# vice87/gam-ngs

Measured on AMD Instinct MI355X. Metric: GCUPS, higher is better.
Workload: dtype int32 (fast blocks: exact packed-f16 offsets from per-lane int32 bases, two tasks per register; results bit-identical to the reference's int64 DP)

## Files before the change

gam_ngs_amd/api.py:

```python
import ctypes as C
from dataclasses import dataclass, field
from typing import List, Optional, Sequence

from . import lib as L

GAP_A, GAP_B, MATCH, MISMATCH = 0, 1, 2, 3
OPS_CHARS = "ABMX"
DEFAULT_BAND_SIZE = 150


def _check(ctx, rc, what):
    if rc != 0:
        msg = L.load_library().gamdp_last_error(ctx.handle) if ctx is not None and ctx.handle else b""
        raise L.GamdpError("%s failed with code %d: %s" % (what, rc, (msg or b"").decode()))


class Context:

    def __init__(self, device: int = 0):
        self.lib = L.load_library()
        h = C.c_void_p()
        rc = self.lib.gamdp_ctx_create(device, C.byref(h))
        if rc != 0:
            raise L.GamdpError("gamdp_ctx_create(device=%d) failed with code %d (no gfx950 GPU?); "
                               "libgamdp has no CPU fallback" % (device, rc))
        self.handle = h
        self.device = device

    def set_arena_bytes(self, nbytes: int):
        _check(self, self.lib.gamdp_ctx_set_arena_bytes(self.handle, nbytes), "gamdp_ctx_set_arena_bytes")

    def last_error(self):
        return (self.lib.gamdp_last_error(self.handle) or b"").decode()

    def set_l1_hits(self, mode: int):
        _check(self, self.lib.gamdp_ctx_set_l1_hits(self.handle, mode), "gamdp_ctx_set_l1_hits")

    def l1_hits_stats(self):
        st = L.L1HitsStats()
        _check(self, self.lib.gamdp_ctx_l1_hits_stats(self.handle, C.byref(st)), "gamdp_ctx_l1_hits_stats")
        return st.as_dict()

    def set_l1_chain(self, mode: int):
        _check(self, self.lib.gamdp_ctx_set_l1_chain(self.handle, mode), "gamdp_ctx_set_l1_chain")

    def set_l1_walk_bands(self, which: int):
        _check(self, self.lib.gamdp_ctx_set_l1_walk_bands(self.handle, which), "gamdp_ctx_set_l1_walk_bands")

    def l1_chain_stats(self):
        st = L.L1ChainStats()
        _check(self, self.lib.gamdp_ctx_l1_chain_stats(self.handle, C.byref(st)), "gamdp_ctx_l1_chain_stats")
        return st.as_dict()

    def set_walk_skip(self, mode: int):
        _check(self, self.lib.gamdp_ctx_set_walk_skip(self.handle, mode), "gamdp_ctx_set_walk_skip")

    def walk_skip_stats(self):
        st = L.WalkSkipStats()
        _check(self, self.lib.gamdp_ctx_walk_skip_stats(self.handle, C.byref(st)), "gamdp_ctx_walk_skip_stats")
        return st.as_dict()

    def l1_tail_calls(self):
        n = C.c_size_t()
        _check(self, self.lib.gamdp_ctx_l1_tail_calls(self.handle, None, 0, C.byref(n)), "gamdp_ctx_l1_tail_calls")
        arr = (L.L1TailCall * max(1, n.value))()
        _check(self, self.lib.gamdp_ctx_l1_tail_calls(self.handle, arr, n.value, C.byref(n)), "gamdp_ctx_l1_tail_calls")
        return [(arr[i].merge_block, bool(arr[i].right), arr[i].begin_a, arr[i].source) for i in range(n.value)]

    def kernel_time(self, reset=False):
        ms, n = C.c_double(), C.c_uint64()
        self.lib.gamdp_ctx_kernel_time(self.handle, C.byref(ms), C.byref(n), int(reset))
        return ms.value, n.value

    def launch_info(self):
        n = C.c_size_t()
        self.lib.gamdp_ctx_launch_info(self.handle, None, 0, C.byref(n))
        arr = (L.LaunchInfo * max(1, n.value))()
        self.lib.gamdp_ctx_launch_info(self.handle, arr, n.value, C.byref(n))
        return [arr[i].as_dict() for i in range(n.value)]

    def score_info(self):
        n = C.c_size_t()
        self.lib.gamdp_ctx_score_info(self.handle, None, 0, C.byref(n))
        arr = (L.ScoreLaunchInfo * max(1, n.value))()
        self.lib.gamdp_ctx_score_info(self.handle, arr, n.value, C.byref(n))
        return [arr[i].as_dict() for i in range(n.value)]

    def carry_info(self):
        n = C.c_size_t()
        self.lib.gamdp_ctx_carry_info(self.handle, None, 0, C.byref(n))
        arr = (L.ScoreLaunchInfo * max(1, n.value))()
        self.lib.gamdp_ctx_carry_info(self.handle, arr, n.value, C.byref(n))
        return [arr[i].as_dict() for i in range(n.value)]

    def close(self):
        if getattr(self, "handle", None):
            self.lib.gamdp_ctx_destroy(self.handle)
            self.handle = None

    def __del__(self):
        try:
            self.close()
        except Exception:
            pass


class SequenceSet:

    def __init__(self, ctx: Context, seqs: Sequence[bytes], ascii: bool = True):
        self.ctx = ctx
        n = len(seqs)
        self._keep = [bytes(s) for s in seqs]
        arr = (C.c_char_p * max(1, n))(*self._keep)
        lens = (C.c_uint64 * max(1, n))(*[len(s) for s in self._keep])
        h = C.c_void_p()
        rc = ctx.lib.gamdp_seqset_create(ctx.handle, arr, lens, n, int(ascii), C.byref(h))
        _check(ctx, rc, "gamdp_seqset_create")
        self.handle = h
        self.lengths = [len(s) for s in self._keep]

    @classmethod
    def from_fasta(cls, ctx: "Context", path: str):
        names, codes = load_fasta(path)
        self = cls(ctx, codes, ascii=False)
        self.names = names
        return self

    @classmethod
    def synthetic(cls, ctx: "Context", first_pair: int, n_pairs: int, length: int, stride: int = 1):
        self = cls.__new__(cls)
        self.ctx = ctx
        self._keep = []
        h = C.c_void_p()
        _check(ctx, ctx.lib.gamdp_seqset_create_synth_strided(ctx.handle, first_pair, stride, n_pairs, length, C.byref(h)),
               "gamdp_seqset_create_synth_strided")
        self.handle = h
        self.lengths = [ctx.lib.gamdp_seqset_length(h, i) for i in range(2 * n_pairs)]
        return self

    def __len__(self):
        return len(self.lengths)

    def contig(self, idx, rc=False, off=0):
        return Contig(self, idx, rc, off)

    def close(self):
        if getattr(self, "handle", None) and self.ctx.handle:
            self.ctx.lib.gamdp_seqset_destroy(self.handle)
        self.handle = None

    def __del__(self):
        try:
            self.close()
        except Exception:
            pass


class MultiContext:

    def __init__(self, devices: Sequence[int]):
        self.lib = L.load_library()
        arr = (C.c_int * len(devices))(*devices)
        h = C.c_void_p()
        rc = self.lib.gamdp_multi_create(arr, len(devices), C.byref(h))
        if rc != 0:
            raise L.GamdpError("gamdp_multi_create(%r) failed with code %d; libgamdp has no CPU fallback" % (list(devices), rc))
        self.handle = h
        self.devices = list(devices)

    def last_error(self):
        return (self.lib.gamdp_multi_last_error(self.handle) or b"").decode()

    def set_l1_hits(self, mode: int):
        for i in range(len(self.devices)):
            if self.lib.gamdp_ctx_set_l1_hits(self.lib.gamdp_multi_ctx(self.handle, i), mode) != 0:
                raise L.GamdpError("gamdp_ctx_set_l1_hits(%r) failed on context %d" % (mode, i))

    def set_l1_chain(self, mode: int):
        for i in range(len(self.devices)):
            if self.lib.gamdp_ctx_set_l1_chain(self.lib.gamdp_multi_ctx(self.handle, i), mode) != 0:
                raise L.GamdpError("gamdp_ctx_set_l1_chain(%r) failed on context %d" % (mode, i))

    def set_l1_walk_bands(self, which: int):
        for i in range(len(self.devices)):
            if self.lib.gamdp_ctx_set_l1_walk_bands(self.lib.gamdp_multi_ctx(self.handle, i), which) != 0:
                raise L.GamdpError("gamdp_ctx_set_l1_walk_bands(%r) failed on context %d" % (which, i))

    def set_walk_skip(self, mode: int, which=None):
        for i in (range(len(self.devices)) if which is None else (which,)):
            if self.lib.gamdp_ctx_set_walk_skip(self.lib.gamdp_multi_ctx(self.handle, i), mode) != 0:
                raise L.GamdpError("gamdp_ctx_set_walk_skip(%r) failed on context %d" % (mode, i))

    def walk_skip_stats(self):
        out = []
        for i in range(len(self.devices)):
            st = L.WalkSkipStats()
            if self.lib.gamdp_ctx_walk_skip_stats(self.lib.gamdp_multi_ctx(self.handle, i), C.byref(st)) != 0:
                raise L.GamdpError("gamdp_ctx_walk_skip_stats failed on context %d" % i)
            out.append(st.as_dict())
        return out

    def l1_chain_stats(self):
        out = []
        for i in range(len(self.devices)):
            st = L.L1ChainStats()
            if self.lib.gamdp_ctx_l1_chain_stats(self.lib.gamdp_multi_ctx(self.handle, i), C.byref(st)) != 0:
                raise L.GamdpError("gamdp_ctx_l1_chain_stats failed on context %d" % i)
            out.append(st.as_dict())
        return out

    def l1_hits_stats(self):
        out = []
# ... 471 lines not shown
```

gam_ngs_amd/csrc/gamdp_dev.h:

```cpp
#pragma once
#include <stdint.h>

namespace gamdp {

typedef uint32_t u32;
typedef uint64_t u64;

constexpr int SEQ_PAD_BASES = 4096;

#ifndef GAMDP_WAVES_PER_SIMD
#define GAMDP_WAVES_PER_SIMD 5
#endif

struct DevTask {
    const u32* a2;
    const u32* an;
    const u32* b2;
    const u32* bn;
    int64_t a_base;
    int64_t b_base;
    int64_t end_a;
    int32_t alen, blen;
    int32_t begin_a, begin_b;
    int32_t X;
    int32_t band;
    u32 flags;
    u32 res_idx;
    u64 ops_off;
    u64 ops_cap;
};

enum : u32 { TF_FORCE_START = 1, TF_FORCE_END = 2, TF_WANT_OPS = 4,
             TF_DIAG_SKIP_TRACEBACK = 8 ,
             TF_NO_DIRFREE = 16 ,
             TF_DIAG_COUNT_MAT = 32 ,
             TF_PADDING = 64 ,
             TF_CALL_N = 128  };

#ifdef GAMDP_DIAG
constexpr u32 TF_LIVE_MASK = ~0u;
#else
constexpr u32 TF_LIVE_MASK = ~(u32)(TF_DIAG_SKIP_TRACEBACK | TF_NO_DIRFREE | TF_DIAG_COUNT_MAT);
#endif

struct DevResult {
    int32_t begin_a, begin_b;
    int32_t score;
    u32 n_match, length;
    int32_t first_a, first_b, last_a, last_b;
    u32 flags;
};

struct LaunchParams {
    const DevTask* tasks;
    u32 n_tasks;
    u32* cursor;
    DevResult* results;
    uint8_t* ops_buf;
    u32* scratch;
    u64 slot_words;
    u64 dir_words;
    u32 ypad;
    u64 ckpt_off;
    u64 bnd_off;
    u32 flags;
    u32 prio_R, prio_from;
    u32* stats;
};
enum : int { LS_UNITS = 0, LS_DIRFREE, LS_PACKED_TOP, LS_PACKED_TOP_MIXED, LS_STRIPS, LS_TOP_WANTED, LS_SKIP_TESTS, LS_SKIP_TESTED, LS_SKIP_GROUPS, LS_SKIP_SHORT, LS_COUNT = 12 };
constexpr u32 LP_WALK_SKIP_DIAG = 32;
constexpr u32 LP_WALK_SIDE_BY_SIDE = 1;
constexpr u32 LP_NO_PACKED_TOP = 2;
constexpr u32 LP_NO_PACKED_TOP_MIXED = 16;
constexpr u32 LP_WALK_PRIO_SHIFT = 8;

enum KernelId : int {
    K_C17_CE4 = 0,
    K_C17_CE4_N,
    K_C5_CE0,
    K_C5_CE0_N,
    K_P17_CE4,
    K_O19_CE15,
    K_Q19_CE15,
    K_Q19_CE15_N,
    K_GEN_C2, K_GEN_C3, K_GEN_C5, K_GEN_C9, K_GEN_C17,
    K_WIDE,
    K_COUNT
};

constexpr int FAMILY_COLS[5] = {2, 3, 5, 9, 17};
constexpr int band_cols(const u32 band)
{
    for (int k = 0; k < 4; k++) if (2 * (u64)band + 1 <= 64u * (u64)FAMILY_COLS[k]) return FAMILY_COLS[k];
    return 17;
}
constexpr int cols_index(const int cols)
{
    for (int k = 0; k < 4; k++) if (FAMILY_COLS[k] == cols) return k;
    return 4;
}
static_assert(K_GEN_C3 == K_GEN_C2 + 1 && K_GEN_C5 == K_GEN_C2 + 2 && K_GEN_C9 == K_GEN_C2 + 3 && K_GEN_C17 == K_GEN_C2 + 4,
              "K_GEN_C2 .. K_GEN_C17: contiguous, in the order of FAMILY_COLS");
constexpr int gen_kernel_id(const int cols) { return (int)K_GEN_C2 + cols_index(cols); }

#if defined(__HIPCC__)
#define GAMDP_HD __host__ __device__
#else
#define GAMDP_HD
#endif

constexpr u32 PAT_OFF = 0x2000u, PAT_MIN = 0x0400u, PAT_MAX = 0x7BFFu - 21u;
GAMDP_HD inline u32 pat_encode(int rel) { return (PAT_OFF + (u32)rel) & 0xFFFFu; }
GAMDP_HD inline int pat_decode(u32 p16) { return (int)(int16_t)(uint16_t)p16 - (int)PAT_OFF; }

GAMDP_HD inline int preflight_hd(u64 alen, u64 blen, u64 band, u64 begin_a, u64 end_a, u64 begin_b, u64 end_b, bool fs, bool fe,
                                 u64* X_out, u64* cells_out)
{
    constexpr int64_t MAXGAP = 10;
    enum { S_OK = 0, S_EMPTY = 1, S_OOR = 2, S_INVALID = 3 };
    auto mn = [](int64_t x, int64_t y) { return x < y ? x : y; };
    *X_out = 0;
    *cells_out = 0;
    if (end_b < begin_b) return S_EMPTY;
    if (begin_a >= (1ull << 31) - 65536) return S_INVALID;
    const int64_t lo = ((int64_t)begin_a - (int64_t)band) > 0 ? ((int64_t)begin_a - (int64_t)band) : 0, hi = (int64_t)begin_a + (int64_t)band;
    if (begin_b >= blen) {
        bool any;
        if (!fs) any = lo < (int64_t)alen;
        else any = (lo <= mn(hi, MAXGAP)) || lo < (int64_t)alen;
        return any ? S_OOR : S_INVALID;
    }
    if (end_b >= blen) end_b = blen - 1;
    u64 X = end_b - begin_b + 1;
    const u64 lim = alen + band - begin_a;
    if (lim < X) X = lim;
    if (X > 500000) X = 500000;
    if (X == 0) return S_INVALID;
    const u64 Y = 2 * band + 1;
    *X_out = X;
    *cells_out = X * Y;
    if (fs) {
        const int64_t up = mn(hi, MAXGAP);
        if (lo <= up && up >= (int64_t)alen) return S_OOR;
    }
    if (begin_a > alen + band) {
        bool found = false;
        if (!fe) found = begin_a + (X - 1) - band <= end_a;
        {
            const bool ge = end_a >= begin_a + band;
            const int64_t i0 = ge ? (int64_t)(end_a - (begin_a + band)) : 0;
            const int64_t j0 = ge ? (int64_t)(2 * band) : (int64_t)(2 * band) - (int64_t)(begin_a + band - end_a);
            if (j0 >= 0 && (u64)i0 < X) {
                const int64_t kmax = mn((int64_t)X - 1 - i0, j0);
                if (!fe) found = true;
                else if (X >= (u64)MAXGAP + 1 && (u64)(i0 + kmax) >= X - 1 - (u64)MAXGAP) found = true;
            }
        }
        return found ? S_OOR : S_EMPTY;
    }
    return S_OK;
}

GAMDP_HD inline bool npre_window_has_n(const u32* pre, int64_t len, bool rc, u64 off, int64_t lo, int64_t hi)
{
    if (pre == nullptr) return false;
    const int64_t o_lo = (int64_t)off + (lo > 0 ? lo : 0), o_hi = ((int64_t)off + hi < len - 1) ? (int64_t)off + hi : len - 1;
    if (o_lo > o_hi) return false;
    const int64_t f_lo = rc ? len - 1 - o_hi : o_lo, f_hi = rc ? len - 1 - o_lo : o_hi;
    return pre[(f_hi / 256) + 1] != pre[f_lo / 256];
}
GAMDP_HD inline bool call_touches_n(const u32* pre_a, int64_t alen, bool a_rc, u64 a_off, const u32* pre_b, int64_t blen, bool b_rc, u64 b_off,
                                    int64_t band, int64_t begin_a, int64_t begin_b, int64_t X, int64_t margin)
{
    return npre_window_has_n(pre_a, alen, a_rc, a_off, begin_a - band - margin, begin_a + X - 1 + band + margin) ||
           npre_window_has_n(pre_b, blen, b_rc, b_off, begin_b - margin, begin_b + X - 1 + margin);
}

struct DevBlk { int32_t m_begin, m_end, s_begin, s_end; };
struct DevMB {
    const u32 *a2, *an;
    const u32 *b2, *bn;
    const u32 *b2rc, *bnrc;
    u64 mlen, slen;
    u64 m_start, s_start, s_end;
    u64 align_thr;
    u32 first_blk, n_blocks;
    u32 audit_first;
    u32 rows;
    u32 try_rev;
    u32 has_n;
    const u32 *npre_a, *npre_b;
    u32 max_x;
    u64 slot_off[2];
    u64 slot_words, dir_words;
    u64 ckpt_off, bnd_off;
};
struct ChainOut { u32 n_dp; u32 state; u32 t_begin, t_end; u32 hw, hw_twin; u32 t_end_att[2]; u32 t_begin2; u32 pad; };
struct ChainWin { u64 begin_a, end_a, begin_b, end_b; u32 X; u32 info; };
struct ChainSync { u32 verdict[2]; u32 n[2]; u32 fin; u32 cancel; u32 t_begin; u32 hw[2]; u32 t_end[2]; u32 t_begin2; };
struct ChainParams {
    const DevMB* mbs; const DevBlk* blks; u32 n_mbs;
    u32 n_twins;
    ChainSync* sync;
    u32 first_mb;
    u32* cursor;
    DevResult* audit; ChainOut* out;
    ChainWin* win;
    u32* scratch; u32 ypad; u32 band;
    u32 max_rows;
    DevResult* host_audit; ChainOut* host_out; u32* host_done; u32 epoch;
    ChainWin* host_win;
    u32 skew_call;
    int32_t n_margin;
    u32 n_by_contig;
};
int chain_slots_per_workgroup();

struct KernelInfo {
    KernelId id;
    const char* name;
    int cols;
    u32 band;
    int tasks_per_wave;
    int waves_per_cu;
    bool n_aware;
    bool dirfree;
    bool two_dir_images;
    int dir_block_words;
    int ckpt_words;
    int bnd_words;
    void (*kernel)(LaunchParams);
};
extern const KernelInfo kernel_info[K_COUNT];

inline u64 dir_words_for(const KernelInfo& ki, const u64 X, const u64 band)
{
    const u64 Y = 2 * band + 1;
    if (ki.id == K_WIDE) return X * Y;
    const u64 C = (u64)ki.cols, LE = (Y - 1) / C;
    const u64 extra = ki.tasks_per_wave > 1 ? 3 : 0;
    return ((X - 1 + LE) / 16 + 1 + extra) * (u64)ki.dir_block_words;
}
struct SlotGeom { u64 dir_words; u32 ypad; u64 slot_words, ckpt_off, bnd_off; };
inline SlotGeom slot_geom(const KernelInfo& ki, const u64 max_dir_words, const u32 max_band)
{
    SlotGeom g;
    g.ypad = ((2 * max_band + 2 + 63) / 64) * 64;
    g.dir_words = ((max_dir_words + 63) / 64) * 64;
    const u64 tpw = (u64)ki.tasks_per_wave;
    u64 ckpt_words = 0, bnd_words = 0;
    if (tpw > 1 || ki.dirfree) {
        const u64 nblk = g.dir_words / (u64)ki.dir_block_words + 1;
        ckpt_words = (nblk / 4 + 2) * (u64)ki.ckpt_words;
        bnd_words = (nblk + 4) * (u64)ki.bnd_words;
    }
    const u64 sides_end = (ki.two_dir_images ? 2 * g.dir_words : g.dir_words) + 4ull * g.ypad * tpw;
    g.slot_words = sides_end + ckpt_words + bnd_words;
    g.ckpt_off = ckpt_words ? sides_end : 0;
    g.bnd_off = g.ckpt_off + ckpt_words;
    return g;
}

struct KernelFamily {
    const void* kernel[5];
    const char* name[5];
    unsigned threads;
};
const KernelFamily& score_family();
const KernelFamily& carry_family();
const KernelFamily& chain_carry_family();
const KernelFamily& chain_gen_family();

enum ChainNBit : int {
    CHAIN_N_UNREPORTED,
    CHAIN_N_BY_WINDOW,
    CHAIN_N_EVERY_DP
};
struct ChainKernel {
    const char* name;
    const void* kernel;
    int cols;
    unsigned threads;
    const KernelInfo* slots;
    bool twins;
    ChainNBit n_bit;
};
const ChainKernel& chain2_kernel(bool has_n);
inline ChainKernel family_chain_kernel(const KernelFamily& f, const int cols, const KernelInfo* slots, const bool twins, const ChainNBit n_bit)
{
    return ChainKernel{f.name[cols_index(cols)], f.kernel[cols_index(cols)], cols, f.threads, slots, twins, n_bit};
}

int launch_align(int kid, const LaunchParams& p, unsigned n_slots, unsigned dyn_lds, void* stream);
int launch_wide(const LaunchParams& p, unsigned n_slots, void* stream);
constexpr int WIDE_WORKGROUPS_PER_CU = 8;

struct alignas(16) ScoreRec {
    int32_t score, end_a, end_b;
    u32 info;
};
struct ScoreParams {
    const DevTask* tasks;
    u32 n_tasks;
    u32* cursor;
    ScoreRec* results;
};

struct CarryParams {
    const DevTask* tasks;
    u32 n_tasks;
    u32* cursor;
    DevResult* results;
};
constexpr u32 CARRY_COLS_SHIFT = 16;


}
```

gam_ngs_amd/csrc/gamdp_host.cpp:

```cpp
#include <hip/hip_runtime.h>

#include <algorithm>
#include <atomic>
#include <thread>
#include <cstdio>
#include <cstdlib>
#include <chrono>
#include <cstring>
#include <memory>
#include <mutex>
#include <string>
#include <vector>

#include "gamdp.h"
#include "gamdp_dev.h"
#include "gamdp_internal.h"
#include "gamdp_hostpool.h"
#include "gamdp_hostsort.h"

namespace gamdp {

#define HIPCHK(ctx, expr)                                                                         \
    do {                                                                                          \
        hipError_t e_ = (expr);                                                                   \
        if (e_ != hipSuccess) {                                                                   \
            (ctx)->set_error(std::string(#expr) + ": " + hipGetErrorString(e_));                  \
            return GAMDP_EHIP;                                                                    \
        }                                                                                         \
    } while (0)

const Diag& diag()
{
    static const Diag d = [] {
        Diag x;
        x.timing = std::getenv("GAMDP_DIAG_TIMING") != nullptr;
#ifdef GAMDP_DIAG
        x.build = true;
        x.skip_traceback = std::getenv("GAMDP_DIAG_SKIP_TRACEBACK") != nullptr;
        x.no_dirfree = std::getenv("GAMDP_DIAG_NO_DIRFREE") != nullptr;
        x.count_mat = std::getenv("GAMDP_DIAG_COUNT_MAT") != nullptr;
        x.force_n = std::getenv("GAMDP_DIAG_FORCE_N") != nullptr;
        if (const char* e = std::getenv("GAMDP_DIAG_N_WINDOW_SHRINK")) x.n_window_shrink = (int64_t)std::atol(e);
        if (const char* e = std::getenv("GAMDP_DIAG_CHAIN_SKEW")) x.chain_skew = (u32)std::atoi(e);
        x.hits_drop = std::getenv("GAMDP_DIAG_HITS_DROP") != nullptr;
#endif
        return x;
    }();
    return d;
}

const Tuning& tuning()
{
    static const Tuning t = [] {
        Tuning x;
        auto set = [](const char* name) { return std::getenv(name) != nullptr; };
        const char* e;
        x.no_merge_n = set("GAMDP_NO_MERGE_N") || set("GAMDP_QUAD_MIN");
        if ((e = std::getenv("GAMDP_QUAD_MIN"))) x.quad_min = std::atol(e);
        if ((e = std::getenv("GAMDP_OCTO_MIN_ROWS"))) x.octo_min_rows = (size_t)std::min(std::max(std::atol(e), 0L), 500000L);
        x.no_pair = set("GAMDP_NO_PAIR");
        x.no_aux_launch = set("GAMDP_NO_AUX_LAUNCH");
        if ((e = std::getenv("GAMDP_SIDE_WALK_ROUNDS"))) x.side_walk_rounds = (u64)std::min(std::max(std::atol(e), 0L), 1000000L);
        x.no_packed_top = set("GAMDP_NO_PACKED_TOP");
        x.no_packed_top_mixed = set("GAMDP_NO_PACKED_TOP_MIXED");
        if ((e = std::getenv("GAMDP_WALK_PRIO"))) x.walk_prio = std::atoi(e) & 3;
        x.no_prio = set("GAMDP_NO_PRIO");
        if ((e = std::getenv("GAMDP_CHUNK_MIN"))) x.chunk_min = (long)std::atoll(e);
        if ((e = std::getenv("GAMDP_CHUNK_MIN_ROUNDS"))) x.chunk_min_rounds = std::min(std::max(std::atof(e), 0.0), 1000.0);
        if ((e = std::getenv("GAMDP_CHUNK_FIRST_DIV"))) x.chunk_first_div = (size_t)std::min(std::max(4L, std::atol(e)), 1024L);
        x.l1_rounds = set("GAMDP_L1_ROUNDS");
        x.l1_no_twins = set("GAMDP_L1_NO_TWINS");
        if ((e = std::getenv("GAMDP_L1_COHORTS"))) x.l1_cohorts = std::min(16, std::max(1, std::atoi(e)));
        if ((e = std::getenv("GAMDP_L1_COHORT_MIN"))) x.l1_cohort_min = (size_t)std::max(1L, std::atol(e));
        if ((e = std::getenv("GAMDP_L1_DEVICE_HITS"))) x.l1_device_hits = std::atoi(e) == 1;
        if ((e = std::getenv("GAMDP_L1_CHAIN_CARRY"))) x.l1_chain_carry = std::atoi(e) == 1;
        if ((e = std::getenv("GAMDP_L1_WALK_ANY_BAND"))) x.l1_walk_any_band = std::atoi(e) == 1;
        if ((e = std::getenv("GAMDP_WALK_SKIP"))) x.walk_skip = std::atoi(e) == 1;
        return x;
    }();
    return t;
}


static inline uint8_t encode_char(char ch)
{
    switch (ch) {
    case 'A': case 'a': return 0;
    case 'T': case 't': return 1;
    case 'C': case 'c': return 2;
    case 'G': case 'g': return 3;
    default: return 4;
    }
}

static inline u64 padded_bases(u64 len) { return ((len + 2 * (u64)SEQ_PAD_BASES + 63) / 64) * 64 + 64; }

static void pack_into(const uint8_t* codes, u64 len, bool rc, u32* plane2, u32* planeN, u64 at)
{
    static const uint8_t comp[5] = {1, 0, 3, 2, 4};
    for (u64 i = 0; i < len; i++) {
        uint8_t c = rc ? comp[codes[len - 1 - i] > 4 ? 4 : codes[len - 1 - i]] : codes[i];
        if (c > 4) c = 4;
        const u64 k = at + i;
        if (c == 4) planeN[k >> 5] |= 1u << (k & 31);
        else plane2[k >> 4] |= (u32)c << ((k & 15) * 2);
    }
}

int SeqSet::upload(Ctx* ctx_, const uint8_t* const* seqs, const uint64_t* lens, uint32_t n, bool ascii)
{
    ctx = ctx_;
    codes.resize(n);
    this->lens.assign(lens, lens + n);
    fwd.resize(n);
    rc.assign(n, DevSeq{nullptr, nullptr});
    has_n.assign(n, 0);
    npre.assign(n, std::vector<u32>());
    u64 total = 0;
    std::vector<u64> at(n);
    for (u32 i = 0; i < n; i++) {
        if (lens[i] >= (1ull << 31) - (1ull << 20)) return GAMDP_EINVAL;
        at[i] = total + SEQ_PAD_BASES;
        total += padded_bases(lens[i]);
    }
    std::vector<u32> h2(total / 16 + 4, 0), hn(total / 32 + 4, 0);
    for (u32 i = 0; i < n; i++) {
        codes[i].resize(lens[i]);
        bool anyn = false;
        for (u64 k = 0; k < lens[i]; k++) {
            uint8_t c = ascii ? encode_char((char)seqs[i][k]) : (seqs[i][k] > 4 ? (uint8_t)4 : seqs[i][k]);
            codes[i][k] = c;
            anyn |= (c == 4);
        }
        has_n[i] = anyn;
        if (anyn) {
            std::vector<u32>& pre = npre[i];
            pre.assign((size_t)(lens[i] + 255) / 256 + 1, 0);
            for (u64 k = 0; k < lens[i]; k++) pre[(size_t)(k / 256) + 1] += (codes[i][k] == 4);
            for (size_t k = 1; k < pre.size(); k++) pre[k] += pre[k - 1];
        }
        pack_into(codes[i].data(), lens[i], false, h2.data(), hn.data(), at[i]);
    }
    HIPCHK(ctx, hipMalloc(&d2, h2.size() * sizeof(u32)));
    HIPCHK(ctx, hipMalloc(&dn, hn.size() * sizeof(u32)));
    HIPCHK(ctx, hipMemcpyAsync(d2, h2.data(), h2.size() * sizeof(u32), hipMemcpyHostToDevice, ctx->stream));
    HIPCHK(ctx, hipMemcpyAsync(dn, hn.data(), hn.size() * sizeof(u32), hipMemcpyHostToDevice, ctx->stream));
    HIPCHK(ctx, hipStreamSynchronize(ctx->stream));
    for (u32 i = 0; i < n; i++) fwd[i] = DevSeq{d2 + at[i] / 16, dn + at[i] / 32};
    dev_npre.assign(n, nullptr);
    {
        std::vector<u32> all;
        std::vector<size_t> first(n, 0);
        for (u32 i = 0; i < n; i++) { first[i] = all.size(); all.insert(all.end(), npre[i].begin(), npre[i].end()); }
        if (!all.empty()) {
            HIPCHK(ctx, hipMalloc(&d_npre, all.size() * sizeof(u32)));
            HIPCHK(ctx, hipMemcpy(d_npre, all.data(), all.size() * sizeof(u32), hipMemcpyHostToDevice));
            for (u32 i = 0; i < n; i++) if (!npre[i].empty()) dev_npre[i] = d_npre + first[i];
        }
    }
    return 0;
}


namespace {
struct SynthGen {
    uint64_t s;
    explicit SynthGen(uint64_t k) : s(0x47414DULL + k * 0xD1B54A32D192ED03ULL) { (void)next(); }
    uint64_t next()
    {
        uint64_t z = (s += 0x9E3779B97F4A7C15ULL);
        z = (z ^ (z >> 30)) * 0xBF58476D1CE4E5B9ULL;
        z = (z ^ (z >> 27)) * 0x94D049BB133111EBULL;
        return z ^ (z >> 31);
    }
};
uint64_t synth_pair_codes(uint64_t k, uint64_t len, uint8_t* master, uint8_t* slave)
{
    SynthGen g(k);
    for (uint64_t i = 0; i < len; i++) master[i] = (uint8_t)(g.next() >> 62);
    uint64_t n = 0;
    for (uint64_t i = 0; i < len; i++) {
        const uint64_t r = g.next(), u = r >> 40;
        if (u >= 167772) {
            uint8_t base = master[i];
            if (u < 671088) base = (uint8_t)((base + 1 + (r & 0xFFFF) % 3) & 3);
            slave[n++] = base;
        }
        const uint64_t r2 = g.next();
        if ((r2 >> 40) < 167772) slave[n++] = (uint8_t)(r2 & 3);
    }
    return n;
}
}

int SeqSet::upload_synth(Ctx* ctx_, uint64_t first_pair, uint64_t stride_pairs, uint32_t n_pairs, uint64_t len)
{
    ctx = ctx_;
    const u32 n = 2 * n_pairs;
    lens.assign(n, 0);
    fwd.resize(n);
    rc.assign(n, DevSeq{nullptr, nullptr});
    has_n.assign(n, 0);
    dev_npre.assign(n, nullptr);
    const u64 stride = padded_bases(len + len / 8 + 64);
    const u64 total = stride * n;
    std::vector<u32> h2(total / 16 + 4, 0), hn(total / 32 + 4, 0);
    const unsigned nt = std::max(1u, std::min(32u, std::thread::hardware_concurrency()));
    Threads pool;
    std::atomic<u32> cursor(0);
    std::atomic<int> failed(0);
    for (unsigned t = 0; t < nt; t++) {
        pool.start([&]() {
            failed |= guarded_thread_body([&]() -> int {
            std::vector<uint8_t> m(len), s(len + len / 8 + 64);
            for (;;) {
                const u32 k = cursor.fetch_add(1);
                if (k >= n_pairs) break;
                const u64 sl = synth_pair_codes(first_pair + (u64)k * stride_pairs, len, m.data(), s.data());
                lens[2 * k] = len;
                lens[2 * k + 1] = sl;
                pack_into(m.data(), len, false, h2.data(), hn.data(), stride * (2 * k) + SEQ_PAD_BASES);
                pack_into(s.data(), sl, false, h2.data(), hn.data(), stride * (2 * k + 1) + SEQ_PAD_BASES);
            }
            return 0;
            });
        });
    }
    pool.join();
    if (failed) return GAMDP_ENOMEM;
    HIPCHK(ctx, hipMalloc(&d2, h2.size() * sizeof(u32)));
// ... 361 lines not shown

static void pair_aux_launch(std::vector<Launch>& launches, int n_cu, u64 arena_call)
{
    int small = -1, big = -1;
    for (size_t li = 0; li < launches.size(); li++) {
        const Launch& L = launches[li];
        const u64 tpw = (u64)kernel_info[L.kid].tasks_per_wave, units = L.count / tpw;
        if (tpw == 1 && L.kid != K_WIDE && units <= (u64)L.n_slots && units <= 4ull * (u64)n_cu) { if (small < 0) small = (int)li; }
        else if (tpw > 1 && units >= 2ull * L.n_slots) { if (big < 0) big = (int)li; }
    }
    if (small < 0 || big < 0 || launches.size() != 2) return;
    const u64 main_words = launches[big].slot_words * launches[big].n_slots, small_words = launches[small].slot_words * launches[small].n_slots;
    if ((main_words + small_words) * sizeof(u32) <= arena_call) {
        launches[small].aux = true;
        launches[small].scratch_off = main_words;
    }
}

int Ctx::align_plan(u64 arena_call)
{
    Plan& plan = w_plan;
    plan.launches.clear(); plan.items.clear(); plan.n_host_tasks = 0;
    const std::vector<u32>& rowsv = w_rows;
    for (int kid = 0; kid < K_COUNT; kid++) {
        auto& g = w_groups[kid];
        if (g.empty()) continue;
        const KernelInfo& ki = kernel_info[kid];
        const u32 max_resident = (u32)n_cu * (u32)ki.waves_per_cu;
        if (ki.band != 0) sort_by_key_desc(g, rowsv, &w_sort_tmp, &w_sort_count);
        else sort_by_key_desc(g, w_key, &w_sort_tmp, &w_sort_count);
        std::vector<std::vector<u32>> work;
        work.push_back(g);
        while (!work.empty()) {
            std::vector<u32> cur = std::move(work.back());
            work.pop_back();
            u32 maxband = ki.band;
            u64 maxdir = 0;
            if (ki.band != 0) maxdir = dir_words_for(ki, rowsv[cur[0]], ki.band);
            else {
                std::mutex red;
                parallel_for(cur.size(), [&](size_t lo, size_t hi) {
                    u32 mb = 0; u64 md = 0;
                    for (size_t k = lo; k < hi; k++) { const u32 i = cur[k]; mb = std::max<u32>(mb, (u32)w_prep[i].dt.band); md = std::max(md, w_prep[i].dir_words); }
                    std::lock_guard<std::mutex> gd(red);
                    maxband = std::max(maxband, mb); maxdir = std::max(maxdir, md);
                });
            }
            const SlotGeom geom = slot_geom(ki, maxdir, maxband);
            const u32 tpw = (u32)ki.tasks_per_wave;
            const u64 fit = arena_call / (geom.slot_words * sizeof(u32));
            if (fit == 0) { set_error("scratch arena too small for one task"); return GAMDP_ENOMEM; }
            const u64 want = std::min<u64>((cur.size() + tpw - 1) / tpw, max_resident);
            if (fit < want && cur.size() > 1) {
                std::vector<u32> big, small;
                for (u32 i : cur) ((ki.band ? dir_words_for(ki, rowsv[i], ki.band) : w_prep[i].dir_words) * 2 >= maxdir ? big : small).push_back(i);
                if (!small.empty()) {
                    work.push_back(std::move(small));
                    work.push_back(std::move(big));
                    continue;
                }
            }
            Launch L;
            const size_t padded = (cur.size() + tpw - 1) / tpw * tpw;
            L.kid = kid; L.first = (u32)plan.n_host_tasks; L.count = (u32)padded;
            L.slot_words = geom.slot_words; L.dir_words = geom.dir_words; L.ypad = geom.ypad; L.band_max = maxband;
            L.ckpt_off = geom.ckpt_off; L.bnd_off = geom.bnd_off;
            L.n_slots = (u32)std::min<u64>(want, fit);
            L.dyn_lds = 0;
            plan.n_host_tasks += padded;
            plan.items.push_back(std::move(cur));
            plan.launches.push_back(L);
        }
    }
    if (!tuning().no_aux_launch && !interval_sink && !defer_frees) pair_aux_launch(plan.launches, n_cu, arena_call);
    return 0;
}


int Ctx::grow_staging(u64 base)
{
    if (base + 1 <= cap_pinned) return 0;
    free_host(h_tasks);
    free_host(h_results);
    h_tasks = nullptr; h_results = nullptr; cap_pinned = 0;
    const u64 want = base + base / 4 + 256;
    if (hipHostMalloc(&h_tasks, want * sizeof(DevTask)) != hipSuccess ||
        hipHostMalloc(&h_results, want * sizeof(DevResult)) != hipSuccess) {
        set_error("hipHostMalloc of staging buffers failed");
        return GAMDP_ENOMEM;
    }
    cap_pinned = want;
    return 0;
}

int Ctx::align_stage(const AlignCall& a)
{
    const Plan& plan = w_plan;
    int rc_ = grow(this, d_tasks, cap_tasks, plan.n_host_tasks + 1);
    if (rc_) return rc_;
    if ((rc_ = grow_staging(std::max<u64>(plan.n_host_tasks, a.n)))) return rc_;
    for (size_t li = 0; li < plan.launches.size(); li++) {
        const std::vector<u32>& cur = plan.items[li];
        const Launch& L = plan.launches[li];
        DevTask* dst = h_tasks + L.first;
        parallel_for(cur.size(), [&](size_t lo, size_t hi) { for (size_t k = lo; k < hi; k++) dst[k] = w_prep[cur[k]].dt; });
        auto pad = [&](size_t k, const DevTask& of) { dst[k] = of; dst[k].res_idx = (u32)a.n; dst[k].flags = (dst[k].flags & ~(u32)TF_WANT_OPS) | TF_PADDING; };
        size_t k = cur.size();
        for (; k < L.count; k++) pad(k, dst[cur.size() - 1]);
    }
    return 0;
}

int Ctx::align_scratch(u64 arena_call)
{
    const std::vector<Launch>& launches = w_plan.launches;
    u64 need_scratch = 0;
    for (auto& L : launches) need_scratch = std::max(need_scratch, L.scratch_off + L.slot_words * L.n_slots);
    if (need_scratch > cap_scratch) {
        if (d_scratch) { free_dev(d_scratch); d_scratch = nullptr; cap_scratch = 0; }
        if (defer_frees) need_scratch = std::max(need_scratch, std::min<u64>(2 * need_scratch, arena_call / sizeof(u32)));
        if (hipMalloc(&d_scratch, need_scratch * sizeof(u32)) != hipSuccess) {
            d_scratch = nullptr;
            (void)hipGetLastError();
            flush_frees();
            if (arena_div == 1) {
                for (Ctx* h : helpers)
                    if (h->d_scratch) { (void)hipFree(h->d_scratch); h->d_scratch = nullptr; h->cap_scratch = 0; }
                if (d_chain_scratch) { (void)hipFree(d_chain_scratch); d_chain_scratch = nullptr; cap_chain_scratch = 0; }
            }
            if (hipMalloc(&d_scratch, need_scratch * sizeof(u32)) != hipSuccess) {
                d_scratch = nullptr;
                set_error("hipMalloc of scratch arena (" + std::to_string(need_scratch * sizeof(u32)) + " bytes) failed");
                return GAMDP_ENOMEM;
            }
        }
        cap_scratch = need_scratch;
    }
    if (launches.size() > cap_cursor) {
        free_dev(d_cursor);
        d_cursor = nullptr; cap_cursor = 0;
        HIPCHK(this, hipMalloc(&d_cursor, launches.size() * (1 + LS_COUNT) * sizeof(u32)));
        cap_cursor = (u32)launches.size();
    }
    return 0;
}

static void launch_policy(const Launch& L, LaunchParams& p, const int walk_skip)
{
    const Tuning& tu = tuning();
    const u64 tpw = (u64)kernel_info[L.kid].tasks_per_wave, units = L.count / tpw;
    p.flags = (L.kid == K_P17_CE4 && (u64)L.count / 2 <= tu.side_walk_rounds * L.n_slots) ? LP_WALK_SIDE_BY_SIDE : 0u;
    if (tu.no_packed_top) p.flags |= LP_NO_PACKED_TOP;
    if (tu.no_packed_top_mixed) p.flags |= LP_NO_PACKED_TOP_MIXED;
    if (L.kid == K_O19_CE15 && walk_skip == GAMDP_WALK_SKIP_DIAG) p.flags |= LP_WALK_SKIP_DIAG;
    p.flags |= (tu.walk_prio >= 0 ? (u32)tu.walk_prio : (units > 2ull * L.n_slots ? 1u : 0u)) << LP_WALK_PRIO_SHIFT;
    p.prio_R = tu.no_prio ? 0u : (u32)std::max<u64>(1, L.dir_words / (u64)kernel_info[L.kid].dir_block_words);
    const u64 shaped = (L.kid == K_P17_CE4 ? 2ull : 1ull) * L.n_slots;
    p.prio_from = units <= 2ull * L.n_slots ? 0u : (u32)(units - std::min<u64>(units, shaped));
}

int Ctx::align_run(AlignCall& a)
{
    const std::vector<Launch>& launches = w_plan.launches;
    u32* const d_stats = d_cursor + cap_cursor;
    a.t_gpu = std::chrono::steady_clock::now();
    bool any_aux = false;
    for (auto& L : launches) any_aux |= L.aux;
    struct AuxJoin {
        Ctx* c = nullptr;
        ~AuxJoin() { if (c) { (void)hipEventRecord(c->aux_done, c->aux_stream); (void)hipStreamWaitEvent(c->stream, c->aux_done, 0); } }
    } aux_join;
    HIPCHK(this, hipMemsetAsync(d_cursor, 0, (size_t)cap_cursor * (1 + LS_COUNT) * sizeof(u32), stream));
    if (any_aux) {
        if (!aux_stream) {
            HIPCHK(this, hipStreamCreateWithFlags(&aux_stream, hipStreamNonBlocking));
            HIPCHK(this, hipEventCreateWithFlags(&aux_done, hipEventDisableTiming));
            HIPCHK(this, hipEventCreateWithFlags(&aux_go, hipEventDisableTiming));
        }
        HIPCHK(this, hipEventRecord(aux_go, stream));
        HIPCHK(this, hipStreamWaitEvent(aux_stream, aux_go, 0));
        aux_join.c = this;
        for (auto& L : launches)
            if (L.aux) HIPCHK(this, hipMemcpyAsync(d_tasks + L.first, h_tasks + L.first, (size_t)L.count * sizeof(DevTask), hipMemcpyHostToDevice, aux_stream));
        for (auto& L : launches)
            if (!L.aux) HIPCHK(this, hipMemcpyAsync(d_tasks + L.first, h_tasks + L.first, (size_t)L.count * sizeof(DevTask), hipMemcpyHostToDevice, stream));
    } else {
        HIPCHK(this, hipMemcpyAsync(d_tasks, h_tasks, w_plan.n_host_tasks * sizeof(DevTask), hipMemcpyHostToDevice, stream));
    }
    while (events.size() < launches.size()) {
        hipEvent_t e0, e1;
        HIPCHK(this, hipEventCreate(&e0));
        HIPCHK(this, hipEventCreate(&e1));
        events.push_back({e0, e1});
    }
    for (size_t li = 0; li < launches.size(); li++) {
        const Launch& L = launches[li];
        LaunchParams p;
        p.tasks = d_tasks + L.first; p.n_tasks = L.count; p.cursor = d_cursor + li;
        p.results = d_results; p.ops_buf = d_ops;
        p.scratch = d_scratch + L.scratch_off; p.slot_words = L.slot_words; p.dir_words = L.dir_words; p.ypad = L.ypad;
        p.ckpt_off = L.ckpt_off; p.bnd_off = L.bnd_off;
        p.stats = d_stats + li * LS_COUNT;
        launch_policy(L, p, walk_skip);
        hipStream_t const on = L.aux ? aux_stream : stream;
        HIPCHK(this, hipEventRecord(events[li].first, on));
        const int e = launch_align(L.kid, p, L.n_slots, L.dyn_lds, on);
        if (e != 0) { set_error(std::string("kernel launch failed: ") + hipGetErrorString((hipError_t)e)); return GAMDP_EHIP; }
        HIPCHK(this, hipEventRecord(events[li].second, on));
    }
    if (any_aux) {
        aux_join.c = nullptr;
        HIPCHK(this, hipEventRecord(aux_done, aux_stream));
        HIPCHK(this, hipStreamWaitEvent(stream, aux_done, 0));
    }
    HIPCHK(this, hipMemcpyAsync(h_results, d_results, a.n * sizeof(DevResult), hipMemcpyDeviceToHost, stream));
    a.hops.resize(a.ops_total);
    if (a.ops_total) HIPCHK(this, hipMemcpyAsync(a.hops.data(), d_ops, a.ops_total, hipMemcpyDeviceToHost, stream));
    a.hstats.resize(log_launches ? launches.size() * LS_COUNT : 0);
    if (!a.hstats.empty()) HIPCHK(this, hipMemcpyAsync(a.hstats.data(), d_stats, a.hstats.size() * sizeof(u32), hipMemcpyDeviceToHost, stream));
    a.mark("enqueued");
    HIPCHK(this, hipStreamSynchronize(stream));
    a.mark("gpu done");
    a.ms_gpu = a.since(a.t_gpu);
    return 0;
}

void Ctx::align_collect(AlignCall& a)
{
    const std::vector<Launch>& launches = w_plan.launches;
    const size_t n = a.n;
    bool any_aux = false;
    for (auto& L : launches) any_aux |= L.aux;
    float busy_hi = 0;
    for (size_t li = 0; li < launches.size(); li++) {
        const Launch& L = launches[li];
        const KernelInfo& ki = kernel_info[L.kid];
        float ms = 0;
        if (hipEventElapsedTime(&ms, events[li].first, events[li].second) == hipSuccess) {
            kernel_launches++;
            if (!any_aux) kernel_ms += ms;
            else {
                float off = 0;
                if (li > 0 && hipEventElapsedTime(&off, events[0].first, events[li].first) != hipSuccess) off = busy_hi;
                const float lo = std::max(off, busy_hi), hi = off + ms;
                if (hi > lo) kernel_ms += hi - lo;
                busy_hi = std::max(busy_hi, hi);
            }
        }
        if (log_launches) {
            gamdp_launch_info r;
            std::memset(&r, 0, sizeof(r));
            std::snprintf(r.kernel, sizeof(r.kernel), "%s", ki.name);
            r.n_aware = ki.n_aware ? 1u : 0u;
            r.tasks_per_wavefront = (u32)ki.tasks_per_wave;
            r.tasks = (u32)w_plan.items[li].size();
            r.units = L.count / r.tasks_per_wavefront;
            r.slots = L.n_slots;
            r.band_max = L.band_max;
            const u32* st = a.hstats.data() + li * LS_COUNT;
            r.units_dirfree = st[LS_DIRFREE]; r.units_packed_top = st[LS_PACKED_TOP]; r.units_packed_top_mixed = st[LS_PACKED_TOP_MIXED];
            r.strips = st[LS_STRIPS]; r.units_top_wanted = st[LS_TOP_WANTED];
            if (L.kid == K_O19_CE15) {
                gamdp_walk_skip_stats& W = last_walk_skip;
                W.tests += st[LS_SKIP_TESTS]; W.groups_tested += st[LS_SKIP_TESTED]; W.groups_skipped += st[LS_SKIP_GROUPS];
                W.rows_skipped += 64ull * st[LS_SKIP_GROUPS] - st[LS_SKIP_SHORT];
                W.strips += st[LS_STRIPS];
            }
            r.piece = log_piece;
            r.rounds = L.n_slots ? (double)r.units / (double)L.n_slots : 0.0;
            r.kernel_ms = (double)ms;
            launch_log.push_back(r);
        }
        if (interval_sink && ref_event) {
            float t0 = 0;
            if (hipEventElapsedTime(&t0, ref_event, events[li].first) == hipSuccess) interval_sink->push_back({t0, t0 + ms});
        }
    }
    a.t_fill = std::chrono::steady_clock::now();
    a.mark("events");
    const DevResult* hres = h_results;
    gamdp_result* out = a.out;
    parallel_for(n, [&](size_t lo, size_t hi) {
        for (size_t i = lo; i < hi; i++) {
            if (w_kid[i] < 0) continue;
            fill_result(hres[i], w_key[i], out[i]);
        }
    });
    if (a.ops_total) {
        parallel_for(w_plan.n_host_tasks, [&](size_t lo, size_t hi) {
            for (size_t q = lo; q < hi; q++) {
                const DevTask& d = h_tasks[q];
                const u32 i = d.res_idx;
                if (i >= n) continue;
                if ((d.flags & TF_WANT_OPS) && out[i].status == GAMDP_ST_OK) {
                    const u64 len = std::min<u64>(out[i].length, d.ops_cap);
                    uint8_t* dst = a.ops->ops_buf + a.ops->ops_off[i];
                    const uint8_t* src = a.hops.data() + d.ops_off;
                    if (out[i].length <= d.ops_cap) for (u64 k = 0; k < len; k++) dst[k] = src[len - 1 - k];
                    else for (u64 k = 0; k < len; k++) dst[k] = 0xFF;
                }
            }
        });
    }
    if (diag().timing) {
        a.mark("results");
        std::fprintf(stderr, "libgamdp align: %zu tasks, %zu launches: prepare %.2f ms, plan+stage %.2f ms, upload+kernels+download %.2f ms [ctx %p began %.3f]\n",
                     n, launches.size(), a.ms_prep, a.ms_plan, a.ms_gpu, (void*)this,
                     std::chrono::duration<double, std::milli>(a.t_begin.time_since_epoch()).count());
        std::fprintf(stderr, "libgamdp align: results %.2f ms [ctx %p began %.3f]\n", a.marks.back().second - std::chrono::duration<double, std::milli>(a.t_fill - a.t_begin).count(), (void*)this,
                     std::chrono::duration<double, std::milli>(a.t_fill.time_since_epoch()).count());
        std::string line = "libgamdp align: phases (ms since the call began):";
        for (auto& m : a.marks) { char b[64]; std::snprintf(b, sizeof b, " %s %.2f", m.first, m.second); line += b; }
        std::fprintf(stderr, "%s; kernels %.2f ms\n", line.c_str(), [&] { double k = 0; for (auto& r : launch_log) k += r.kernel_ms; return k; }());
    }
}

int Ctx::align(const TaskSrc& tasks, size_t n, gamdp_result* out, const gamdp_ops* ops)
{
    if (hipSetDevice(device) != hipSuccess) { set_error("hipSetDevice failed"); return GAMDP_EHIP; }
    if (n == 0) return 0;
    int rc_ = align_check(tasks, n);
    if (rc_) return rc_;
    AlignCall a{tasks, n, out, ops};
    align_prepare(a);
    align_group(a);
    route_merge_n(w_groups, a.rows_of, w_prep, w_kid, n_cu);
    route_band150(w_groups, a.rows_of, n_cu);
    route_band512(w_groups);
    a.ms_prep = a.since(a.t_begin);
    a.mark("groups");
    rc_ = grow(this, d_results, cap_results, n + 1);
    if (rc_) return rc_;
    if (a.ops_total) { rc_ = grow(this, d_ops, cap_ops, a.ops_total); if (rc_) return rc_; }
    if (arena_budget() == 0) { set_error("hipMemGetInfo failed"); return GAMDP_EHIP; }
    const u64 arena_call = this->arena_call();
    if ((rc_ = align_plan(arena_call))) return rc_;
    a.mark("sort+plan");
    if ((rc_ = align_stage(a))) return rc_;
    a.mark("staging");
    if (w_plan.launches.empty()) return 0;
    if ((rc_ = align_scratch(arena_call))) return rc_;
    a.ms_plan = a.since(a.t_begin) - a.ms_prep;
    a.mark("buffers");
    if ((rc_ = align_run(a))) return rc_;
    align_collect(a);
    w_plan.items.clear();
    return 0;
}


struct ScoreCall {
    typedef ScoreRec Rec;
    typedef gamdp_score_result Out;
    typedef ScoreParams Params;
    static constexpr const char* api = "gamdp_score_batch";
    static const KernelFamily& family() { return score_family(); }
    static u32 cols_of(const Rec& r) { return r.info >> 8; }
    static void collect(const Rec& r, u64 cells, Out& o)
    {
        (void)cells;
        o.status = (uint8_t)(r.info & 0xFFu);
        if (o.status != GAMDP_ST_OK) return;
        o.score = r.score;
        o.end_a = (u64)(int64_t)r.end_a; o.end_b = (u64)(int64_t)r.end_b;
    }
};
struct CarryCall {
    typedef DevResult Rec;
    typedef gamdp_result Out;
    typedef CarryParams Params;
    static constexpr const char* api = "gamdp_carry_batch";
    static const KernelFamily& family() { return carry_family(); }
    static u32 cols_of(const Rec& r) { return r.flags >> CARRY_COLS_SHIFT; }
    static void collect(const Rec& r, u64 cells, Out& o) { fill_result(r, cells, o); }
};

template <class K>
int Ctx::fill_only(const TaskSrc& tasks, size_t n, typename K::Out* out, std::vector<gamdp_score_launch_info>& log)
{
    typedef typename K::Rec Rec;
    if (hipSetDevice(device) != hipSuccess) { set_error("hipSetDevice failed"); return GAMDP_EHIP; }
    log.clear();
    if (n == 0) return 0;
    int rc_ = align_check(tasks, n);
    if (rc_) return rc_;
    for (size_t i = 0; i < n; i++) {
        const u32 band = tasks[i].band;
        if (band > GAMDP_MAX_TUNED_BAND) {
            set_error(std::string(K::api) + ": task " + std::to_string(i) + " has band " + std::to_string(band) + ", above GAMDP_MAX_TUNED_BAND");
            return GAMDP_ENOTSUP;
        }
    }
    if (w_prep.size() < n) { w_prep.resize(n); w_status.resize(n); w_key.resize(n); w_kid.resize(n); w_rows.resize(n); }
    std::vector<int8_t> colsv(n);
    parallel_for(n, [&](size_t lo, size_t hi) {
        for (size_t i = lo; i < hi; i++) {
            const int st = w_status[i] = prepare_task(tasks[i], w_prep[i]);
            w_key[i] = w_prep[i].cells;
            std::memset(&out[i], 0, sizeof(out[i]));
            out[i].status = (uint8_t)st;
            out[i].cells = w_prep[i].cells;
            w_prep[i].dt.res_idx = (u32)i;
            colsv[i] = st != GAMDP_ST_OK ? (int8_t)-1 : (int8_t)band_cols((u32)w_prep[i].dt.band);
            w_rows[i] = st != GAMDP_ST_OK ? 0u : (u32)w_prep[i].dt.X;
        }
    });
    struct SLaunch { int cols; u32 first, count, band_max; };
    std::vector<SLaunch> launches;
    std::vector<u32> order, g;
    for (const int cols : FAMILY_COLS) {
        g.clear();
        u32 band_max = 0;
        for (size_t i = 0; i < n; i++) if (colsv[i] == cols) { g.push_back((u32)i); band_max = std::max(band_max, (u32)w_prep[i].dt.band); }
        if (g.empty()) continue;
        sort_by_key_desc(g, w_rows, &w_sort_tmp, &w_sort_count);
        launches.push_back({cols, (u32)order.size(), (u32)g.size(), band_max});
        order.insert(order.end(), g.begin(), g.end());
    }
    if (launches.empty()) return 0;
    static_assert(sizeof(Rec) <= sizeof(DevResult), "the records are staged in the result buffers of align()");
// ... 19 lines not shown
        typename K::Params p;
        p.tasks = d_tasks + L.first; p.n_tasks = L.count; p.cursor = d_cursor + li; p.results = d_rec;
        const int e = launch_kernel(K::family().kernel[cols_index(L.cols)], K::family().threads, p, slots[li], stream);
        if (e != 0) { set_error(std::string("kernel launch failed: ") + hipGetErrorString((hipError_t)e)); return GAMDP_EHIP; }
        HIPCHK(this, hipEventRecord(events[li].second, stream));
    }
    HIPCHK(this, hipMemcpyAsync(h_rec, d_rec, n * sizeof(Rec), hipMemcpyDeviceToHost, stream));
    HIPCHK(this, hipStreamSynchronize(stream));
    parallel_for(n, [&](size_t lo, size_t hi) {
        for (size_t i = lo; i < hi; i++) {
            if (colsv[i] < 0) continue;
            K::collect(h_rec[i], w_key[i], out[i]);
        }
    });
    for (size_t li = 0; li < launches.size(); li++) {
        const SLaunch& L = launches[li];
        float ms = 0;
        if (hipEventElapsedTime(&ms, events[li].first, events[li].second) == hipSuccess) { kernel_launches++; kernel_ms += ms; }
        gamdp_score_launch_info r;
        std::memset(&r, 0, sizeof(r));
        std::snprintf(r.kernel, sizeof(r.kernel), "%s", K::family().name[cols_index(L.cols)]);
        r.cols = K::cols_of(h_rec[order[L.first]]);
        for (u32 k = 0; k < L.count; k++) if (K::cols_of(h_rec[order[L.first + k]]) != r.cols) r.cols = 0;
        r.tasks = L.count; r.slots = slots[li]; r.band_max = L.band_max;
        r.kernel_ms = (double)ms;
        log.push_back(r);
    }
    return 0;
}

int Ctx::score(const TaskSrc& tasks, size_t n, gamdp_score_result* out) { return fill_only<ScoreCall>(tasks, n, out, score_log); }
int Ctx::carry(const TaskSrc& tasks, size_t n, gamdp_result* out) { return fill_only<CarryCall>(tasks, n, out, carry_log); }


static bool batch_pieces(const gamdp_task* tasks, size_t n, const SeqSet* sb, int n_cu, size_t bound[5])
{
    const long chunk_env = tuning().chunk_min;
    bool chunked = chunk_env >= 0 && n >= (size_t)chunk_env;
    bool b150 = false;
    if (chunked) { size_t n150 = 0, cnt = 0; for (size_t i = 0; i < n; i += 64, cnt++) n150 += tasks[i].band == 150; b150 = 2 * n150 >= cnt; }
    if (chunk_env < 0 && n >= 65536) {
        double est = 0;
        size_t cnt = 0;
        size_t n150 = 0;
        u64 rows_max = 0, rows_sum = 0;
        for (size_t i = 0; i < n; i += 64, cnt++) {
            const gamdp_task& t = tasks[i];
            const u64 blen = t.b_id < sb->lens.size() ? sb->lens[t.b_id] - std::min<u64>(t.b_off, sb->lens[t.b_id]) : 0;
            const u64 eb = blen ? std::min<u64>(t.end_b, blen - 1) : 0;
            const u64 rows = (blen && eb >= t.begin_b) ? std::min<u64>(eb - t.begin_b + 1, 500000) : 0;
            est += (double)rows * (2.0 * t.band + 1.0);
            rows_max = std::max(rows_max, rows); rows_sum += rows;
            n150 += t.band == 150;
        }
        b150 = 2 * n150 >= cnt;
        chunked = est / (double)std::max<size_t>(1, cnt) < (b150 ? 4.5e6 : 8e6);
        const double units_per_piece = (double)n * (7.0 / 24.0) / (b150 ? 8.0 : 2.0);
        const bool one_length = (double)rows_max * (double)std::max<size_t>(1, cnt) <= 1.25 * (double)rows_sum;
        const double min_rounds_env = tuning().chunk_min_rounds;
        const double min_rounds = min_rounds_env >= 0 ? min_rounds_env : (one_length ? 3.0 : 2.5);
        if (units_per_piece < min_rounds * 16.0 * (double)n_cu) chunked = false;
        {
            const double cells_total = est / (double)std::max<size_t>(1, cnt) * (double)n;
            const double kernel_ms = cells_total / (b150 ? 7.0e9 : 12.0e9), host_ms = (double)n * 1.5e-5;
            if (min_rounds_env < 0 && host_ms < 0.05 * kernel_ms) chunked = false;
        }
    }
    if (!chunked) return false;
    const size_t first_div = tuning().chunk_first_div;
    const size_t round = (size_t)n_cu * 16 * (b150 ? 8 : 2);
    auto whole = [&](size_t v, bool up) { const size_t r = up ? (v + round - 1) / round : v / round; return std::max<size_t>(1, r) * round; };
    const bool by_rounds = chunk_env < 0;
    const size_t n0 = by_rounds ? std::min(n, whole(n / first_div, false)) : n / first_div;
    const size_t per = by_rounds ? whole((n - n0 + 2) / 3, true) : (n - n0 + 2) / 3;
    const size_t b[5] = {0, n0, std::min(n, n0 + per), std::min(n, n0 + 2 * per), n};
    std::copy(b, b + 5, bound);
    return true;
}

}

using namespace gamdp;

extern "C" {

int gamdp_ctx_create(int device, gamdp_ctx** out)
{
    if (!out) return GAMDP_EINVAL;
    *out = nullptr;
    Ctx* c = new (std::nothrow) Ctx();
    if (!c) return GAMDP_ENOMEM;
    const int rc_ = c->init(device);
    if (rc_) {
        std::fprintf(stderr, "libgamdp: %s\n", c->err.c_str());
        delete c;
        return rc_;
    }
    *out = reinterpret_cast<gamdp_ctx*>(c);
    return 0;
}

void gamdp_ctx_destroy(gamdp_ctx* ctx) { delete reinterpret_cast<Ctx*>(ctx); }

int gamdp_ctx_set_arena_bytes(gamdp_ctx* ctx, uint64_t bytes)
{
    if (!ctx) return GAMDP_EINVAL;
    Ctx* c = reinterpret_cast<Ctx*>(ctx);
    c->arena_limit = bytes;
    c->arena_auto = bytes == 0;
    for (Ctx* h : c->helpers) h->arena_limit = bytes;
    return 0;
}

const char* gamdp_last_error(const gamdp_ctx* ctx) { return ctx ? reinterpret_cast<const Ctx*>(ctx)->err.c_str() : "null ctx"; }

void* gamdp_ctx_stream(gamdp_ctx* ctx) { return ctx ? (void*)reinterpret_cast<Ctx*>(ctx)->stream : nullptr; }

int gamdp_ctx_kernel_time(gamdp_ctx* ctx, double* total_ms, uint64_t* launches, int reset)
{
    if (!ctx) return GAMDP_EINVAL;
    Ctx* c = reinterpret_cast<Ctx*>(ctx);
    if (total_ms) *total_ms = c->kernel_ms;
    if (launches) *launches = c->kernel_launches;
    if (reset) { c->kernel_ms = 0; c->kernel_launches = 0; }
    return 0;
}

int gamdp_ctx_launch_info(const gamdp_ctx* ctx, gamdp_launch_info* out, size_t cap, size_t* n)
{
    if (!ctx || (cap && !out)) return GAMDP_EINVAL;
    const Ctx* c = reinterpret_cast<const Ctx*>(ctx);
    if (n) *n = c->launch_log.size();
    for (size_t i = 0; i < c->launch_log.size() && i < cap; i++) out[i] = c->launch_log[i];
    return 0;
}

static_assert(sizeof(gamdp_walk_skip_stats) == 48 && offsetof(gamdp_walk_skip_stats, strips) == 32 && offsetof(gamdp_walk_skip_stats, mode) == 40,
              "gamdp_walk_skip_stats: the layout include/gamdp.h documents (gam_ngs_amd/lib.py WalkSkipStats mirrors it)");

int gamdp_ctx_set_walk_skip(gamdp_ctx* ctx, int mode)
{
    if ((mode != GAMDP_WALK_STRIPS && mode != GAMDP_WALK_SKIP_DIAG) || !ctx) return GAMDP_EINVAL;
    reinterpret_cast<Ctx*>(ctx)->walk_skip = mode;
    return 0;
}

int gamdp_ctx_walk_skip_stats(const gamdp_ctx* ctx, gamdp_walk_skip_stats* out)
{
    if (!ctx || !out) return GAMDP_EINVAL;
    *out = reinterpret_cast<const Ctx*>(ctx)->last_walk_skip;
    return 0;
}

int gamdp_seqset_create(gamdp_ctx* ctx, const uint8_t* const* seqs, const uint64_t* lens, uint32_t n, int is_ascii,
                        gamdp_seqset** out)
{
    if (!ctx || !out || (n && (!seqs || !lens))) return GAMDP_EINVAL;
    *out = nullptr;
    Ctx* c = reinterpret_cast<Ctx*>(ctx);
    if (hipSetDevice(c->device) != hipSuccess) return GAMDP_EHIP;
    SeqSet* s = new (std::nothrow) SeqSet();
    if (!s) return GAMDP_ENOMEM;
    const int rc_ = guarded(c, [&] { return s->upload(c, seqs, lens, n, is_ascii != 0); });
    if (rc_) { delete s; return rc_; }
    *out = reinterpret_cast<gamdp_seqset*>(s);
    return 0;
}

void gamdp_seqset_destroy(gamdp_seqset* set)
{
    SeqSet* s = reinterpret_cast<SeqSet*>(set);
    if (s && s->ctx) (void)hipSetDevice(s->ctx->device);
    delete s;
}

uint32_t gamdp_seqset_size(const gamdp_seqset* set) { return set ? (uint32_t)reinterpret_cast<const SeqSet*>(set)->lens.size() : 0; }

uint64_t gamdp_seqset_length(const gamdp_seqset* set, uint32_t id)
{
    const SeqSet* s = reinterpret_cast<const SeqSet*>(set);
    return (s && id < s->lens.size()) ? s->lens[id] : 0;
}

int gamdp_align_batch(gamdp_ctx* ctx, const gamdp_seqset* set_a, const gamdp_seqset* set_b, const gamdp_task* tasks,
                      size_t n, gamdp_result* out, const gamdp_ops* ops)
{
    if (!ctx || !set_a || !set_b || (n && (!tasks || !out))) return GAMDP_EINVAL;
    Ctx* c = reinterpret_cast<Ctx*>(ctx);
    const SeqSet* sa = reinterpret_cast<const SeqSet*>(set_a);
    const SeqSet* sb = reinterpret_cast<const SeqSet*>(set_b);
    c->launch_log.clear();
    c->last_walk_skip = gamdp_walk_skip_stats{};
    c->last_walk_skip.mode = (uint32_t)c->walk_skip;
    struct LogGuard { Ctx* c; ~LogGuard() { c->log_launches = false; for (Ctx* h : c->helpers) h->log_launches = false; } } log_guard{c};
    c->log_launches = true; c->log_piece = 0;
    return guarded(c, [&]() -> int {
    const auto t_call = std::chrono::steady_clock::now();
    if (c->arena_budget(true) == 0) { c->set_error("hipMemGetInfo failed"); return GAMDP_EHIP; }
    const double ms_arena = std::chrono::duration<double, std::milli>(std::chrono::steady_clock::now() - t_call).count();
    struct CallTimer { std::chrono::steady_clock::time_point t0; size_t n; const double* arena; ~CallTimer() { if (diag().timing) std::fprintf(stderr, "libgamdp align_batch: %zu calls, %.2f ms in all (arena budget %.2f ms)\n", n, std::chrono::duration<double, std::milli>(std::chrono::steady_clock::now() - t0).count(), *arena); } } call_timer{t_call, n, &ms_arena};
    auto run = [&](Ctx* cc, size_t first, size_t cnt) -> int {
        TaskSrc src;
        src.gt = tasks + first; src.sa = sa; src.sb = sb;
        return cc->align(src, cnt, out + first, nullptr);
    };
    if (ops && ops->ops_buf) {
        TaskSrc src;
        src.gt = tasks; src.sa = sa; src.sb = sb;
        return c->align(src, n, out, ops);
    }
    size_t bound[5];
    if (n < 8 || !batch_pieces(tasks, n, sb, c->n_cu, bound)) return run(c, 0, n);
    if (hipSetDevice(c->device) != hipSuccess) { c->set_error("hipSetDevice failed"); return GAMDP_EHIP; }
    if (c->helpers.empty()) {
        Ctx* h = new (std::nothrow) Ctx();
        if (!h || h->init(c->device) != 0) { c->set_error("helper context: " + (h ? h->err : std::string("out of memory"))); delete h; return GAMDP_ENODEV; }
        c->helpers.push_back(h);
    }
    Ctx* cc[2] = {c, c->helpers[0]};
    if (c->arena_budget() == 0) { c->set_error("hipMemGetInfo failed"); return GAMDP_EHIP; }
    cc[1]->arena_limit = c->arena_limit; cc[1]->arena_share = c->arena_share;
    struct DivGuard { Ctx* a; Ctx* b; ~DivGuard() { a->arena_div = 1; b->arena_div = 1; } } div_guard{cc[0], cc[1]};
    cc[0]->arena_div = cc[1]->arena_div = 2;
    cc[0]->trim_scratch(); cc[1]->trim_scratch();
    cc[1]->kernel_ms = 0; cc[1]->kernel_launches = 0;
    cc[1]->launch_log.clear(); cc[1]->log_launches = true;
    cc[1]->walk_skip = c->walk_skip; cc[1]->last_walk_skip = gamdp_walk_skip_stats{};
    int rc[2] = {0, 0};
    auto worker = [&](int t) noexcept {
        for (size_t k = (size_t)t; k < 4 && rc[t] == 0; k += 2) {
            const size_t first = bound[k], cnt = bound[k + 1] - bound[k];
            cc[t]->log_piece = (u32)k;
            if (cnt) rc[t] = guarded(cc[t], [&] { return run(cc[t], first, cnt); });
        }
    };
    {
        Threads pool;
        pool.start(worker, 1);
        worker(0);
    }
    c->kernel_ms += cc[1]->kernel_ms; c->kernel_launches += cc[1]->kernel_launches;
    c->launch_log.insert(c->launch_log.end(), cc[1]->launch_log.begin(), cc[1]->launch_log.end());
    {
        gamdp_walk_skip_stats& W = c->last_walk_skip;
        const gamdp_walk_skip_stats& H = cc[1]->last_walk_skip;
        W.tests += H.tests; W.groups_tested += H.groups_tested; W.groups_skipped += H.groups_skipped; W.rows_skipped += H.rows_skipped; W.strips += H.strips;
    }
    std::stable_sort(c->launch_log.begin(), c->launch_log.end(), [](const gamdp_launch_info& x, const gamdp_launch_info& y) { return x.piece < y.piece; });
    if (rc[1]) c->set_error(cc[1]->err);
    return rc[0] ? rc[0] : rc[1];
    });
}

int gamdp_score_batch(gamdp_ctx* ctx, const gamdp_seqset* set_a, const gamdp_seqset* set_b, const gamdp_task* tasks, size_t n,
                      gamdp_score_result* out)
{
    if (!ctx || !set_a || !set_b || !out || (n && !tasks)) return GAMDP_EINVAL;
    Ctx* c = reinterpret_cast<Ctx*>(ctx);
    return guarded(c, [&]() -> int {
        TaskSrc src;
        src.gt = tasks; src.sa = reinterpret_cast<const SeqSet*>(set_a); src.sb = reinterpret_cast<const SeqSet*>(set_b);
        return c->score(src, n, out);
    });
}

int gamdp_ctx_score_info(const gamdp_ctx* ctx, gamdp_score_launch_info* out, size_t cap, size_t* n)
{
    if (!ctx || (cap && !out)) return GAMDP_EINVAL;
    const Ctx* c = reinterpret_cast<const Ctx*>(ctx);
    if (n) *n = c->score_log.size();
    for (size_t i = 0; i < c->score_log.size() && i < cap; i++) out[i] = c->score_log[i];
    return 0;
}

int gamdp_carry_batch(gamdp_ctx* ctx, const gamdp_seqset* set_a, const gamdp_seqset* set_b, const gamdp_task* tasks, size_t n,
                      gamdp_result* out)
{
    if (!ctx || !set_a || !set_b || !out || (n && !tasks)) return GAMDP_EINVAL;
    Ctx* c = reinterpret_cast<Ctx*>(ctx);
    return guarded(c, [&]() -> int {
        TaskSrc src;
        src.gt = tasks; src.sa = reinterpret_cast<const SeqSet*>(set_a); src.sb = reinterpret_cast<const SeqSet*>(set_b);
        return c->carry(src, n, out);
    });
}

int gamdp_ctx_carry_info(const gamdp_ctx* ctx, gamdp_score_launch_info* out, size_t cap, size_t* n)
{
    if (!ctx || (cap && !out)) return GAMDP_EINVAL;
    const Ctx* c = reinterpret_cast<const Ctx*>(ctx);
    if (n) *n = c->carry_log.size();
    for (size_t i = 0; i < c->carry_log.size() && i < cap; i++) out[i] = c->carry_log[i];
    return 0;
}

int gamdp_task_preflight(uint64_t alen, uint64_t blen, uint32_t band, uint64_t begin_a, uint64_t end_a, uint64_t begin_b,
                         uint64_t end_b, int force_start, int force_end, uint64_t* cells)
{
    u64 X = 0, c = 0;
    const int st = preflight(alen, blen, band, begin_a, end_a, begin_b, end_b, force_start != 0, force_end != 0, &X, &c);
    if (cells) *cells = c;
    return st;
}

unsigned gamdp_build_info(void) { return diag().build ? 1u : 0u; }

void gamdp_encode(const char* chars, uint64_t n, uint8_t* codes)
{
    for (uint64_t i = 0; i < n; i++) codes[i] = encode_char(chars[i]);
}

void gamdp_decode(const uint8_t* codes, uint64_t n, char* chars)
{
    static const char L[5] = {'A', 'T', 'C', 'G', 'N'};
    for (uint64_t i = 0; i < n; i++) chars[i] = L[codes[i] > 4 ? 4 : codes[i]];
}

void gamdp_revcomp(uint8_t* codes, uint64_t n)
{
    static const uint8_t comp[5] = {1, 0, 3, 2, 4};
    for (uint64_t i = 0; i < n / 2; i++) {
        const uint8_t x = comp[codes[i] > 4 ? 4 : codes[i]], y = comp[codes[n - 1 - i] > 4 ? 4 : codes[n - 1 - i]];
        codes[i] = y;
        codes[n - 1 - i] = x;
    }
    if (n & 1) codes[n / 2] = comp[codes[n / 2] > 4 ? 4 : codes[n / 2]];
}

int64_t gamdp_find_hits(const uint8_t* a, uint64_t alen, uint64_t a_start, uint64_t a_end, const uint8_t* b, uint64_t blen,
                        uint64_t b_start, uint64_t b_end, uint64_t word, uint32_t* hits, uint64_t cap)
{
    std::vector<uint32_t> h;
    find_hits(a, alen, a_start, a_end, b, blen, b_start, b_end, word, h);
    for (size_t i = 0; i < h.size() && i < cap && hits; i++) hits[i] = h[i];
    return (int64_t)h.size();
}

uint64_t gamdp_synth_pair(uint64_t k, uint64_t len, uint8_t* master, uint8_t* slave)
{
    return synth_pair_codes(k, len, master, slave);
}

int gamdp_seqset_create_synth(gamdp_ctx* ctx, uint64_t first_pair, uint32_t n_pairs, uint64_t len, gamdp_seqset** out)
{
    return gamdp_seqset_create_synth_strided(ctx, first_pair, 1, n_pairs, len, out);
}

int gamdp_seqset_create_synth_strided(gamdp_ctx* ctx, uint64_t first_pair, uint64_t stride_pairs, uint32_t n_pairs, uint64_t len,
                                      gamdp_seqset** out)
{
    if (!ctx || !out || len == 0 || len >= (1ull << 30) || n_pairs >= (1u << 30)) return GAMDP_EINVAL;
    *out = nullptr;
    Ctx* c = reinterpret_cast<Ctx*>(ctx);
    if (hipSetDevice(c->device) != hipSuccess) return GAMDP_EHIP;
    SeqSet* s = new (std::nothrow) SeqSet();
    if (!s) return GAMDP_ENOMEM;
    const int rc_ = guarded(c, [&] { return s->upload_synth(c, first_pair, stride_pairs, n_pairs, len); });
    if (rc_) { delete s; return rc_; }
    *out = reinterpret_cast<gamdp_seqset*>(s);
    return 0;
}

}
```

gam_ngs_amd/csrc/gamdp_internal.h:

```cpp
#pragma once
#include <hip/hip_runtime.h>

#include <algorithm>
#include <mutex>
#include <new>
#include <thread>
#include <string>
#include <utility>
#include <vector>

#include "gamdp.h"
#include "gamdp_dev.h"

namespace gamdp {

constexpr int64_t FORCE_MAXGAP_ = 10;

struct Ctx;

struct Diag {
    bool build = false;
    bool timing = false;
    bool skip_traceback = false;
    bool no_dirfree = false;
    bool count_mat = false;
    bool force_n = false;
    int64_t n_window_shrink = 0;
    u32 chain_skew = ~0u;
    bool hits_drop = false;
};
const Diag& diag();

struct Tuning {
    bool no_merge_n = false;
    long quad_min = -1;
    size_t octo_min_rows = 0;
    bool no_pair = false;
    bool no_aux_launch = false;
    u64 side_walk_rounds = 2;
    bool no_packed_top = false;
    bool no_packed_top_mixed = false;
    int walk_prio = -1;
    bool no_prio = false;
    long chunk_min = -1;
    double chunk_min_rounds = -1;
    size_t chunk_first_div = 8;
    bool l1_rounds = false;
    bool l1_no_twins = false;
    int l1_cohorts = 0;
    size_t l1_cohort_min = 48;
    bool l1_device_hits = false;
    bool l1_chain_carry = false;
    bool l1_walk_any_band = false;
    bool walk_skip = false;
};
const Tuning& tuning();

int preflight(u64 alen, u64 blen, u64 band, u64 begin_a, u64 end_a, u64 begin_b, u64 end_b, bool fs, bool fe,
              u64* X_out, u64* cells_out);

struct DevSeq {
    u32* p2;
    u32* pn;
};

struct SeqSet {
    Ctx* ctx = nullptr;
    std::vector<std::vector<uint8_t>> codes;
    std::vector<u64> lens;
    std::vector<uint8_t> has_n;
    std::vector<std::vector<u32>> npre;
    bool window_has_n(u32 id, bool rc, u64 off, int64_t lo, int64_t hi) const
    {
        if (!has_n[id]) return false;
        if (id >= npre.size() || npre[id].empty()) return true;
        return npre_window_has_n(npre[id].data(), (int64_t)lens[id], rc, off, lo, hi);
    }
    u32* d_npre = nullptr;
    std::vector<const u32*> dev_npre;
    std::vector<DevSeq> fwd;
    mutable std::vector<DevSeq> rc;
    mutable std::vector<u32*> rc_allocs;
    mutable std::mutex rc_mu;
    u32 *d2 = nullptr, *dn = nullptr;

    int upload(Ctx* ctx, const uint8_t* const* seqs, const uint64_t* lens, uint32_t n, bool ascii);
    int ensure_rc(const std::vector<u32>& ids, Ctx* use = nullptr) const;
    int upload_synth(Ctx* ctx, uint64_t first_pair, uint64_t stride_pairs, uint32_t n_pairs, uint64_t len);
    bool has_codes() const { return !codes.empty() || lens.empty(); }
    ~SeqSet();
};

struct ITask {
    const SeqSet* sa;
    const SeqSet* sb;
    u32 a_id, b_id;
    u64 a_off, b_off;
    bool a_rc, b_rc, force_start, force_end;
    u32 band;
    u64 begin_a, end_a, begin_b, end_b;
};

struct TaskSrc {
    const ITask* it = nullptr;
    const gamdp_task* gt = nullptr;
    const SeqSet* sa = nullptr;
    const SeqSet* sb = nullptr;
    ITask operator[](size_t i) const
    {
        if (it) return it[i];
        const gamdp_task& t = gt[i];
        return ITask{sa, sb, t.a_id, t.b_id, t.a_off, t.b_off, t.a_rc != 0, t.b_rc != 0, t.force_start != 0, t.force_end != 0, t.band, t.begin_a, t.end_a, t.begin_b, t.end_b};
    }
};

struct Prepared {
    DevTask dt;
    int kid;
    u64 cells;
    u64 dir_words;
};

struct Launch {
    int kid;
    u32 first, count;
    u64 slot_words, dir_words;
    u32 ypad, n_slots, dyn_lds;
    u64 ckpt_off, bnd_off;
    u32 band_max;
    u64 scratch_off = 0;
    bool aux = false;
};
struct Plan {
    std::vector<Launch> launches;
    std::vector<std::vector<u32>> items;
    u64 n_host_tasks = 0;
};
struct AlignCall;
struct HitsBuffers;
void hits_free(HitsBuffers* h);

struct Ctx {
    int device = -1;
    int n_cu = 0;
    u32 max_lds_per_wg = 65536;
    hipStream_t stream = nullptr;
    hipStream_t aux_stream = nullptr;
    hipEvent_t aux_done = nullptr, aux_go = nullptr;
    std::string err;
    u64 arena_limit = 0;
    bool arena_auto = true;
    u32 arena_share = 1, arena_div = 1;
    u64 arena_budget(bool refresh = false);
    u64 arena_call() const { return arena_limit / ((u64)(arena_share ? arena_share : 1) * (u64)(arena_div ? arena_div : 1)); }
    void trim_scratch();

    u32* d_scratch = nullptr; u64 cap_scratch = 0;
    DevTask* d_tasks = nullptr; u64 cap_tasks = 0;
    DevResult* d_results = nullptr; u64 cap_results = 0;
    uint8_t* d_ops = nullptr; u64 cap_ops = 0;
    u32* d_cursor = nullptr;
    u32 cap_cursor = 0;
    std::vector<gamdp_launch_info> launch_log;
    bool log_launches = false;
    u32 log_piece = 0;
    DevTask* h_tasks = nullptr;
    DevResult* h_results = nullptr;
    u64 cap_pinned = 0;
    std::vector<std::pair<hipEvent_t, hipEvent_t>> events;
    double kernel_ms = 0;
    u64 kernel_launches = 0;
    std::vector<Ctx*> helpers;
    hipEvent_t ref_event = nullptr;
    std::vector<std::pair<float, float>>* interval_sink = nullptr;
    gamdp_l1_stats last_l1{};
    int l1_hits_mode = GAMDP_L1_HITS_HOST;
    gamdp_l1_hits_stats last_l1_hits{};
    std::vector<gamdp_l1_tail_call> last_l1_tails;
    int l1_chain = GAMDP_L1_CHAIN_WALK;
    int walk_bands = GAMDP_L1_WALK_BAND_150;
    gamdp_l1_chain_stats last_l1_chain{};
    int walk_skip = GAMDP_WALK_STRIPS;
    gamdp_walk_skip_stats last_walk_skip{};
    HitsBuffers* hits = nullptr;

    void set_error(const std::string& s) { err = s; }
    int init(int dev);
    std::vector<Prepared> w_prep;
    std::vector<int> w_status;
    std::vector<u64> w_key;
    std::vector<int8_t> w_kid;
    std::vector<u32> w_rows;
    std::vector<std::vector<u32>> w_groups;
    std::vector<u32> w_sort_tmp; std::vector<size_t> w_sort_count;
    Plan w_plan;

    uint8_t* d_chain = nullptr; u64 cap_chain = 0;
    uint8_t* h_chain = nullptr; u64 cap_hchain = 0;
    hipStream_t chain_stream = nullptr;
    bool defer_frees = false;
    std::vector<void*> deferred_dev, deferred_host;
    void free_dev(void* p) { if (!p) return; if (defer_frees) deferred_dev.push_back(p); else (void)hipFree(p); }
    void free_host(void* p) { if (!p) return; if (defer_frees) deferred_host.push_back(p); else (void)hipHostFree(p); }
    void flush_frees()
    {
        for (void* p : deferred_dev) (void)hipFree(p);
        for (void* p : deferred_host) (void)hipHostFree(p);
        deferred_dev.clear(); deferred_host.clear();
    }
    u32* d_chain_scratch = nullptr; u64 cap_chain_scratch = 0;
    uint8_t* h_mirror = nullptr; u64 cap_mirror = 0;
    u32 chain_epoch = 0;

    int align(const TaskSrc& tasks, size_t n, gamdp_result* out, const gamdp_ops* ops);
    int align_check(const TaskSrc& tasks, size_t n);
    void align_prepare(AlignCall& a);
    void align_group(AlignCall& a);
    int align_plan(u64 arena_call);
    int align_stage(const AlignCall& a);
    int align_scratch(u64 arena_call);
    int align_run(AlignCall& a);
    void align_collect(AlignCall& a);
    int grow_staging(u64 base);
    int score(const TaskSrc& tasks, size_t n, gamdp_score_result* out);
    std::vector<gamdp_score_launch_info> score_log;
    int carry(const TaskSrc& tasks, size_t n, gamdp_result* out);
    std::vector<gamdp_score_launch_info> carry_log;
    template <class K> int fill_only(const TaskSrc& tasks, size_t n, typename K::Out* out, std::vector<gamdp_score_launch_info>& log);
    int align(const ITask* tasks, size_t n, gamdp_result* out, const gamdp_ops* ops) { TaskSrc s; s.it = tasks; return align(s, n, out, ops); }
    int align(const std::vector<ITask>& tasks, gamdp_result* out, const gamdp_ops* ops) { return align(tasks.data(), tasks.size(), out, ops); }
    ~Ctx();
};

struct Fasta {
    std::vector<std::string> names;
    std::vector<std::vector<uint8_t>> codes;
    std::string err;
};

template <class F>
int guarded(Ctx* c, F&& f) noexcept
{
    auto note = [&](const char* what) noexcept { try { if (c) c->set_error(what); } catch (...) {} };
    try { return f(); }
    catch (const std::bad_alloc&) { note("out of host memory"); return GAMDP_ENOMEM; }
    catch (const std::exception& e) { try { if (c) c->set_error(std::string("host exception: ") + e.what()); } catch (...) {} return GAMDP_EHIP; }
    catch (...) { note("unknown host exception"); return GAMDP_EHIP; }
}
template <class F>
int guarded_thread_body(F&& f) noexcept
{
    try { return f(); }
    catch (const std::bad_alloc&) { return GAMDP_ENOMEM; }
    catch (...) { return GAMDP_EHIP; }
}
struct Threads {
    std::vector<std::thread> th;
    template <class... A> void start(A&&... a) { th.emplace_back(std::forward<A>(a)...); }
    void join() { for (auto& t : th) if (t.joinable()) t.join(); }
    ~Threads() { join(); }
};

template <class T>
int grow(Ctx* ctx, T*& ptr, u64& cap, u64 need, bool exact = false)
{
    if (need <= cap) return 0;
    if (ptr) { ctx->free_dev(ptr); ptr = nullptr; cap = 0; }
    u64 want = exact ? need : need + (ctx->defer_frees ? need + 1024 : need / 4);
    if (hipMalloc(&ptr, want * sizeof(T)) != hipSuccess) {
        if (hipMalloc(&ptr, need * sizeof(T)) != hipSuccess) {
            ctx->set_error("hipMalloc of " + std::to_string(need * sizeof(T)) + " bytes failed");
            return GAMDP_ENOMEM;
        }
        want = need;
    }
    cap = want;
    return 0;
}

inline int grow_pinned(Ctx* ctx, uint8_t*& ptr, u64& cap, u64 need, unsigned flags)
{
    if (need <= cap) return 0;
    if (ptr) { ctx->free_host(ptr); ptr = nullptr; cap = 0; }
    const u64 want = need + need / 4;
    if (hipHostMalloc(&ptr, want, flags) != hipSuccess) {
        ptr = nullptr;
        ctx->set_error("hipHostMalloc of " + std::to_string(want) + " bytes failed");
        return GAMDP_ENOMEM;
    }
    cap = want;
    return 0;
}

template <class P>
int launch_kernel(const void* kernel, unsigned threads, const P& p, unsigned grid, void* stream)
{
    P copy = p;
    void* args[] = {&copy};
    return (int)hipLaunchKernel(kernel, dim3(grid), dim3(threads), args, 0, static_cast<hipStream_t>(stream));
}
inline int family_waves_per_cu(const KernelFamily& f, int cols)
{
    int n = 0;
    const hipError_t e = hipOccupancyMaxActiveBlocksPerMultiprocessor(&n, f.kernel[cols_index(cols)], (int)f.threads, 0);
    return (e == hipSuccess && n > 0) ? n : 4;
}

void fill_result(const DevResult& r, u64 cells, gamdp_result& o);

void partition_lpt(const u64* weights, size_t n, int parts, u32* part_of);

struct HitsReq {
    const SeqSet *sa, *sb;
    gamdp_hits_task t;
};
enum HitsHow : uint8_t { HITS_DEVICE = 0, HITS_TRIVIAL = 1, HITS_UNFIT = 2 };
int find_hits_queries(Ctx* c, const HitsReq* q, size_t n, gamdp_hits_result* out, uint32_t* hits_buf, const uint64_t* hits_off,
                      const uint64_t* hits_cap, uint8_t* how, double* kernel_ms = nullptr, u32* launches = nullptr);

void find_hits(const uint8_t* a, u64 alen, u64 a_start, u64 a_end, const uint8_t* b, u64 blen, u64 b_start, u64 b_end,
               u64 word, std::vector<uint32_t>& hits);

}
```

gam_ngs_amd/csrc/gamdp_kernel.hip:

```cpp
#include <hip/hip_runtime.h>

#include <type_traits>
#include <utility>

#include "gamdp_dev.h"

namespace gamdp {
namespace {

#include "kernel_common.inc"
#include "kernel_fill.inc"
#include "kernel_pair.inc"
#include "kernel_strip.inc"
#include "kernel_finish.inc"

#ifdef GAMDP_DIAG
__device__ __forceinline__ u32 diag_clock() { return (u32)wall_clock64(); }
__device__ __forceinline__ u32 diag_hw_id() { return ((u32)__builtin_amdgcn_s_getreg((3 << 11) | 20) << 16) | ((u32)__builtin_amdgcn_s_getreg((15 << 11) | 4) & 0xffffu); }
#else
__device__ __forceinline__ constexpr u32 diag_clock() { return 0u; }
__device__ __forceinline__ constexpr u32 diag_hw_id() { return 0u; }
#endif

__device__ __forceinline__ void count_unit(const LaunchParams& p, const int lane, const bool dirfree, const bool packed_top, const bool mixed_top, const bool top_wanted = false)
// ... 600 lines not shown
                const int32_t pm_b = uni(bk[-1].m_begin), pm_e = uni(bk[-1].m_end), ps_b = uni(bk[-1].s_begin), ps_e = uni(bk[-1].s_end);
                const int32_t mgap = pm_b <= cm_b ? (cm_b - pm_e - 1) : (pm_b - cm_e - 1);
                const int32_t sgap = ps_b <= cs_b ? (cs_b - ps_e - 1) : (ps_b - cs_e - 1);
                cur_ms = (int64_t)(last_a + (u64)(int64_t)mgap); if (cur_ms < 0) cur_ms = 0;
                cur_ss = (int64_t)(last_b + (u64)(int64_t)sgap); if (cur_ss < 0) cur_ss = 0;
            }
#ifdef GAMDP_DIAG
            if (attempt == 0 && k == cp.skew_call) ++cur_ss;
#endif
            const u64 begin_a = (u64)cur_ms, end_a = (u64)(cur_ms + ml - 1), begin_b = (u64)cur_ss, end_b = (u64)(cur_ss + sl - 1);
            set_prio_by_remaining(rows_left, (int)cp.max_rows);
            rows_left -= sl;
            u64 X = 0, cells = 0;
            const int st = preflight_hd(mlen, slen, band, begin_a, end_a, begin_b, end_b, false, false, &X, &cells);
            const u32 idx = audit_first + n_dp;
            if (st == 0 && X > (u64)max_x) { overflow = true; break; }
            bool call_n = false;
            if constexpr (CE < 0) call_n = st == 0;
            else if constexpr (HASN)
                call_n = st == 0 && (cp.n_by_contig != 0 || call_touches_n(unip(mb->npre_a), (int64_t)mlen, false, 0, unip(mb->npre_b), (int64_t)slen, try_rev, 0, (int64_t)band,
                                                                            (int64_t)begin_a, (int64_t)begin_b, (int64_t)X, (int64_t)cp.n_margin));
            if (lane == 0) { ChainWin w; w.begin_a = begin_a; w.end_a = end_a; w.begin_b = begin_b; w.end_b = end_b; w.X = (u32)X; w.info = (try_rev ? 1u : 0u) | (call_n ? 2u : 0u) | ((u32)st << 8); cp.win[idx] = w; }
            u32 status;
            if (st != 0) {
                DevResult r;
                r.begin_a = r.begin_b = r.score = 0; r.n_match = r.length = 0;
                r.first_a = r.first_b = r.last_a = r.last_b = 0;
                r.flags = (u32)st << 8;
                if (lane == 0) cp.audit[idx] = r;
                status = (u32)st;
                last_a = last_b = 0;
                settled_bad = true;
            } else {
                const int par = sent % CH_NS;
                mail_wait_ge(&s_mail.done_of[par], sent - CH_NS + 1);
                DevTask dt;
                dt.a2 = mb->a2; dt.an = mb->an;
                dt.b2 = try_rev ? mb->b2rc : mb->b2; dt.bn = try_rev ? mb->bnrc : mb->bn;
                dt.a_base = 0; dt.b_base = 0;
                dt.end_a = (int64_t)(end_a < (1ull << 40) ? end_a : (1ull << 40));
                dt.alen = (int32_t)mlen; dt.blen = (int32_t)slen;
                dt.begin_a = (int32_t)begin_a; dt.begin_b = (int32_t)begin_b;
                dt.X = (int32_t)X; dt.band = (int32_t)band;
                dt.flags = call_n ? TF_CALL_N : 0u; dt.res_idx = idx; dt.ops_off = 0; dt.ops_cap = 0;
                Tk t;
                t.cancel = role == 2 ? &sy->cancel : nullptr;
                if constexpr (CE < 0) fill_task<C, -1, true>(dt, p, slots + (u64)par * p.slot_words, lane, false, t);
                else if constexpr (HASN) {
                    if (call_n) fill_task<C, CE, true>(dt, p, slots + (u64)par * p.slot_words, lane, false, t);
                    else fill_task<C, CE, false>(dt, p, slots + (u64)par * p.slot_words, lane, false, t);
                } else fill_task<C, CE, false>(dt, p, slots + (u64)par * p.slot_words, lane, false, t);
                if (lane == 0) { s_mail.tk[par] = t; s_mail.dt[par] = dt; }
                ++sent;
                mail_post(&s_mail.filled, sent, lane);
                mail_wait_ge(&s_mail.early_of[par], sent);
                const u32 fl = (u32)uni(s_mail.e_flags[par]);
                status = fl >> 8;
                if (status == ST_OK) { last_a = (u64)(int64_t)uni(s_mail.e_last_a[par]); last_b = (u64)(int64_t)uni(s_mail.e_last_b[par]); }
                else last_a = last_b = 0;
            }
            ++n_dp;
            if (status == ST_OUT_OF_RANGE || status == 3u) { thrown = true; break; }
        }
        mail_wait_ge(&s_mail.n_done, sent);
        const bool all_good = !settled_bad && uni(s_mail.bad) == 0;
        const u64 sumlen = (u64)uni64((int64_t)s_mail.sum);
        if (cancelled) { state = 1; break; }
        if (overflow) { state = 3; break; }
        if (thrown) { state = 2; break; }
        if (all_good && sumlen >= align_thr) { state = try_rev ? 0x100u : 0u; break; }
        if (++attempt == 2 || role == 1) { state = 1; break; }
        try_rev = !try_rev;
    }
    if (lane == 0) { s_mail.total = sent; s_mail.quit = 1; }
    mail_post(&s_mail.filled, sent + CH_NW, lane);
    __builtin_amdgcn_s_waitcnt(0);
    if (role != 0) {
        const int me = role - 1;
        if (lane == 0) {
            sy->verdict[me] = state; sy->n[me] = n_dp;
            sy->hw[me] = hw_me; sy->t_end[me] = diag_clock(); if (role == 2) sy->t_begin2 = t_begin;
            if (role == 1 && state != 1u) __hip_atomic_store(&sy->cancel, 1u, __ATOMIC_RELAXED, __HIP_MEMORY_SCOPE_AGENT);
        }
        __builtin_amdgcn_s_waitcnt(0);
        u32 before = 0;
        if (lane == 0) before = __hip_atomic_fetch_add(&sy->fin, 1u, __ATOMIC_ACQ_REL, __HIP_MEMORY_SCOPE_AGENT);
        before = (u32)__builtin_amdgcn_readfirstlane((int)before);
        const bool mine = role == 1 ? (state != 1u || before != 0u) : (before != 0u && (u32)uni((int)__hip_atomic_load(&sy->verdict[0], __ATOMIC_RELAXED, __HIP_MEMORY_SCOPE_AGENT)) == 1u);
        if (!mine) {
            if (role == 2 && lane == 0) { cp.host_out[mi].t_begin2 = t_begin; cp.host_out[mi].t_end_att[1] = diag_clock(); }
            return;
        }
        __builtin_amdgcn_fence(__ATOMIC_ACQUIRE, "agent");
        const u32 v0 = (u32)uni((int)sy->verdict[0]), n0 = (u32)uni((int)sy->n[0]), v1 = (u32)uni((int)sy->verdict[1]), n1 = (u32)uni((int)sy->n[1]);
        if (v0 != 1u) { state = v0; n_dp = n0; }
        else { state = v1; n_dp = n1; }
        t_begin = (u32)uni((int)sy->t_begin);
        hw_me = (u32)uni((int)sy->hw[0]); hw_other = (u32)uni((int)sy->hw[1]);
        te0 = (u32)uni((int)sy->t_end[0]); te1 = (u32)uni((int)sy->t_end[1]); tb2 = (u32)uni((int)sy->t_begin2);
    }
    if (lane == 0) { ChainOut o; o.n_dp = n_dp; o.state = state; o.t_begin = t_begin; o.t_end = diag_clock(); o.hw = hw_me; o.hw_twin = hw_other; o.t_end_att[0] = te0; o.t_end_att[1] = te1; o.t_begin2 = tb2; o.pad = 0; cp.out[mi] = o; }
    __builtin_amdgcn_fence(__ATOMIC_ACQUIRE, "agent");
    {
        const u32* src = reinterpret_cast<const u32*>(cp.audit + audit_first);
        u32* dst = reinterpret_cast<u32*>(cp.host_audit + audit_first);
        const u32 nw = n_dp * (u32)(sizeof(DevResult) / sizeof(u32));
        for (u32 w = (u32)lane; w < nw; w += 64) dst[w] = src[w];
        const u32* wsrc = reinterpret_cast<const u32*>(cp.win + audit_first);
        u32* wdst = reinterpret_cast<u32*>(cp.host_win + audit_first);
        const u32 nww = n_dp * (u32)(sizeof(ChainWin) / sizeof(u32));
        for (u32 w = (u32)lane; w < nww; w += 64) wdst[w] = wsrc[w];
        if (lane == 0) { ChainOut o; o.n_dp = n_dp; o.state = state; o.t_begin = t_begin; o.t_end = diag_clock(); o.hw = hw_me; o.hw_twin = hw_other; o.t_end_att[0] = te0; o.t_end_att[1] = te1; o.t_begin2 = tb2; o.pad = 0; cp.host_out[mi] = o; }
    }
    __builtin_amdgcn_s_waitcnt(0);
    __builtin_amdgcn_fence(__ATOMIC_RELEASE, "");
    if (lane == 0) __hip_atomic_store(cp.host_done + mi, cp.epoch, __ATOMIC_RELEASE, __HIP_MEMORY_SCOPE_SYSTEM);
}

template <int C, int CE, bool HASN>
__device__ __forceinline__ void chain_walker(const LaunchParams& p, const int lane)
{
    __builtin_amdgcn_s_setprio(3);
    for (;;) {
        int w = 0;
        if (lane == 0) w = __hip_atomic_fetch_add(&s_mail.claim, 1, __ATOMIC_RELAXED, __HIP_MEMORY_SCOPE_WORKGROUP);
        w = __builtin_amdgcn_readfirstlane(w);
        mail_wait_ge(&s_mail.filled, w + 1);
        if (uni(s_mail.quit) != 0 && w >= uni(s_mail.total)) break;
        const int par = w % CH_NS;
        WalkCarry wc;
        end_cell<C, true>(&s_mail.tk[par], lane, &wc);
        wc.early_seq = w + 1;
        if constexpr (CE < 0) finish_walk<C, -1, true, 64, false, true>(&s_mail.tk[par], &s_mail.dt[par], &p, lane, 0, 0, &wc);
        else if constexpr (HASN) {
            if ((u32)uni((int)s_mail.dt[par].flags) & TF_CALL_N) finish_walk<C, CE, true, 64, false, true>(&s_mail.tk[par], &s_mail.dt[par], &p, lane, 0, 0, &wc);
            else finish_walk<C, CE, false, 64, false, true>(&s_mail.tk[par], &s_mail.dt[par], &p, lane, 0, 0, &wc);
        } else finish_walk<C, CE, false, 64, false, true>(&s_mail.tk[par], &s_mail.dt[par], &p, lane, 0, 0, &wc);
    }
}

template <int C, int CE, bool HASN>
__device__ __forceinline__ void chain_workgroup(const ChainParams& cp)
{
    const int lane = threadIdx.x & 63;
    const int wave = uni((int)(threadIdx.x >> 6));
    const bool twin = blockIdx.x < cp.n_twins;
    const u32 mi = twin ? blockIdx.x : cp.first_mb + blockIdx.x - cp.n_twins;
    const int role = twin ? 2 : (mi < cp.n_twins ? 1 : 0);
    const DevMB* const mbp = unip(cp.mbs + mi);
    u32* slots = cp.scratch + (u64)uni64((int64_t)mbp->slot_off[twin ? 1 : 0]);
    LaunchParams p;
    p.tasks = nullptr; p.n_tasks = 0; p.cursor = nullptr; p.results = cp.audit; p.ops_buf = nullptr;
    p.scratch = cp.scratch; p.slot_words = (u64)uni64((int64_t)mbp->slot_words); p.dir_words = (u64)uni64((int64_t)mbp->dir_words); p.ypad = cp.ypad;
    p.ckpt_off = (u64)uni64((int64_t)mbp->ckpt_off); p.bnd_off = (u64)uni64((int64_t)mbp->bnd_off); p.flags = 0; p.prio_R = 0; p.prio_from = 0; p.stats = nullptr;
    if (threadIdx.x == 0) {
        s_mail.filled = 0; s_mail.quit = 0; s_mail.total = 0; s_mail.claim = 0; s_mail.n_done = 0;
        for (int k = 0; k < CH_NS; ++k) { s_mail.early_of[k] = 0; s_mail.done_of[k] = 0; }
    }
    __syncthreads();
    if constexpr (CE < 0) {
        if (wave == 0) chain_filler<C, -1, true>(cp, p, mi, slots, lane, role);
        else chain_walker<C, -1, true>(p, lane);
    } else {
        const bool mb_n = HASN && uni((int)cp.mbs[mi].has_n) != 0;
        if (wave == 0) {
            if constexpr (HASN) {
                if (mb_n) chain_filler<C, CE, true>(cp, p, mi, slots, lane, role);
                else chain_filler<C, CE, false>(cp, p, mi, slots, lane, role);
            } else chain_filler<C, CE, false>(cp, p, mi, slots, lane, role);
        } else {
            if constexpr (HASN) {
                if (mb_n) chain_walker<C, CE, true>(p, lane);
                else chain_walker<C, CE, false>(p, lane);
            } else chain_walker<C, CE, false>(p, lane);
        }
    }
}

template <bool HASN>
__global__ __launch_bounds__(64 * (1 + CH_NW), GAMDP_WAVES_PER_SIMD) void k_chain2(const ChainParams cp)
{
    chain_workgroup<5, 0, HASN>(cp);
}

template <int C>
__global__ __launch_bounds__(64 * (1 + CH_NW), GAMDP_WAVES_PER_SIMD) void k_chain2g(const ChainParams cp)
{
    static_assert(C == 2 || C == 3 || C == 5 || C == 9 || C == 17, "the column counts of the generic kernels");
    chain_workgroup<C, -1, true>(cp);
}

}

int chain_slots_per_workgroup() { return CH_NS; }

const ChainKernel& chain2_kernel(const bool has_n)
{
    static const ChainKernel with_n = {"k_chain2<true>", (const void*)k_chain2<true>, 5, 64 * (1 + CH_NW), &kernel_info[K_C5_CE0_N], true, CHAIN_N_BY_WINDOW};
    static const ChainKernel without = {"k_chain2<false>", (const void*)k_chain2<false>, 5, 64 * (1 + CH_NW), &kernel_info[K_C5_CE0_N], true, CHAIN_N_BY_WINDOW};
    return has_n ? with_n : without;
}

const KernelFamily& chain_gen_family()
{
    static const KernelFamily f = {
        {(const void*)k_chain2g<2>, (const void*)k_chain2g<3>, (const void*)k_chain2g<5>, (const void*)k_chain2g<9>, (const void*)k_chain2g<17>},
        {"k_chain2g<2>", "k_chain2g<3>", "k_chain2g<5>", "k_chain2g<9>", "k_chain2g<17>"},
        64 * (1 + CH_NW)};
    return f;
}

namespace {
constexpr int W1 = 4 * GAMDP_WAVES_PER_SIMD, W2 = 4 * GAMDP_PAIR_WAVES_PER_SIMD;
constexpr int I17 = IMG_WORDS<17, true>, I19 = IMG_WORDS<19, true>, I9 = IMG_WORDS<9, true>;
constexpr int B1 = (int)Strip<64>::BND_WORDS, BQ = (int)Strip<QL>::BND_WORDS;
constexpr int P17_CK = (int)PairFmt<17, 64>::CK_WORDS, P17_BND = (int)PairFmt<17, 64>::BND_WORDS;
constexpr int O19_CK = (int)PairFmt<19, QL>::CK_WORDS, O19_BND = (int)PairFmt<19, QL>::BND_WORDS;
}
constexpr KernelInfo kernel_info[K_COUNT] = {
    {K_C17_CE4,    "k_align<17,4,false>",    17, 512, 1,      W1, false, true,  false, I17,    I17,    B1,      k_align<17, 4, false>},
    {K_C17_CE4_N,  "k_align<17,4,true>",     17, 512, 1,      W1, true,  true,  false, I17,    I17,    B1,      k_align<17, 4, true>},
    {K_C5_CE0,     "k_align<5,0,false>",      5, 150, 1,      W1, false, false, false, 5 * 64, 5 * 64, B1,      k_align<5, 0, false>},
    {K_C5_CE0_N,   "k_align<5,0,true>",       5, 150, 1,      W1, true,  false, false, 5 * 64, 5 * 64, B1,      k_align<5, 0, true>},
    {K_P17_CE4,    "k_align_p<17,4>",        17, 512, 2,      W2, false, true,  true,  I17,    P17_CK, P17_BND, k_align_p<17, 4>},
    {K_O19_CE15,   "k_align_o<19,15>",       19, 150, 2 * QT, W2, false, true,  true,  I19,    O19_CK, O19_BND, k_align_o<19, 15>},
    {K_Q19_CE15,   "k_align_q<19,15,false>", 19, 150, QT,     W1, false, true,  false, I19,    I19,    BQ,      k_align_q<19, 15, false>},
    {K_Q19_CE15_N, "k_align_q<19,15,true>",  19, 150, QT,     W1, true,  true,  false, I19,    I19,    BQ,      k_align_q<19, 15, true>},
    {K_GEN_C2,     "k_align<2,-1,true>",      2,   0, 1,      W1, true,  false, false, 2 * 64, 2 * 64, B1,      k_align<2, -1, true>},
    {K_GEN_C3,     "k_align<3,-1,true>",      3,   0, 1,      W1, true,  false, false, 3 * 64, 3 * 64, B1,      k_align<3, -1, true>},
    {K_GEN_C5,     "k_align<5,-1,true>",      5,   0, 1,      W1, true,  false, false, 5 * 64, 5 * 64, B1,      k_align<5, -1, true>},
    {K_GEN_C9,     "k_align<9,-1,true>",      9,   0, 1,      W1, true,  true,  false, I9,     I9,     B1,      k_align<9, -1, true>},
    {K_GEN_C17,    "k_align<17,-1,true>",    17,   0, 1,      W1, true,  true,  false, I17,    I17,    B1,      k_align<17, -1, true>},
    {K_WIDE,       "k_align_w",               0,   0, 1,      WIDE_WORKGROUPS_PER_CU, true, false, false, 1, 1, B1, nullptr},
};
static_assert([] { for (int k = 0; k < K_COUNT; k++) if (kernel_info[k].id != k) return false; return true; }(),
              "kernel_info: one row per KernelId, in KernelId order");
static_assert(kernel_info[K_C17_CE4].dirfree == DIRFREE_OK<4, 17, false> && kernel_info[K_C17_CE4_N].dirfree == DIRFREE_OK<4, 17, true> &&
                  kernel_info[K_C5_CE0].dirfree == DIRFREE_OK<0, 5, false> && kernel_info[K_C5_CE0_N].dirfree == DIRFREE_OK<0, 5, true> &&
                  kernel_info[K_P17_CE4].dirfree == DIRFREE_OK<4, 17, false> && kernel_info[K_O19_CE15].dirfree == DIRFREE_OK<15, 19, false> &&
                  kernel_info[K_Q19_CE15].dirfree == DIRFREE_OK<15, 19, false> && kernel_info[K_Q19_CE15_N].dirfree == DIRFREE_OK<15, 19, true> &&
                  kernel_info[K_GEN_C2].dirfree == DIRFREE_OK<-1, 2, true> && kernel_info[K_GEN_C3].dirfree == DIRFREE_OK<-1, 3, true> &&
                  kernel_info[K_GEN_C5].dirfree == DIRFREE_OK<-1, 5, true> && kernel_info[K_GEN_C9].dirfree == DIRFREE_OK<-1, 9, true> &&
                  kernel_info[K_GEN_C17].dirfree == DIRFREE_OK<-1, 17, true>,
              "kernel_info: the dirfree column must agree with DIRFREE_OK");

int launch_align(int kid, const LaunchParams& p, unsigned n_slots, unsigned dyn_lds, void* stream)
{
    if (kid == K_WIDE) return launch_wide(p, n_slots, stream);
    if (kid < 0 || kid >= K_COUNT) return (int)hipErrorInvalidValue;
    const void* f = (const void*)kernel_info[kid].kernel;
    LaunchParams lp = p;
    void* args[] = {&lp};
    return (int)hipLaunchKernel(f, dim3(n_slots), dim3(64), args, dyn_lds, static_cast<hipStream_t>(stream));
}

}
```

gam_ngs_amd/csrc/gamdp_l1.cpp:

```cpp
#include <algorithm>
#include <atomic>
#include <chrono>
#include <cstdio>
#include <cstdlib>
#include <cstring>
#include <mutex>
#include <thread>
#include <new>
#include <string>
#include <unordered_map>
#include <vector>

#include "gamdp.h"
#include "gamdp_internal.h"

namespace gamdp {

void find_hits(const uint8_t* a, u64 alen, u64 a_start, u64 a_end, const uint8_t* b, u64 blen, u64 b_start, u64 b_end,
               u64 word, std::vector<uint32_t>& hits)
{
    hits.clear();
    if (alen == 0 || blen == 0) return;
    if (a_end >= alen) a_end = alen - 1;
    if (b_end >= blen) b_end = blen - 1;
// ... 424 lines not shown
    for (u32 i = 0; i < (u32)M.size(); i++) {
        if (M[i].phase != Machine::MAIN) continue;
        const gamdp_mb_in& in = *M[i].in;
        ChainPick p{i, 0, 1};
        bool empty_frame = false;
        for (u32 k = 0; k < in.n_blocks; k++) {
            const int32_t sl = frame_len(in.blocks[k].s_begin, in.blocks[k].s_end);
            empty_frame = empty_frame || in.blocks[k].s_end < in.blocks[k].s_begin;
            p.rows += (u64)sl;
            p.longest = std::max<u32>(p.longest, (u32)sl);
        }
        if (empty_frame) continue;
        s.ch.push_back(p);
        s.n_blk += in.n_blocks;
        s.has_n = s.has_n || ms->has_n[in.m_id] || ss->has_n[in.s_id];
        s.need_rc.push_back((u32)in.s_id);
    }
    std::stable_sort(s.ch.begin(), s.ch.end(), [](const ChainPick& x, const ChainPick& y) { return x.rows > y.rows; });
    const u64 n_mb = s.ch.size();
    const u64 tw_cap = n_mb < 256 ? std::max<u64>(16, 256 - n_mb) : 256;
    if (!tuning().l1_no_twins)
        while (s.n_tw < n_mb && s.n_tw < tw_cap && s.ch[s.n_tw].rows * 8 >= s.ch[0].rows && s.ch[s.n_tw].rows >= 1024) s.n_tw++;
    return s;
}

struct ChainLayout {
    u64 n_mb, n_audit;
    u64 mb, blk, sync, out, aud, win, total;
    u64 m_out, m_done, m_aud, m_win, m_total;
    ChainLayout(const u64 n_mb_, const u64 n_blk, const u64 n_tw) : n_mb(n_mb_), n_audit(2 * n_blk)
    {
        auto up = [](u64 v) { return (v + 255) & ~255ull; };
        mb = 0; blk = up(mb + n_mb * sizeof(DevMB)); sync = up(blk + n_blk * sizeof(DevBlk)); out = up(sync + (n_tw + 1) * sizeof(ChainSync));
        aud = up(out + n_mb * sizeof(ChainOut)); win = up(aud + n_audit * sizeof(DevResult)); total = up(win + n_audit * sizeof(ChainWin));
        m_out = 0; m_done = up(m_out + n_mb * sizeof(ChainOut)); m_aud = up(m_done + n_mb * sizeof(u32));
        m_win = up(m_aud + n_audit * sizeof(DevResult)); m_total = up(m_win + n_audit * sizeof(ChainWin));
    }
};

int chain_buffers(Ctx* c, const ChainLayout& L, uint8_t*& d_mirror)
{
    int rc_ = grow(c, c->d_chain, c->cap_chain, L.total);
    if (!rc_) rc_ = grow_pinned(c, c->h_chain, c->cap_hchain, L.out, hipHostMallocDefault);
    if (!rc_) rc_ = grow_pinned(c, c->h_mirror, c->cap_mirror, L.m_total, hipHostMallocMapped | hipHostMallocCoherent);
    if (rc_) return rc_;
    if (hipHostGetDevicePointer((void**)&d_mirror, c->h_mirror, 0) != hipSuccess) { c->set_error("hipHostGetDevicePointer failed"); return GAMDP_EHIP; }
    if (!c->chain_stream) {
        int least = 0, greatest = 0;
        if (hipDeviceGetStreamPriorityRange(&least, &greatest) != hipSuccess) { least = 0; (void)hipGetLastError(); }
        if (hipStreamCreateWithPriority(&c->chain_stream, hipStreamNonBlocking, least) != hipSuccess) { c->set_error("hipStreamCreate failed"); return GAMDP_EHIP; }
    }
    std::memset(c->h_mirror + L.m_done, 0, L.n_mb * sizeof(u32));
    if (++c->chain_epoch == 0) c->chain_epoch = 1;
    return 0;
}

void describe_chains(const std::vector<Machine>& M, const ChainSel& sel, const SeqSet* ms, const SeqSet* ss, DevMB* hmb, DevBlk* hbk,
                     std::vector<u32>& q_of)
{
    q_of.assign(M.size(), ~0u);
    u32 blk_at = 0;
    for (size_t q = 0; q < sel.ch.size(); q++) {
        const Machine& m = M[sel.ch[q].mi];
        const gamdp_mb_in& in = *m.in;
        q_of[sel.ch[q].mi] = (u32)q;
        DevMB& x = hmb[q];
        x.a2 = ms->fwd[in.m_id].p2; x.an = ms->fwd[in.m_id].pn;
        x.b2 = ss->fwd[in.s_id].p2; x.bn = ss->fwd[in.s_id].pn;
        x.b2rc = ss->rc[in.s_id].p2; x.bnrc = ss->rc[in.s_id].pn;
        x.mlen = m.mlen; x.slen = m.slen;
        x.m_start = m.m_start; x.s_start = m.s_start; x.s_end = m.s_end;
        x.align_thr = m.align_thr;
        x.first_blk = blk_at; x.n_blocks = in.n_blocks; x.audit_first = 2 * blk_at;
        x.rows = (u32)std::min<u64>(sel.ch[q].rows, 0x7fffffffu);
        x.try_rev = m.try_rev ? 1u : 0u;
        x.has_n = (ms->has_n[in.m_id] || ss->has_n[in.s_id] || diag().force_n) ? 1u : 0u;
        x.npre_a = (size_t)in.m_id < ms->dev_npre.size() ? ms->dev_npre[in.m_id] : nullptr;
        x.npre_b = (size_t)in.s_id < ss->dev_npre.size() ? ss->dev_npre[in.s_id] : nullptr;
        for (u32 k = 0; k < in.n_blocks; k++) {
            const gamdp_block& b = m.blk(k);
            hbk[blk_at + k] = DevBlk{b.m_begin, b.m_end, b.s_begin, b.s_end};
        }
        blk_at += in.n_blocks;
    }
}

struct ChainSlots {
    std::vector<std::pair<u32, u32>> pieces;
    u64 need_scratch = 0, slotw_max = 0, n_tw = 0;
    u32 ypad = 0;
};
bool plan_slots(const ChainSel& sel, DevMB* hmb, const KernelInfo* ki, const u32 band, const u64 arena, ChainSlots& S)
{
    const u64 n_mb = sel.ch.size();
    if (ki == nullptr) {
        for (size_t q = 0; q < n_mb; q++) {
            DevMB& x = hmb[q];
            x.max_x = 0; x.slot_off[0] = x.slot_off[1] = 0; x.slot_words = x.dir_words = x.ckpt_off = x.bnd_off = 0;
        }
        S.pieces.emplace_back(0u, (u32)n_mb);
        return true;
    }
    const u64 per_wg = (u64)chain_slots_per_workgroup();
    const u64 arena_words = arena / sizeof(u32);
    S.n_tw = sel.n_tw;
    u64 words_all = 0, words_twins = 0;
    for (size_t q = 0; q < n_mb; q++) {
        DevMB& x = hmb[q];
        const SlotGeom g = slot_geom(*ki, dir_words_for(*ki, sel.ch[q].longest, band), band);
        S.ypad = g.ypad;
        x.max_x = sel.ch[q].longest;
        x.dir_words = g.dir_words; x.slot_words = g.slot_words;
        x.ckpt_off = g.ckpt_off; x.bnd_off = g.bnd_off;
        S.slotw_max = std::max(S.slotw_max, x.slot_words);
        words_all += per_wg * x.slot_words;
        if (q < S.n_tw) words_twins += per_wg * x.slot_words;
    }
    if (per_wg * S.slotw_max > arena_words) return false;
    if (words_all + words_twins > arena_words) S.n_tw = 0;
    u64 at = 0;
    for (size_t q = 0; q < S.n_tw; q++) { hmb[q].slot_off[1] = at; at += per_wg * hmb[q].slot_words; }
    u32 first = 0;
    for (size_t q = 0; q < n_mb; q++) {
        const u64 mine = per_wg * hmb[q].slot_words;
        if (at + mine > arena_words) {
            S.pieces.emplace_back(first, (u32)q - first);
            S.need_scratch = std::max(S.need_scratch, at);
            first = (u32)q; at = 0;
        }
        hmb[q].slot_off[0] = at;
        if (q >= S.n_tw) hmb[q].slot_off[1] = 0;
        at += mine;
    }
    S.pieces.emplace_back(first, (u32)n_mb - first);
    S.need_scratch = std::max(S.need_scratch, at);
    return true;
}

int enqueue_chains(Ctx* c, const ChainSel& sel, const ChainLayout& L, const ChainSlots& S, uint8_t* const dm, const u32 band,
                   const SeqSet* ms, const SeqSet* ss, const ChainKernel& ck, ChainRun& run)
{
    uint8_t *const h = c->h_chain, *const d = c->d_chain, *const hm = c->h_mirror;
    ChainParams cp;
    cp.mbs = (const DevMB*)(d + L.mb); cp.blks = (const DevBlk*)(d + L.blk); cp.n_mbs = (u32)L.n_mb;
    cp.n_twins = (u32)S.n_tw; cp.sync = (ChainSync*)(d + L.sync);
    std::memset(h + L.sync, 0, (S.n_tw + 1) * sizeof(ChainSync));
    cp.cursor = nullptr; cp.audit = (DevResult*)(d + L.aud); cp.out = (ChainOut*)(d + L.out); cp.win = (ChainWin*)(d + L.win);
    cp.scratch = c->d_chain_scratch; cp.ypad = S.ypad; cp.band = band;
    cp.max_rows = (u32)std::min<u64>(std::max<u64>(1, sel.ch[0].rows), 0x7fffffffu);
    cp.host_out = (ChainOut*)(dm + L.m_out); cp.host_done = (u32*)(dm + L.m_done); cp.host_audit = (DevResult*)(dm + L.m_aud); cp.host_win = (ChainWin*)(dm + L.m_win);
    cp.epoch = c->chain_epoch;
    cp.skew_call = diag().chain_skew;
    cp.n_margin = (int32_t)(64 - diag().n_window_shrink); cp.n_by_contig = diag().force_n ? 1u : 0u;
    run.n_by_contig = cp.n_by_contig != 0;
    run.kernel = ck;
    run.scratch_bytes = S.need_scratch * sizeof(u32); run.n_launches = (u32)S.pieces.size(); run.n_twins = (u32)S.n_tw;
    if (hipEventCreate(&run.e0) != hipSuccess || hipEventCreate(&run.e1) != hipSuccess) { c->set_error("hipEventCreate failed"); return GAMDP_EHIP; }
    if (diag().timing) std::fprintf(stderr, "gamdp chain: %zu merge blocks, %llu blocks, %zu piece(s), %.1f MB of scratch (slots of up to %llu words), %llu twins, has_n %d\n", (size_t)L.n_mb, (unsigned long long)sel.n_blk, S.pieces.size(), S.need_scratch * 4e-6, (unsigned long long)S.slotw_max, (unsigned long long)S.n_tw, (int)sel.has_n);
    run.n_mb = L.n_mb; run.band = band; run.hmb = (const DevMB*)(h + L.mb); run.ms = ms; run.ss = ss;
    run.hout = (const ChainOut*)(hm + L.m_out); run.done = (const volatile u32*)(hm + L.m_done); run.haud = (const DevResult*)(hm + L.m_aud); run.hwin = (const ChainWin*)(hm + L.m_win);
    run.epoch = cp.epoch; run.stream = c->chain_stream; run.dout = cp.out;
    run.t_launch = std::chrono::steady_clock::now();
    bool ok = hipMemcpyAsync(d, h, L.out, hipMemcpyHostToDevice, c->chain_stream) == hipSuccess;
    ok = ok && hipEventRecord(run.e0, c->chain_stream) == hipSuccess;
    for (size_t pc = 0; ok && pc < S.pieces.size(); pc++) {
        cp.first_mb = S.pieces[pc].first;
        ok = launch_kernel(ck.kernel, ck.threads, cp, (unsigned)(S.pieces[pc].second + S.n_tw), c->chain_stream) == 0;
    }
    ok = ok && hipEventRecord(run.e1, c->chain_stream) == hipSuccess;
    if (!ok) {
        (void)hipStreamSynchronize(c->chain_stream);
        c->set_error(std::string("chain launch: ") + hipGetErrorString(hipGetLastError()));
        return GAMDP_EHIP;
    }
    run.launched = true;
    return 0;
}

ChainKernel pick_chain_kernel(const int l1_chain, const int walk_bands, const u32 band, const bool has_n, const bool rounds)
{
    const bool carry = l1_chain == GAMDP_L1_CHAIN_CARRY;
    const bool generic = !carry && band != 150 && walk_bands == GAMDP_L1_WALK_ANY_BAND;
    if (rounds || ((carry || generic) ? band > GAMDP_MAX_TUNED_BAND : band != 150)) return ChainKernel{};
    const int cols = band_cols(band);
    if (carry) return family_chain_kernel(chain_carry_family(), cols, nullptr, false, CHAIN_N_UNREPORTED);
    if (generic) return family_chain_kernel(chain_gen_family(), cols, &kernel_info[gen_kernel_id(cols)], true, CHAIN_N_EVERY_DP);
    return chain2_kernel(has_n);
}

int launch_main_chains(Ctx* c, std::vector<Machine>& M, const SeqSet* ms, const SeqSet* ss, const u32 band, const u64 arena, ChainRun& run)
{
    run.launched = false;
    ChainSel sel = select_chains(M, ms, ss);
    const ChainKernel ck = pick_chain_kernel(c->l1_chain, c->walk_bands, band, sel.has_n || diag().force_n, tuning().l1_rounds);
    if (!ck.kernel || sel.ch.empty()) return 0;
    if (!ck.twins) sel.n_tw = 0;
    int rc_ = ss->ensure_rc(sel.need_rc, c);
    if (rc_) return rc_;
    const ChainLayout L(sel.ch.size(), sel.n_blk, sel.n_tw);
    uint8_t* d_mirror = nullptr;
    if ((rc_ = chain_buffers(c, L, d_mirror))) return rc_;
    DevMB* const hmb = (DevMB*)(c->h_chain + L.mb);
    describe_chains(M, sel, ms, ss, hmb, (DevBlk*)(c->h_chain + L.blk), run.q_of);
    ChainSlots slots;
    if (!plan_slots(sel, hmb, ck.slots, band, arena, slots)) return 0;
    if ((rc_ = grow(c, c->d_chain_scratch, c->cap_chain_scratch, slots.need_scratch, true))) return rc_;
    if ((rc_ = enqueue_chains(c, sel, L, slots, d_mirror, band, ms, ss, ck, run))) return rc_;
    for (const ChainPick& p : sel.ch) M[p.mi].on_device = true;
    return 0;
}

int replay_chain(Ctx* cc, const ChainRun& run, Machine& m, const u32 mi, u64* calls_used)
{
    const u32 q = run.q_of[mi];
    const DevMB& x = run.hmb[q];
    const u32 n_dp = run.hout[q].n_dp;
    *calls_used = 0;
    if ((run.hout[q].state & 0xffu) == 3u) {
        m.on_device = false;
        return 0;
    }
    u32 used = 0;
    auto differs = [&](const char* what, const u64 dev, const u64 host) {
        cc->set_error("internal: merge block " + std::to_string(mi) + ", call " + std::to_string(used) + " of its chain: the device's " + what + " is " +
                      std::to_string(dev) + ", the host's " + std::to_string(host));
        return GAMDP_EHIP;
    };
    while (m.phase == Machine::MAIN) {
        if (used >= n_dp) { cc->set_error("internal: the device's chain of merge block " + std::to_string(mi) + " is shorter than the host's"); return GAMDP_EHIP; }
        ITask t;
        m.pending(t);
        u64 X = 0, cells = 0;
        const int st = preflight(m.mlen, m.slen, run.band, t.begin_a, t.end_a, t.begin_b, t.end_b, false, false, &X, &cells);
        const ChainWin& w = run.hwin[x.audit_first + used];
        const DevResult& rec = run.haud[x.audit_first + used];
        if (w.begin_a != t.begin_a) return differs("begin_a", w.begin_a, t.begin_a);
        if (w.end_a != t.end_a) return differs("end_a", w.end_a, t.end_a);
        if (w.begin_b != t.begin_b) return differs("begin_b", w.begin_b, t.begin_b);
        if (w.end_b != t.end_b) return differs("end_b", w.end_b, t.end_b);
        if ((w.info & 1u) != (t.b_rc ? 1u : 0u)) return differs("orientation", w.info & 1u, t.b_rc ? 1u : 0u);
        if ((w.info >> 8) != (u32)st) return differs("pre-check status", w.info >> 8, (u64)st);
        if (w.X != (u32)X) return differs("row count", w.X, X);
        if (run.kernel.n_bit != CHAIN_N_UNREPORTED) {
            const bool want_n = run.kernel.n_bit == CHAIN_N_EVERY_DP ? st == GAMDP_ST_OK : st == GAMDP_ST_OK && x.has_n != 0 &&
                                (run.n_by_contig || run.ms->window_has_n(t.a_id, false, 0, (int64_t)t.begin_a - (int64_t)run.band - 64, (int64_t)t.begin_a + (int64_t)X - 1 + (int64_t)run.band + 64) ||
                                 run.ss->window_has_n(t.b_id, t.b_rc, 0, (int64_t)t.begin_b - 64, (int64_t)t.begin_b + (int64_t)X - 1 + 64));
            if (((w.info >> 1) & 1u) != (want_n ? 1u : 0u)) return differs("choice of the N-aware cell", (w.info >> 1) & 1u, want_n ? 1u : 0u);
        }
        if (st != GAMDP_ST_OK && (rec.flags >> 8) != (u32)st) return differs("record status", rec.flags >> 8, (u64)st);
        gamdp_result r;
        fill_result(rec, cells, r);
        m.feed(r);
        used++;
    }
    if (used != n_dp) { cc->set_error("internal: the device's chain of merge block " + std::to_string(mi) + " is longer than the host's"); return GAMDP_EHIP; }
    *calls_used = used;
    return 0;
}

struct CohortStats {
    int rounds = 0; double pending_ms = 0, align_ms = 0, feed_ms = 0; int rc = 0;
    gamdp_l1_hits_stats hits{};
    std::vector<gamdp_l1_tail_call> tails;
    u64 chains = 0, chain_calls = 0;
};

inline auto now() { return std::chrono::steady_clock::now(); }
template <class T> double msec(T a, T b) { return std::chrono::duration<double, std::milli>(b - a).count(); }

enum class Wait { NOTHING, AGAIN, FAILED };
Wait wait_for_chain(Ctx* c, const ChainRun& run, const std::vector<u32>& waiting, bool& drained)
{
    if (waiting.empty()) return Wait::NOTHING;
    if (drained) { c->set_error("internal: the chain launch ended without handing over merge block " + std::to_string(waiting[0])); return Wait::FAILED; }
    const hipError_t qs = hipStreamQuery(run.stream);
    if (qs == hipSuccess) { drained = true; return Wait::AGAIN; }
    if (qs != hipErrorNotReady) { c->set_error(std::string("chain kernel: ") + hipGetErrorString(qs)); return Wait::FAILED; }
    if (diag().timing && diag().build && std::chrono::duration<double>(now() - run.t_launch).count() > 5.0) {
        run.dump(stderr);
        std::_Exit(3);
    }
    for (int spin = 0; spin < 256; spin++) {
        bool any = false;
        for (u32 i : waiting) any = any || run.done[run.q_of[i]] == run.epoch;
        if (any) break;
        std::this_thread::yield();
    }
    return Wait::AGAIN;
}

struct TailQuery { u32 mi; Machine::Phase side; u32 task; HitsReq req; };
struct Seed { u64 n_hits; u32 first, last; int source; };
inline Seed seed_of(const std::vector<uint32_t>& hits, const int source)
{
    return Seed{hits.size(), hits.empty() ? 0 : hits.front(), hits.empty() ? 0 : hits.back(), source};
}

int answer_tails(Ctx* c, const std::vector<Machine>& M, const std::vector<TailQuery>& tq, const bool device_hits, RcCache& rc_cache,
                 gamdp_l1_hits_stats& hs, std::vector<Seed>& seeds)
{
    std::vector<uint32_t> hits;
    auto on_host = [&](const TailQuery& q, const int source) {
        const auto h0 = now();
        M[q.mi].host_tail_hits(q.side, q.req, rc_cache, hits);
        hs.host_hits_ms += msec(h0, now());
        return seed_of(hits, source);
// ... 368 lines not shown
```

gam_ngs_amd/csrc/kernel_finish.inc:

```

constexpr int CH_NW = 2, CH_NS = CH_NW + 1;
struct ChainMail {
    int filled, quit, total;
    int claim;
    int n_done;
    int early_of[CH_NS], done_of[CH_NS];
    int e_flags[CH_NS], e_last_a[CH_NS], e_last_b[CH_NS];
    int bad;
    unsigned long long sum;
    Tk tk[CH_NS];
    DevTask dt[CH_NS];
};
__shared__ ChainMail s_mail;
__device__ __forceinline__ int mail_load(int* p) { return __builtin_amdgcn_readfirstlane(__hip_atomic_load(p, __ATOMIC_ACQUIRE, __HIP_MEMORY_SCOPE_WORKGROUP)); }
__device__ __forceinline__ void mail_wait_ge(int* p, const int v) { while (mail_load(p) < v) __builtin_amdgcn_s_sleep(1); }
__device__ __forceinline__ void mail_post(int* p, const int v, const int lane)
{
    __builtin_amdgcn_s_waitcnt(0);
    if (lane == 0) __hip_atomic_store(p, v, __ATOMIC_RELEASE, __HIP_MEMORY_SCOPE_WORKGROUP);
}

struct WalkCarry {
    int early_seq;
    int status;
    int best;
    int x, y, pos, end_pos, end_x;
    u32 len, nm;
    int la, lb, fa, fb, have;
    int mat_q, mat_lo, mat_hi, old_q, old_lo, old_hi, mat_calls;
    int need_q, need_ghi;
    int mat_ticks;
};

template <int C, bool WG2 = false>
__device__ __noinline__ void end_cell(const Tk* tp, const int lane, WalkCarry* wc)
{
    const Tk t = load_uniform(tp);
    const int X = t.X, Y = t.Y, w = t.band;
    if constexpr (!WG2) __syncthreads();
    __builtin_amdgcn_fence(__ATOMIC_ACQUIRE, "agent");

    int best = NEG, bkey = 0x7fffffff;
    {
        const giptr lr = (X == 1) ? t.h0row : t.lastrow;
        if (!t.fe) {
            for (int j = lane; j < Y; j += 64) {
                const int64_t pos = (int64_t)t.begin_a + (X - 1) + j - w;
                if (pos >= 0 && pos <= t.end_a) {
                    const int v = (pos < t.alen) ? lr[j] : 0;
                    if (v > best || (v == best && j < bkey)) { best = v; bkey = j; }
                }
            }
        }
        const bool ge = t.end_a >= (int64_t)t.begin_a + w;
        const int64_t jA64 = ge ? (int64_t)2 * w : (int64_t)2 * w - ((int64_t)t.begin_a + w - t.end_a);
        if (jA64 >= 0 && t.iA < X) {
            const int jA = (int)jA64;
            const int cnt = min(X - t.iA, jA + 1);
            for (int k = lane; k < cnt; k += 64) {
                const int i = t.iA + k, j = jA - k;
                bool ok = true;
                if (t.fe) ok = (X >= FORCE_MAXGAP + 1) && (i >= X - 1 - FORCE_MAXGAP);
                if (ok) {
                    int v = 0;
                    if (t.end_a < t.alen) v = (i == 0) ? t.h0row[j] : ((i == X - 1) ? lr[j] : t.adh[k]);
                    const int key = Y + k;
                    if (v > best || (v == best && key < bkey)) { best = v; bkey = key; }
                }
            }
        }
#pragma unroll
        for (int o = 32; o >= 1; o >>= 1) {
            const int ov = __shfl_xor(best, o, 64), ok = __shfl_xor(bkey, o, 64);
            if (ov > best || (ov == best && ok < bkey)) { best = ov; bkey = ok; }
        }
    }
    best = __builtin_amdgcn_readfirstlane(best);
    bkey = __builtin_amdgcn_readfirstlane(bkey);
    WalkCarry r;
    r.early_seq = 0;
    r.status = 0; r.best = best;
    r.x = r.y = r.pos = r.end_pos = r.end_x = 0;
    r.len = r.nm = 0;
    r.la = r.lb = r.fa = r.fb = r.have = 0;
    r.mat_q = -1; r.mat_lo = 0; r.mat_hi = -1; r.old_q = -1; r.old_lo = 0; r.old_hi = -1; r.mat_calls = 0; r.mat_ticks = 0;
    r.need_q = 0; r.need_ghi = 0;
    if (bkey != 0x7fffffff) {
        int x, y;
        if (bkey < Y) { x = X - 1; y = bkey; }
        else {
            const bool ge = t.end_a >= (int64_t)t.begin_a + w;
            const int jA = ge ? 2 * w : (int)((int64_t)2 * w - ((int64_t)t.begin_a + w - t.end_a));
            x = t.iA + (bkey - Y);
            y = jA - (bkey - Y);
        }
        const int64_t pos64 = (int64_t)t.begin_a + x + y - w;
        if (pos64 >= t.alen) r.status = 1;
        else { r.status = 2; r.x = x; r.y = y; r.pos = (int)pos64; r.end_pos = (int)pos64; r.end_x = x; }
    }
    *wc = r;
}

template <int C, int CE, bool HASN, int LPT = 64, bool PK = false, bool EARLY = false>
__device__ __noinline__ void finish_walk(const Tk* tp, const DevTask* dtp_, const LaunchParams* pp, const int lane, const int lane_base_, const int pk_half_, WalkCarry* wcp)
{
    const int lane_base = (LPT == 64) ? 0 : uni(lane_base_);
    const int pk_half = PK ? uni(pk_half_) : 0;
    typedef Strip<LPT, PK> ST;
    const Tk t = load_uniform(tp);
    const DevTask* dtp = unip(dtp_);
    const u32 dt_flags = (u32)uni((int)dtp->flags) & TF_LIVE_MASK, dt_res_idx = (u32)uni((int)dtp->res_idx);
    const u64 dt_ops_off = (u64)uni64((int64_t)dtp->ops_off), dt_ops_cap = (u64)uni64((int64_t)dtp->ops_cap);
    uint8_t* const p_ops_buf = unip(pp->ops_buf);
    DevResult* const p_results = unip(pp->results);
    const int Y = t.Y;
    const int wc_status = uni(wcp->status), best = uni(wcp->best);

    DevResult res;
    res.begin_a = res.begin_b = res.score = 0;
    res.n_match = res.length = 0;
    res.first_a = res.first_b = res.last_a = res.last_b = 0;
    res.flags = ST_EMPTY << 8;
    bool posted = false;
    const int early_seq = EARLY ? uni(wcp->early_seq) : 0;
    auto post_early = [&](const u32 flags, const int a, const int b) {
        if constexpr (EARLY) {
            if (!posted) {
                posted = true;
                const int sl = (early_seq - 1) % CH_NS;
                if (lane == 0) { s_mail.e_flags[sl] = (int)flags; s_mail.e_last_a[sl] = a; s_mail.e_last_b[sl] = b; }
                mail_post(&s_mail.early_of[sl], early_seq, lane);
            }
        }
    };
    if (wc_status != 0) {
        if (wc_status == 1) {
            res.flags = ST_OUT_OF_RANGE << 8;
        } else {
            int x = uni(wcp->x), y = uni(wcp->y), pos = uni(wcp->pos);
            const int end_pos = uni(wcp->end_pos), end_x = uni(wcp->end_x);
            const bool want_ops = dt_flags & TF_WANT_OPS;
            uint8_t* ops = p_ops_buf + dt_ops_off;
            u32 len = (u32)uni((int)wcp->len), nm = (u32)uni((int)wcp->nm);
            const int have0 = uni(wcp->have);
            bool have_last = have0 & 2, have_first = have0 & 1;
            int la = uni(wcp->la), lb = uni(wcp->lb), fa = uni(wcp->fa), fb = uni(wcp->fb);
            int l = y / C, c = y - l * C;
            constexpr int TB_DEPTH = 16;
            int cblk0 = -1, cl = -1, cg = -1;
            u32 cw = 0;
            int64_t sa_w0 = INT64_MIN, sb_w0 = INT64_MIN, san_w0 = INT64_MIN, sbn_w0 = INT64_MIN;
            u32 sa_v = 0, sb_v = 0, san_v = 0, sbn_v = 0;
            int mat_q = uni(wcp->mat_q), mat_lo = uni(wcp->mat_lo), mat_hi = uni(wcp->mat_hi), mat_calls = uni(wcp->mat_calls);
            int old_q = uni(wcp->old_q), old_lo = uni(wcp->old_lo), old_hi = uni(wcp->old_hi);
            long long mat_ticks = 0;
            int dg_iters = 0, dg_refills = 0;
            const long long walk_t0 = (dt_flags & TF_DIAG_COUNT_MAT) ? wall_clock64() : 0;
            int cvalid_lo = 0;
            auto get_word = [&](const int blk, const int l_, const int c_) -> u32 {
                const int g = c_ >> 2;
                int k = cblk0 - blk;
                if (l_ != cl || g != cg || k < 0 || k >= TB_DEPTH || blk < cvalid_lo) {
                    cvalid_lo = 0;
                    dg_refills++;
                    if constexpr (DIRFREE_OK<CE, C, HASN>) {
                        if (blk >= t.df_hi) {
                            cvalid_lo = t.df_hi;
                        } else if (blk >= t.df_lo) {
                            if (ST::strip_of(lane_base + l_, t.sshift) == old_q && blk >= old_lo && blk <= old_hi) {
                                const int tq = mat_q, tl = mat_lo, th = mat_hi;
                                mat_q = old_q; mat_lo = old_lo; mat_hi = old_hi;
                                old_q = tq; old_lo = tl; old_hi = th;
                            } else if (!(ST::strip_of(lane_base + l_, t.sshift) == mat_q && blk >= mat_lo && blk <= mat_hi)) {
                                const int g_hi = blk >> 2;
                                const long long tm0 = (dt_flags & TF_DIAG_COUNT_MAT) ? wall_clock64() : 0;
                                materialise_auto<C, (DIRFREE_OK<CE, C, HASN> ? CE : 0), HASN, LPT, PK>(tp, ST::strip_of(lane_base + l_, t.sshift), g_hi, lane, pk_half, lane_base);
                                if (dt_flags & TF_DIAG_COUNT_MAT) mat_ticks += wall_clock64() - tm0;
                                __builtin_amdgcn_s_waitcnt(0);
                                __builtin_amdgcn_fence(__ATOMIC_ACQUIRE, "agent");
                                old_q = mat_q; old_lo = mat_lo; old_hi = mat_hi;
                                mat_q = ST::strip_of(lane_base + l_, t.sshift); mat_hi = 4 * g_hi + 3; mat_lo = max(4 * (g_hi - (ST::groups_of(mat_q) - 1)), t.df_lo);
                                mat_calls++;
                            }
                            cvalid_lo = (mat_lo == t.df_lo) ? 0 : mat_lo;
                        }
                    }
                    cblk0 = blk; cl = l_; cg = g; k = 0;
                    const int myblk = max(blk - (lane >> 2), 0);
                    const int myc = min(4 * g + (lane & 3), C - 1);
                    cw = t.dir[dir_index<C, DIRFREE_OK<CE, C, HASN>>(myblk, lane_base + l_, myc)];
                }
                return (u32)__builtin_amdgcn_readlane((int)cw, __builtin_amdgcn_readfirstlane(4 * k + (c_ & 3)));
            };
            if (dt_flags & TF_DIAG_SKIP_TRACEBACK) {
                if constexpr (DIRFREE_OK<CE, C, HASN>) {
                    if (dt_flags & TF_DIAG_COUNT_MAT)
                        for (int g_hi = (t.df_hi >> 2) - 1; g_hi >= (t.df_lo >> 2); g_hi -= ST::groups_of(ST::strip_of(lane_base + (Y / 2) / C, t.sshift)))
                            materialise_auto<C, (DIRFREE_OK<CE, C, HASN> ? CE : 0), HASN, LPT, PK>(tp, ST::strip_of(lane_base + (Y / 2) / C, t.sshift), g_hi, lane, pk_half, lane_base);
                }
                x = -1;
            }
            int walk_it = 0;
            while (x >= 0 && y >= 0 && pos >= 0) {
                if constexpr (EARLY) {
                    walk_it = uni(walk_it) + 1;
                    if ((walk_it & 31) == 0 && cancelled(t.cancel)) break;
                }
                x = uni(x); y = uni(y); pos = uni(pos); l = uni(l); c = uni(c);
#ifdef GAMDP_DIAG_COUNTERS
                dg_iters = uni(dg_iters) + 1; dg_refills = uni(dg_refills); mat_calls = uni(mat_calls);
#endif
                cblk0 = uni(cblk0); cl = uni(cl); cg = uni(cg);
                mat_q = uni(mat_q); mat_lo = uni(mat_lo); mat_hi = uni(mat_hi); cvalid_lo = uni(cvalid_lo);
                old_q = uni(old_q); old_lo = uni(old_lo); old_hi = uni(old_hi);
                sa_w0 = uni64(sa_w0); sb_w0 = uni64(sb_w0);
                if (HASN) { san_w0 = uni64(san_w0); sbn_w0 = uni64(sbn_w0); }
                if (x == 0 || pos == 0 || want_ops) {
                    const int pa = HASN ? code_at(t.a2, t.an, t.a_base + pos) : (int)((t.a2[(t.a_base + pos) >> 4] >> (((t.a_base + pos) & 15) * 2)) & 3);
                    const int64_t bi = t.b_base + t.begin_b + x;
                    const int pb = HASN ? code_at(t.b2, t.bn, bi) : (int)((t.b2[bi >> 4] >> ((bi & 15) * 2)) & 3);
                    const bool is_match = (pa == pb) || pa == 4 || pb == 4;
                    int op;
                    if (pos == 0) {
                        const int s = score_of(pa, pb);
                        const int h = (x == 0) ? t.h0row[y] : t.pos0[x];
                        const bool left_ok = !(t.fs && x > FORCE_MAXGAP);
                        if (h == s) op = 2;
                        else if (y == Y - 1 || (left_ok && h == GAP)) op = 1;
                        else op = 0;
                    } else if (x == 0) {
                        const int s = score_of(pa, pb);
                        const int h = t.h0row[y];
                        const bool up_ok = !(t.fs && pos > FORCE_MAXGAP);
                        if (h == s) op = 2;
                        else if (y < Y - 1 && y > 0 && up_ok && h == GAP) op = 0;
                        else if (y < Y - 1 && y > 0) op = 1;
                        else if (y < Y - 1) op = 0;
                        else op = 1;
                    } else {
                        const int tau = x + l, blk = tau >> 4;
                        const u32 cw = get_word(blk, l, c);
                        const u32 tag = (cw >> ((tau & 15) * 2)) & 3u;
                        op = (tag == 2u) ? 2 : (tag == 1u ? 0 : 1);
                    }
                    if (op == 2) {
                        if (is_match) {
                            nm++;
                            if (!have_last) { have_last = true; la = pos; lb = t.begin_b + x; post_early((ST_OK << 8) | 2u, la, lb); }
                            have_first = true; fa = pos; fb = t.begin_b + x;
                        }
                        if (want_ops && len < dt_ops_cap) ops[len] = is_match ? 2 : 3;
                        x--; pos--;
                    } else if (op == 1) {
                        if (want_ops && len < dt_ops_cap) ops[len] = 1;
                        y--; pos--;
                        if (--c < 0) { c = C - 1; l--; }
                    } else {
                        if (want_ops && len < dt_ops_cap) ops[len] = 0;
                        x--; y++;
                        if (++c == C) { c = 0; l++; }
                    }
                    len++;
                } else {
                    const int tau = x + l, blk = tau >> 4, r = tau & 15;
                    const u32 w_here = get_word(blk, l, c);
                    const int k0 = cblk0 - blk, e = c & 3;
                    const int myk = lane >> 2;
                    const bool mine = ((lane & 3) == e) && myk >= k0 && (cblk0 - myk) >= max(cvalid_lo, 0);
                    u32 T = cw ^ 0xAAAAAAAAu;
                    if (myk == k0) T <<= (30 - 2 * r);
                    const int avail = T ? (__builtin_clz(T) >> 1) : ((myk == k0) ? r + 1 : 16);
                    const u64 m_mine = __ballot(mine), m_stop = __ballot(mine && T != 0u);
                    int n, Ls = -1;
                    if (m_stop == 0) {
                        n = (r + 1) + 16 * (((63 - __builtin_clzll(m_mine)) >> 2) - k0);
                    } else {
                        Ls = __builtin_ctzll(m_stop);
                        const int ks = Ls >> 2;
                        const int lead = __builtin_amdgcn_readlane(avail, Ls);
                        n = (ks == k0) ? lead : (r + 1) + 16 * (ks - k0 - 1) + lead;
                    }
                    const int n_run = n;
                    n = min(n, min(x, pos));
                    if (n > 0) {
                        const int64_t ia_hi = t.a_base + pos, ib_hi = t.b_base + t.begin_b + x;
                        const int64_t wa = (ia_hi - 15) >> 4, wb = (ib_hi - 15) >> 4;
                        const int64_t wa_bot = (ia_hi - n - 15) >> 4, wb_bot = (ib_hi - n - 15) >> 4;
                        if (wa + 1 > sa_w0 || wa_bot < sa_w0 - 63) { sa_w0 = wa + 1; sa_v = t.a2[sa_w0 - lane]; }
                        if (wb + 1 > sb_w0 || wb_bot < sb_w0 - 63) { sb_w0 = wb + 1; sb_v = t.b2[sb_w0 - lane]; }
                        const int da = (int)(sa_w0 - wa), db = (int)(sb_w0 - wb);
                        const u32 a16 = __builtin_amdgcn_alignbit((u32)wave_shr1(0, (int)sa_v), sa_v, (u32)((ia_hi - 15) & 15) * 2u);
                        const u32 b16s = __builtin_amdgcn_alignbit((u32)wave_shr1(0, (int)sb_v), sb_v, (u32)((ib_hi - 15) & 15) * 2u);
                        const u32 b16 = (u32)__builtin_amdgcn_ds_bpermute(4 * (lane + db - da), (int)b16s);
                        const int j = lane - da;
                        const u32 xr = a16 ^ b16;
                        u32 ne = (xr | (xr >> 1)) & 0x55555555u;
                        if constexpr (HASN) {
                            const int64_t na_lo = ia_hi - 15 - 16 * (int64_t)j, nb_lo = ib_hi - 15 - 16 * (int64_t)j;
                            const int64_t wna = (ia_hi >> 5) + 1, wnb = (ib_hi >> 5) + 1;
                            const int64_t wna_bot = (ia_hi - n - 31) >> 5, wnb_bot = (ib_hi - n - 31) >> 5;
                            if (wna > san_w0 || wna_bot < san_w0 - 63) { san_w0 = wna; san_v = t.an[san_w0 - lane]; }
                            if (wnb > sbn_w0 || wnb_bot < sbn_w0 - 63) { sbn_w0 = wnb; sbn_v = t.bn[sbn_w0 - lane]; }
                            auto nbits = [&](const u32 win, const int64_t w0, const int64_t lo) -> u32 {
                                const int src = (int)(w0 - (lo >> 5));
                                const u32 wl = (u32)__builtin_amdgcn_ds_bpermute(4 * src, (int)win);
                                const u32 wh = (u32)__builtin_amdgcn_ds_bpermute(4 * (src - 1), (int)win);
                                return __builtin_amdgcn_alignbit(wh, wl, (u32)(lo & 31)) & 0xFFFFu;
                            };
                            u32 nn = nbits(san_v, san_w0, na_lo) | nbits(sbn_v, sbn_w0, nb_lo);
                            nn = (nn | (nn << 8)) & 0x00FF00FFu;
                            nn = (nn | (nn << 4)) & 0x0F0F0F0Fu;
                            nn = (nn | (nn << 2)) & 0x33333333u;
                            nn = (nn | (nn << 1)) & 0x55555555u;
                            ne &= ~nn;
                        }
                        const int p0 = 16 * j + 16 - n;
                        u32 msk = (p0 <= 0) ? 0x55555555u : ((p0 >= 16) ? 0u : (0x55555555u << (2 * p0)));
                        if (j < 0) msk = 0u;
                        u32 eq = ~ne & msk;
                        const u64 m_eq = __ballot(eq != 0u);
                        if (m_eq) {
                            int cnt = __builtin_popcount(eq);
                            cnt += __builtin_amdgcn_update_dpp(0, cnt, 0xB1, 0xf, 0xf, true);
                            cnt += __builtin_amdgcn_update_dpp(0, cnt, 0x4E, 0xf, 0xf, true);
                            cnt += __builtin_amdgcn_update_dpp(0, cnt, 0x141, 0xf, 0xf, true);
                            cnt += __builtin_amdgcn_update_dpp(0, cnt, 0x140, 0xf, 0xf, true);
                            nm += (u32)(__builtin_amdgcn_readlane(cnt, 0) + __builtin_amdgcn_readlane(cnt, 16) +
                                        __builtin_amdgcn_readlane(cnt, 32) + __builtin_amdgcn_readlane(cnt, 48));
                            const int Ltop = __builtin_ctzll(m_eq), Lbot = 63 - __builtin_clzll(m_eq);
                            const u32 eq_top = (u32)__builtin_amdgcn_readlane((int)eq, Ltop), eq_bot = (u32)__builtin_amdgcn_readlane((int)eq, Lbot);
                            const int off_hi = 16 * (Ltop - da) + 15 - ((31 - __builtin_clz(eq_top)) >> 1);
                            const int off_lo = 16 * (Lbot - da) + 15 - (__builtin_ctz(eq_bot) >> 1);
                            if (!have_last) { have_last = true; la = pos - off_hi; lb = t.begin_b + x - off_hi; post_early((ST_OK << 8) | 2u, la, lb); }
                            have_first = true; fa = pos - off_lo; fb = t.begin_b + x - off_lo;
                        }
                        x -= n; pos -= n; len += (u32)n;
                        if (Ls >= 0 && n == n_run && x >= 1 && pos >= 1) {
                            const u32 w2 = (u32)__builtin_amdgcn_readlane((int)cw, Ls);
                            const u32 tag2 = (w2 >> (((x + l) & 15) * 2)) & 3u;
                            if (tag2 == 1u) {
                                x--; y++;
                                if (++c == C) { c = 0; l++; }
                            } else {
                                y--; pos--;
                                if (--c < 0) { c = C - 1; l--; }
                            }
                            len++;
                        }
                    } else {
                        const u32 tag = (w_here >> (r * 2)) & 3u;
                        if (tag == 1u) {
                            x--; y++;
                            if (++c == C) { c = 0; l++; }
                        } else {
                            y--; pos--;
                            if (--c < 0) { c = C - 1; l--; }
                        }
                        len++;
                    }
                }
            }
            res.begin_a = pos + 1;
            res.begin_b = t.begin_b + x + 1;
            res.score = best;
            res.n_match = nm;
            res.length = len;
            res.first_a = have_first ? fa : end_pos + 1;
            res.first_b = have_first ? fb : t.begin_b + end_x + 1;
            res.last_a = have_last ? la : res.begin_a;
            res.last_b = have_last ? lb : res.begin_b;
            res.flags = (have_first ? 1u : 0u) | (have_last ? 2u : 0u) | (ST_OK << 8);
            if (pp->stats != nullptr && lane == 0 && mat_calls > 0) atomicAdd(unip(pp->stats) + LS_STRIPS, (u32)mat_calls);
            if (dt_flags & TF_DIAG_COUNT_MAT) {
                res.n_match = (u32)mat_calls;
                res.first_a = (int)mat_ticks + uni(wcp->mat_ticks);
                res.first_b = (int)(wall_clock64() - walk_t0);
                res.last_a = dg_iters; res.last_b = dg_refills;
            }
        }
    }
#ifdef GAMDP_DIAG
    if (uni(t.pos0[-1]) != 0) res.flags = ST_DIAG_RANGE << 8;
#endif
    if (lane == 0) p_results[dt_res_idx] = res;
    if constexpr (EARLY) {
        post_early(res.flags, res.last_a, res.last_b);
        const u32 status = res.flags >> 8;
        if (lane == 0) {
            if (status == ST_OK) {
                if (res.length == 0 || (u64)res.n_match * 100u < 95ull * (u64)res.length) atomicOr(&s_mail.bad, 1);
                atomicAdd(&s_mail.sum, (unsigned long long)res.length);
            } else atomicOr(&s_mail.bad, 1);
        }
        mail_post(&s_mail.done_of[(early_seq - 1) % CH_NS], early_seq, lane);
        if (lane == 0) __hip_atomic_fetch_add(&s_mail.n_done, 1, __ATOMIC_RELEASE, __HIP_MEMORY_SCOPE_WORKGROUP);
    } else __syncthreads();
}

template <int C, int CE, bool HASN, int LPT = 64, bool PK = false>
__device__ __forceinline__ void finish_task(const Tk* tp, const DevTask* dtp, const LaunchParams* pp, const int lane, const int lane_base = 0, const int pk_half = 0)
{
    WalkCarry wc;
    end_cell<C>(tp, lane, &wc);
    finish_walk<C, CE, HASN, LPT, PK>(tp, dtp, pp, lane, lane_base, pk_half, &wc);
}
```

gam_ngs_amd/lib.py:

```python
import ctypes as C
import os

HERE = os.path.dirname(os.path.abspath(__file__))

SYMBOLS = [
    "gamdp_ctx_create", "gamdp_ctx_destroy", "gamdp_ctx_set_arena_bytes", "gamdp_last_error", "gamdp_ctx_stream",
    "gamdp_ctx_kernel_time", "gamdp_ctx_launch_info", "gamdp_seqset_create", "gamdp_seqset_destroy", "gamdp_seqset_size",
    "gamdp_seqset_length", "gamdp_align_batch", "gamdp_align_merge_blocks", "gamdp_find_hits", "gamdp_encode",
    "gamdp_decode", "gamdp_revcomp", "gamdp_synth_pair", "gamdp_seqset_create_synth", "gamdp_seqset_create_synth_strided",
    "gamdp_fasta_open", "gamdp_fasta_close", "gamdp_fasta_count", "gamdp_fasta_name", "gamdp_fasta_codes",
    "gamdp_seqset_create_from_fasta",
    "gamdp_fasta_create", "gamdp_merge_lists_prepare", "gamdp_zscore_vote", "gamdp_pctgs_create", "gamdp_pctgs_destroy",
    "gamdp_pctgs_last_error", "gamdp_pctgs_add_graph", "gamdp_pctgs_finish", "gamdp_pctgs_count",
    "gamdp_pctgs_merged_count", "gamdp_pctgs_codes", "gamdp_pctgs_rows", "gamdp_pctgs_contig_use",
    "gamdp_pctgs_write_fasta", "gamdp_pctgs_write_descriptors",
    "gamdp_task_preflight", "gamdp_build_info", "gamdp_ctx_l1_stats",
    "gamdp_multi_create", "gamdp_multi_destroy", "gamdp_multi_size", "gamdp_multi_ctx", "gamdp_multi_last_error",
    "gamdp_multi_seqset_create", "gamdp_multi_seqset_create_from_fasta", "gamdp_multi_seqset_destroy",
    "gamdp_multi_seqset_on", "gamdp_multi_align_batch", "gamdp_multi_align_merge_blocks", "gamdp_partition_lpt",
    "gamdp_blocks_open", "gamdp_blocks_close", "gamdp_blocks_count", "gamdp_blocks_data", "gamdp_blocks_write",
    "gamdp_no_blocks_contigs", "gamdp_no_blocks_after_filter", "gamdp_pctgs_not_merged", "gamdp_fasta_write_selected",
    "gamdp_find_hits_batch", "gamdp_ctx_set_l1_hits", "gamdp_ctx_l1_hits_stats",
    "gamdp_ctx_l1_tail_calls", "gamdp_score_batch", "gamdp_ctx_score_info", "gamdp_carry_batch", "gamdp_ctx_carry_info",
    "gamdp_ctx_set_l1_chain", "gamdp_ctx_l1_chain_stats", "gamdp_ctx_set_l1_walk_bands",
    "gamdp_ctx_set_walk_skip", "gamdp_ctx_walk_skip_stats",
]

EINVAL, ENODEV, ENOMEM, ENOTSUP, EHIP = -1, -2, -3, -4, -5
ST_OK, ST_EMPTY, ST_OUT_OF_RANGE, ST_INVALID = 0, 1, 2, 3
L1_HITS_HOST, L1_HITS_DEVICE = 0, 1
L1_CHAIN_WALK, L1_CHAIN_CARRY = 0, 1
L1_WALK_BAND_150, L1_WALK_ANY_BAND = 0, 1
WALK_STRIPS, WALK_SKIP_DIAG = 0, 1
ST_DIAG_RANGE = 9


class GamdpError(RuntimeError):
    pass


class Task(C.Structure):
    _fields_ = [("a_id", C.c_uint32), ("b_id", C.c_uint32), ("a_off", C.c_uint64), ("b_off", C.c_uint64),
                ("a_rc", C.c_uint8), ("b_rc", C.c_uint8), ("force_start", C.c_uint8), ("force_end", C.c_uint8),
                ("band", C.c_uint32), ("begin_a", C.c_uint64), ("end_a", C.c_uint64), ("begin_b", C.c_uint64),
                ("end_b", C.c_uint64)]


class Result(C.Structure):
    _fields_ = [("begin_a", C.c_uint64), ("begin_b", C.c_uint64), ("score", C.c_int64), ("n_match", C.c_uint64),
                ("length", C.c_uint64), ("first_a", C.c_uint64), ("first_b", C.c_uint64), ("last_a", C.c_uint64),
                ("last_b", C.c_uint64), ("cells", C.c_uint64), ("homology", C.c_double),
                ("first_found", C.c_uint8), ("last_found", C.c_uint8), ("status", C.c_uint8), ("pad_", C.c_uint8 * 5)]

    def key(self):
        return (self.status, self.begin_a, self.begin_b, self.score, self.n_match, self.length, self.first_a,
                self.first_b, self.first_found, self.last_a, self.last_b, self.last_found, self.homology)


class ScoreResult(C.Structure):
    _fields_ = [("score", C.c_int64), ("end_a", C.c_uint64), ("end_b", C.c_uint64), ("cells", C.c_uint64),
                ("status", C.c_uint8), ("pad_", C.c_uint8 * 7)]


class ScoreLaunchInfo(C.Structure):
    _fields_ = [("kernel", C.c_char * 24), ("cols", C.c_uint32), ("tasks", C.c_uint32), ("slots", C.c_uint32),
                ("band_max", C.c_uint32), ("kernel_ms", C.c_double)]

    def as_dict(self):
        d = {k: getattr(self, k) for k, _ in self._fields_}
        d["kernel"] = d["kernel"].decode()
        return d


class HitsTask(C.Structure):
    _fields_ = [("a_id", C.c_uint32), ("b_id", C.c_uint32), ("a_off", C.c_uint64), ("b_off", C.c_uint64),
                ("a_rc", C.c_uint8), ("b_rc", C.c_uint8), ("pad_", C.c_uint8 * 2), ("word", C.c_uint32),
                ("a_start", C.c_uint64), ("a_end", C.c_uint64), ("b_start", C.c_uint64), ("b_end", C.c_uint64)]


class HitsResult(C.Structure):
    _fields_ = [("n_hits", C.c_uint64), ("votes", C.c_uint64), ("first", C.c_uint32), ("last", C.c_uint32),
                ("status", C.c_uint8), ("pad_", C.c_uint8 * 7)]


class Ops(C.Structure):
    _fields_ = [("ops_buf", C.c_void_p), ("ops_off", C.POINTER(C.c_uint64)), ("ops_cap", C.POINTER(C.c_uint64))]


class BlockC(C.Structure):
    _fields_ = [("m_begin", C.c_int32), ("m_end", C.c_int32), ("s_begin", C.c_int32), ("s_end", C.c_int32),
                ("m_strand", C.c_char), ("s_strand", C.c_char), ("n_reads", C.c_int64)]


class MbIn(C.Structure):
    _fields_ = [("m_id", C.c_int32), ("s_id", C.c_int32), ("m_ltail", C.c_uint8), ("m_rtail", C.c_uint8),
                ("s_ltail", C.c_uint8), ("s_rtail", C.c_uint8), ("n_blocks", C.c_uint32),
                ("blocks", C.POINTER(BlockC))]


class MbOut(C.Structure):
    _fields_ = [("align_ok", C.c_uint8), ("align_rev", C.c_uint8), ("status", C.c_uint8), ("coords_set", C.c_uint8),
                ("m_start", C.c_int32), ("m_end", C.c_int32), ("s_start", C.c_int32), ("s_end", C.c_int32),
                ("n_dp", C.c_uint32), ("cells", C.c_uint64)]


class L1Stats(C.Structure):
    _fields_ = [("merge_blocks", C.c_uint64), ("dp_calls", C.c_uint64), ("cells", C.c_uint64), ("rounds", C.c_uint32),
                ("cohorts", C.c_uint32), ("launches", C.c_uint32), ("pad_", C.c_uint32), ("wall_ms", C.c_double),
                ("gpu_busy_ms", C.c_double), ("kernel_sum_ms", C.c_double), ("host_pending_ms", C.c_double),
                ("host_feed_ms", C.c_double)]


class L1HitsStats(C.Structure):
    _fields_ = [("tail_queries", C.c_uint64), ("device_queries", C.c_uint64), ("trivial_queries", C.c_uint64),
                ("host_fallback", C.c_uint64), ("host_queries", C.c_uint64), ("hits_launches", C.c_uint32), ("mode", C.c_uint32),
                ("hits_kernel_ms", C.c_double), ("host_hits_ms", C.c_double)]

    def as_dict(self):
        return {k: getattr(self, k) for k, _ in self._fields_}


class L1ChainStats(C.Structure):
    _fields_ = [("chains", C.c_uint64), ("chain_calls", C.c_uint64), ("round_loop_mbs", C.c_uint64), ("scratch_bytes", C.c_uint64),
                ("mode", C.c_uint32), ("launches", C.c_uint32), ("twins", C.c_uint32), ("cols", C.c_uint32),
                ("kernel", C.c_char * 24), ("chain_ms", C.c_double)]

    def as_dict(self):
        d = {k: getattr(self, k) for k, _ in self._fields_}
        d["kernel"] = d["kernel"].decode()
        return d


class WalkSkipStats(C.Structure):
    _fields_ = [("tests", C.c_uint64), ("groups_tested", C.c_uint64), ("groups_skipped", C.c_uint64), ("rows_skipped", C.c_uint64),
                ("strips", C.c_uint64), ("mode", C.c_uint32), ("pad_", C.c_uint32)]

    def as_dict(self):
        return {k: getattr(self, k) for k, _ in self._fields_ if k != "pad_"}


class L1TailCall(C.Structure):
    _fields_ = [("begin_a", C.c_uint64), ("merge_block", C.c_uint32), ("right", C.c_uint8), ("source", C.c_uint8),
                ("pad_", C.c_uint8 * 2)]


class LaunchInfo(C.Structure):
    _fields_ = [("kernel", C.c_char * 40), ("n_aware", C.c_uint32), ("tasks_per_wavefront", C.c_uint32), ("tasks", C.c_uint32),
                ("units", C.c_uint32), ("slots", C.c_uint32), ("band_max", C.c_uint32), ("units_dirfree", C.c_uint32),
                ("units_packed_top", C.c_uint32), ("units_packed_top_mixed", C.c_uint32), ("strips", C.c_uint32),
                ("piece", C.c_uint32), ("units_top_wanted", C.c_uint32), ("rounds", C.c_double), ("kernel_ms", C.c_double)]

    def as_dict(self):
        d = {k: getattr(self, k) for k, _ in self._fields_ if k != "pad_"}
        d["kernel"] = d["kernel"].decode()
        return d


class MBlock(C.Structure):
    _fields_ = [("m_id", C.c_int32), ("m_start", C.c_int32), ("m_end", C.c_int32), ("s_id", C.c_int32),
                ("s_start", C.c_int32), ("s_end", C.c_int32), ("align_rev", C.c_uint8), ("align_ok", C.c_uint8),
                ("m_ltail", C.c_uint8), ("m_rtail", C.c_uint8), ("s_ltail", C.c_uint8), ("s_rtail", C.c_uint8),
                ("ext_slave_next", C.c_uint8), ("ext_slave_prev", C.c_uint8), ("m_rev", C.c_uint8),
                ("s_rev", C.c_uint8), ("pad_", C.c_uint8 * 2)]


class PctgRow(C.Structure):
    _fields_ = [("start", C.c_int64), ("end", C.c_int64), ("ctg_id", C.c_int32), ("reversed", C.c_uint8),
                ("is_master", C.c_uint8), ("pad_", C.c_uint8 * 2)]


class BlockRec(C.Structure):
    _fields_ = [("n_reads", C.c_int64), ("m_block_reads_len", C.c_uint64), ("m_reads_len", C.c_uint64),
                ("s_block_reads_len", C.c_uint64), ("s_reads_len", C.c_uint64), ("m_ctg", C.c_int32),
                ("m_begin", C.c_int32), ("m_end", C.c_int32), ("s_ctg", C.c_int32), ("s_begin", C.c_int32),
                ("s_end", C.c_int32), ("m_strand", C.c_char), ("s_strand", C.c_char), ("pad_", C.c_uint8 * 6)]

    KEYS = ("n_reads", "m_ctg", "m_strand", "m_begin", "m_end", "m_block_reads_len", "m_reads_len",
            "s_ctg", "s_strand", "s_begin", "s_end", "s_block_reads_len", "s_reads_len")

    def as_dict(self):
        d = {k: getattr(self, k) for k in self.KEYS}
        d["m_strand"], d["s_strand"] = d["m_strand"].decode("latin1"), d["s_strand"].decode("latin1")
        return d


REGION_VOTE_FN = C.CFUNCTYPE(C.c_int, C.c_void_p, C.c_int32, C.c_int32, C.c_int32, C.c_int32, C.c_int32, C.c_int32)

_lib = None


def library_path():
    return os.environ.get("GAMDP_LIB") or os.path.join(HERE, "libgamdp.so")


def load_library():
    global _lib
    if _lib is not None:
        return _lib
    path = library_path()
    if not os.path.exists(path):
        raise GamdpError("%s is missing: build it with `make -C gam_ngs_amd/csrc` "
                         "(or __graft_entry__.build()); there is no CPU fallback" % path)
    lib = C.CDLL(path)
    u64, u32, vp = C.c_uint64, C.c_uint32, C.c_void_p
    lib.gamdp_ctx_create.argtypes = [C.c_int, C.POINTER(vp)]
    lib.gamdp_ctx_create.restype = C.c_int
    lib.gamdp_ctx_destroy.argtypes = [vp]
    lib.gamdp_ctx_destroy.restype = None
    lib.gamdp_ctx_set_arena_bytes.argtypes = [vp, u64]
    lib.gamdp_last_error.argtypes = [vp]
    lib.gamdp_last_error.restype = C.c_char_p
    lib.gamdp_ctx_stream.argtypes = [vp]
    lib.gamdp_ctx_stream.restype = vp
    lib.gamdp_ctx_kernel_time.argtypes = [vp, C.POINTER(C.c_double), C.POINTER(u64), C.c_int]
    lib.gamdp_ctx_launch_info.argtypes = [vp, C.POINTER(LaunchInfo), C.c_size_t, C.POINTER(C.c_size_t)]
    lib.gamdp_seqset_create.argtypes = [vp, C.POINTER(C.c_char_p), C.POINTER(u64), u32, C.c_int, C.POINTER(vp)]
    lib.gamdp_seqset_destroy.argtypes = [vp]
    lib.gamdp_seqset_destroy.restype = None
    lib.gamdp_seqset_size.argtypes = [vp]
    lib.gamdp_seqset_size.restype = u32
    lib.gamdp_seqset_length.argtypes = [vp, u32]
    lib.gamdp_seqset_length.restype = u64
    lib.gamdp_align_batch.argtypes = [vp, vp, vp, C.POINTER(Task), C.c_size_t, C.POINTER(Result), C.POINTER(Ops)]
    lib.gamdp_align_merge_blocks.argtypes = [vp, vp, vp, C.POINTER(MbIn), C.c_size_t, u32, C.POINTER(MbOut),
                                             C.POINTER(Result), u32]
    lib.gamdp_score_batch.argtypes = [vp, vp, vp, C.POINTER(Task), C.c_size_t, C.POINTER(ScoreResult)]
    lib.gamdp_score_batch.restype = C.c_int
    lib.gamdp_ctx_score_info.argtypes = [vp, C.POINTER(ScoreLaunchInfo), C.c_size_t, C.POINTER(C.c_size_t)]
    lib.gamdp_ctx_score_info.restype = C.c_int
    lib.gamdp_carry_batch.argtypes = [vp, vp, vp, C.POINTER(Task), C.c_size_t, C.POINTER(Result)]
    lib.gamdp_carry_batch.restype = C.c_int
    lib.gamdp_ctx_carry_info.argtypes = [vp, C.POINTER(ScoreLaunchInfo), C.c_size_t, C.POINTER(C.c_size_t)]
    lib.gamdp_ctx_carry_info.restype = C.c_int
    lib.gamdp_task_preflight.argtypes = [u64, u64, u32, u64, u64, u64, u64, C.c_int, C.c_int, C.POINTER(u64)]
    lib.gamdp_ctx_l1_stats.argtypes = [vp, C.POINTER(L1Stats)]
    lib.gamdp_ctx_set_l1_hits.argtypes = [vp, C.c_int]
    lib.gamdp_ctx_set_l1_hits.restype = C.c_int
    lib.gamdp_ctx_set_l1_chain.argtypes = [vp, C.c_int]
    lib.gamdp_ctx_set_l1_chain.restype = C.c_int
    lib.gamdp_ctx_set_l1_walk_bands.argtypes = [vp, C.c_int]
    lib.gamdp_ctx_set_l1_walk_bands.restype = C.c_int
    lib.gamdp_ctx_l1_chain_stats.argtypes = [vp, C.POINTER(L1ChainStats)]
    lib.gamdp_ctx_l1_chain_stats.restype = C.c_int
    if hasattr(lib, "gamdp_ctx_set_walk_skip"):
        lib.gamdp_ctx_set_walk_skip.argtypes = [vp, C.c_int]
        lib.gamdp_ctx_set_walk_skip.restype = C.c_int
        lib.gamdp_ctx_walk_skip_stats.argtypes = [vp, C.POINTER(WalkSkipStats)]
        lib.gamdp_ctx_walk_skip_stats.restype = C.c_int
    lib.gamdp_ctx_l1_hits_stats.argtypes = [vp, C.POINTER(L1HitsStats)]
    lib.gamdp_ctx_l1_hits_stats.restype = C.c_int
    lib.gamdp_ctx_l1_tail_calls.argtypes = [vp, C.POINTER(L1TailCall), C.c_size_t, C.POINTER(C.c_size_t)]
    lib.gamdp_ctx_l1_tail_calls.restype = C.c_int
    lib.gamdp_build_info.argtypes = []
    lib.gamdp_build_info.restype = C.c_uint
    lib.gamdp_multi_create.argtypes = [C.POINTER(C.c_int), C.c_int, C.POINTER(vp)]
    lib.gamdp_multi_destroy.argtypes = [vp]
    lib.gamdp_multi_destroy.restype = None
    lib.gamdp_multi_size.argtypes = [vp]
    lib.gamdp_multi_ctx.argtypes = [vp, C.c_int]
    lib.gamdp_multi_ctx.restype = vp
    lib.gamdp_multi_last_error.argtypes = [vp]
    lib.gamdp_multi_last_error.restype = C.c_char_p
    lib.gamdp_multi_seqset_create.argtypes = [vp, C.POINTER(C.c_char_p), C.POINTER(u64), u32, C.c_int, C.POINTER(vp)]
    lib.gamdp_multi_seqset_create_from_fasta.argtypes = [vp, vp, C.POINTER(vp)]
    lib.gamdp_multi_seqset_destroy.argtypes = [vp]
    lib.gamdp_multi_seqset_destroy.restype = None
    lib.gamdp_multi_seqset_on.argtypes = [vp, C.c_int]
    lib.gamdp_multi_seqset_on.restype = vp
    lib.gamdp_multi_align_batch.argtypes = [vp, vp, vp, C.POINTER(Task), C.c_size_t, C.POINTER(Result)]
    lib.gamdp_multi_align_merge_blocks.argtypes = [vp, vp, vp, C.POINTER(MbIn), C.c_size_t, u32, C.POINTER(MbOut),
                                                   C.POINTER(Result), u32]
    lib.gamdp_partition_lpt.argtypes = [C.POINTER(u64), C.c_size_t, C.c_int, C.POINTER(u32)]
    lib.gamdp_find_hits.argtypes = [C.c_char_p, u64, u64, u64, C.c_char_p, u64, u64, u64, u64, vp, u64]
    lib.gamdp_find_hits.restype = C.c_int64
    lib.gamdp_find_hits_batch.argtypes = [vp, vp, vp, C.POINTER(HitsTask), C.c_size_t, C.POINTER(HitsResult), C.POINTER(u32),
                                          C.POINTER(u64), C.POINTER(u64)]
    lib.gamdp_find_hits_batch.restype = C.c_int
    lib.gamdp_encode.argtypes = [C.c_char_p, u64, vp]
    lib.gamdp_encode.restype = None
    lib.gamdp_decode.argtypes = [vp, u64, vp]
    lib.gamdp_decode.restype = None
    lib.gamdp_revcomp.argtypes = [vp, u64]
    lib.gamdp_revcomp.restype = None
    lib.gamdp_synth_pair.argtypes = [u64, u64, vp, vp]
    lib.gamdp_synth_pair.restype = u64
    lib.gamdp_seqset_create_synth.argtypes = [vp, u64, u32, u64, C.POINTER(vp)]
    lib.gamdp_seqset_create_synth_strided.argtypes = [vp, u64, u64, u32, u64, C.POINTER(vp)]
    lib.gamdp_fasta_open.argtypes = [C.c_char_p, C.POINTER(vp)]
    lib.gamdp_fasta_close.argtypes = [vp]
    lib.gamdp_fasta_close.restype = None
    lib.gamdp_fasta_count.argtypes = [vp]
    lib.gamdp_fasta_count.restype = u32
    lib.gamdp_fasta_name.argtypes = [vp, u32]
    lib.gamdp_fasta_name.restype = C.c_char_p
    lib.gamdp_fasta_codes.argtypes = [vp, u32, C.POINTER(u64)]
    lib.gamdp_fasta_codes.restype = C.POINTER(C.c_uint8)
    lib.gamdp_seqset_create_from_fasta.argtypes = [vp, vp, C.POINTER(vp)]
    lib.gamdp_fasta_create.argtypes = [C.POINTER(C.c_char_p), C.POINTER(C.c_char_p), C.POINTER(u64), u32, C.c_int,
                                       C.POINTER(vp)]
    lib.gamdp_merge_lists_prepare.argtypes = [vp, vp, C.POINTER(MBlock), C.POINTER(u32), u32, C.c_uint,
                                              C.POINTER(MBlock), u64, C.POINTER(u32), u32, C.POINTER(u32)]
    lib.gamdp_zscore_vote.argtypes = [C.POINTER(C.c_double), C.POINTER(C.c_double), C.c_size_t]
    lib.gamdp_pctgs_create.argtypes = [vp, vp, C.POINTER(vp)]
    lib.gamdp_pctgs_destroy.argtypes = [vp]
    lib.gamdp_pctgs_destroy.restype = None
    lib.gamdp_pctgs_last_error.argtypes = [vp]
    lib.gamdp_pctgs_last_error.restype = C.c_char_p
    lib.gamdp_pctgs_add_graph.argtypes = [vp, C.POINTER(MBlock), C.POINTER(u32), u32, REGION_VOTE_FN, vp]
    lib.gamdp_pctgs_finish.argtypes = [vp]
    lib.gamdp_pctgs_count.argtypes = [vp]
    lib.gamdp_pctgs_count.restype = u32
    lib.gamdp_pctgs_merged_count.argtypes = [vp]
    lib.gamdp_pctgs_merged_count.restype = u32
    lib.gamdp_pctgs_codes.argtypes = [vp, u32, C.POINTER(u64)]
    lib.gamdp_pctgs_codes.restype = C.POINTER(C.c_uint8)
    lib.gamdp_pctgs_rows.argtypes = [vp, u32, C.POINTER(PctgRow), u32]
    lib.gamdp_pctgs_rows.restype = u32
    lib.gamdp_pctgs_contig_use.argtypes = [vp, vp, vp]
    lib.gamdp_pctgs_write_fasta.argtypes = [vp, C.c_char_p]
    lib.gamdp_pctgs_write_descriptors.argtypes = [vp, C.c_char_p]
    lib.gamdp_blocks_open.argtypes = [C.c_char_p, C.c_int64, C.POINTER(vp)]
    lib.gamdp_blocks_close.argtypes = [vp]
    lib.gamdp_blocks_close.restype = None
    lib.gamdp_blocks_count.argtypes = [vp]
    lib.gamdp_blocks_count.restype = u64
    lib.gamdp_blocks_data.argtypes = [vp]
    lib.gamdp_blocks_data.restype = C.POINTER(BlockRec)
    lib.gamdp_blocks_write.argtypes = [C.c_char_p, C.POINTER(BlockRec), u64]
    lib.gamdp_no_blocks_contigs.argtypes = [C.POINTER(BlockRec), u64, u32, u32, vp, vp]
    lib.gamdp_no_blocks_after_filter.argtypes = [C.POINTER(BlockRec), u64, u32, u32, vp, vp, vp, vp]
    lib.gamdp_pctgs_not_merged.argtypes = [vp, vp, vp, vp]
    lib.gamdp_fasta_write_selected.argtypes = [vp, vp, C.c_char_p]
    _lib = lib
    return lib
```

include/gamdp.h:

```cpp
#ifndef GAMDP_H
#define GAMDP_H

#include <stddef.h>
#include <stdint.h>

#ifdef __cplusplus
extern "C" {
#endif

#define GAMDP_VERSION 1

#define GAMDP_EINVAL  (-1)
#define GAMDP_ENODEV  (-2)
#define GAMDP_ENOMEM  (-3)
#define GAMDP_ENOTSUP (-4)
#define GAMDP_EHIP    (-5)

#define GAMDP_ST_OK           0
#define GAMDP_ST_EMPTY        1
#define GAMDP_ST_OUT_OF_RANGE 2
#define GAMDP_ST_INVALID      3
#define GAMDP_ST_DIAG_RANGE   9

#define GAMDP_OP_GAP_A 0
#define GAMDP_OP_GAP_B 1
#define GAMDP_OP_MATCH 2
#define GAMDP_OP_MISMATCH 3

#define GAMDP_DEFAULT_BAND 150
#define GAMDP_MAX_BAND 1048576
#define GAMDP_MAX_TUNED_BAND 543

typedef struct gamdp_ctx gamdp_ctx;
typedef struct gamdp_seqset gamdp_seqset;
typedef struct gamdp_fasta gamdp_fasta;

typedef struct gamdp_task {
    uint32_t a_id, b_id;
    uint64_t a_off, b_off;
    uint8_t a_rc, b_rc, force_start, force_end;
    uint32_t band;
    uint64_t begin_a, end_a, begin_b, end_b;
} gamdp_task;

typedef struct gamdp_result {
    uint64_t begin_a, begin_b;
    int64_t score;
    uint64_t n_match, length;
    uint64_t first_a, first_b;
    uint64_t last_a, last_b;
    uint64_t cells;
    double homology;
    uint8_t first_found, last_found;
    uint8_t status;
    uint8_t pad_[5];
} gamdp_result;

typedef struct gamdp_ops {
    uint8_t* ops_buf;
    const uint64_t* ops_off;
    const uint64_t* ops_cap;
} gamdp_ops;

typedef struct gamdp_block {
    int32_t m_begin, m_end, s_begin, s_end;
    char m_strand, s_strand;
    int64_t n_reads;
} gamdp_block;

typedef struct gamdp_mb_in {
    int32_t m_id, s_id;
    uint8_t m_ltail, m_rtail, s_ltail, s_rtail;
    uint32_t n_blocks;
    const gamdp_block* blocks;
} gamdp_mb_in;

typedef struct gamdp_mb_out {
    uint8_t align_ok, align_rev;
    uint8_t status;
    uint8_t coords_set;
    int32_t m_start, m_end, s_start, s_end;
    uint32_t n_dp;
    uint64_t cells;
} gamdp_mb_out;

int gamdp_ctx_create(int device, gamdp_ctx** out);
void gamdp_ctx_destroy(gamdp_ctx* ctx);
int gamdp_ctx_set_arena_bytes(gamdp_ctx* ctx, uint64_t bytes);
const char* gamdp_last_error(const gamdp_ctx* ctx);
void* gamdp_ctx_stream(gamdp_ctx* ctx);
int gamdp_ctx_kernel_time(gamdp_ctx* ctx, double* total_ms, uint64_t* launches, int reset);
typedef struct gamdp_launch_info {
    char kernel[40];
    uint32_t n_aware;
    uint32_t tasks_per_wavefront;
    uint32_t tasks;
    uint32_t units;
    uint32_t slots;
    uint32_t band_max;
    uint32_t units_dirfree;
    uint32_t units_packed_top;
    uint32_t units_packed_top_mixed;
    uint32_t strips;
    uint32_t piece;
    uint32_t units_top_wanted;
    double rounds;
    double kernel_ms;
} gamdp_launch_info;
int gamdp_ctx_launch_info(const gamdp_ctx* ctx, gamdp_launch_info* out, size_t cap, size_t* n);

#define GAMDP_WALK_STRIPS     0
#define GAMDP_WALK_SKIP_DIAG  1
int gamdp_ctx_set_walk_skip(gamdp_ctx* ctx, int mode);
typedef struct gamdp_walk_skip_stats {
    uint64_t tests;
    uint64_t groups_tested;
    uint64_t groups_skipped;
    uint64_t rows_skipped;
    uint64_t strips;
    uint32_t mode;
    uint32_t pad_;
} gamdp_walk_skip_stats;
int gamdp_ctx_walk_skip_stats(const gamdp_ctx* ctx, gamdp_walk_skip_stats* out);

int gamdp_seqset_create(gamdp_ctx* ctx, const uint8_t* const* seqs, const uint64_t* lens, uint32_t n,
                        int is_ascii, gamdp_seqset** out);
void gamdp_seqset_destroy(gamdp_seqset* set);
uint32_t gamdp_seqset_size(const gamdp_seqset* set);
uint64_t gamdp_seqset_length(const gamdp_seqset* set, uint32_t id);

int gamdp_fasta_open(const char* path, gamdp_fasta** out);
void gamdp_fasta_close(gamdp_fasta* f);
uint32_t gamdp_fasta_count(const gamdp_fasta* f);
const char* gamdp_fasta_name(const gamdp_fasta* f, uint32_t i);
const uint8_t* gamdp_fasta_codes(const gamdp_fasta* f, uint32_t i, uint64_t* len);
int gamdp_seqset_create_from_fasta(gamdp_ctx* ctx, const gamdp_fasta* f, gamdp_seqset** out);

typedef struct gamdp_block_rec {
    int64_t n_reads;
    uint64_t m_block_reads_len, m_reads_len, s_block_reads_len, s_reads_len;
    int32_t m_ctg, m_begin, m_end, s_ctg, s_begin, s_end;
    char m_strand, s_strand;
    uint8_t pad_[6];
} gamdp_block_rec;
typedef struct gamdp_blocks gamdp_blocks;
int gamdp_blocks_open(const char* path, int64_t min_block_size, gamdp_blocks** out);
void gamdp_blocks_close(gamdp_blocks* b);
uint64_t gamdp_blocks_count(const gamdp_blocks* b);
const gamdp_block_rec* gamdp_blocks_data(const gamdp_blocks* b);
int gamdp_blocks_write(const char* path, const gamdp_block_rec* recs, uint64_t n);

int gamdp_align_batch(gamdp_ctx* ctx, const gamdp_seqset* set_a, const gamdp_seqset* set_b,
                      const gamdp_task* tasks, size_t n, gamdp_result* out, const gamdp_ops* ops_or_null);

int gamdp_task_preflight(uint64_t alen, uint64_t blen, uint32_t band, uint64_t begin_a, uint64_t end_a, uint64_t begin_b,
                         uint64_t end_b, int force_start, int force_end, uint64_t* cells);

typedef struct gamdp_score_result {
    int64_t score;
    uint64_t end_a, end_b;
    uint64_t cells;
    uint8_t status;
    uint8_t pad_[7];
} gamdp_score_result;
int gamdp_score_batch(gamdp_ctx* ctx, const gamdp_seqset* set_a, const gamdp_seqset* set_b,
                      const gamdp_task* tasks, size_t n, gamdp_score_result* out);
typedef struct gamdp_score_launch_info {
    char kernel[24];
    uint32_t cols;
    uint32_t tasks;
    uint32_t slots;
    uint32_t band_max;
    double kernel_ms;
} gamdp_score_launch_info;
int gamdp_ctx_score_info(const gamdp_ctx* ctx, gamdp_score_launch_info* out, size_t cap, size_t* n);

int gamdp_carry_batch(gamdp_ctx* ctx, const gamdp_seqset* set_a, const gamdp_seqset* set_b,
                      const gamdp_task* tasks, size_t n, gamdp_result* out);
int gamdp_ctx_carry_info(const gamdp_ctx* ctx, gamdp_score_launch_info* out, size_t cap, size_t* n);

unsigned gamdp_build_info(void);

int gamdp_align_merge_blocks(gamdp_ctx* ctx, const gamdp_seqset* master, const gamdp_seqset* slave,
                             const gamdp_mb_in* in, size_t n, uint32_t band, gamdp_mb_out* out,
                             gamdp_result* audit, uint32_t audit_stride);

typedef struct gamdp_l1_stats {
    uint64_t merge_blocks, dp_calls, cells;
    uint32_t rounds;
    uint32_t cohorts;
    uint32_t launches;
    uint32_t pad_;
    double wall_ms;
    double gpu_busy_ms;
    double kernel_sum_ms;
    double host_pending_ms;
    double host_feed_ms;
} gamdp_l1_stats;
int gamdp_ctx_l1_stats(const gamdp_ctx* ctx, gamdp_l1_stats* out);

#define GAMDP_L1_HITS_HOST   0
#define GAMDP_L1_HITS_DEVICE 1
int gamdp_ctx_set_l1_hits(gamdp_ctx* ctx, int mode);
typedef struct gamdp_l1_hits_stats {
    uint64_t tail_queries;
    uint64_t device_queries;
    uint64_t trivial_queries;
    uint64_t host_fallback;
    uint64_t host_queries;
    uint32_t hits_launches;
    uint32_t mode;
    double hits_kernel_ms;
    double host_hits_ms;
} gamdp_l1_hits_stats;
int gamdp_ctx_l1_hits_stats(const gamdp_ctx* ctx, gamdp_l1_hits_stats* out);
#define GAMDP_L1_SEED_HOST     0
#define GAMDP_L1_SEED_DEVICE   1
#define GAMDP_L1_SEED_TRIVIAL  2
#define GAMDP_L1_SEED_FALLBACK 3
typedef struct gamdp_l1_tail_call {
    uint64_t begin_a;
    uint32_t merge_block;
    uint8_t right;
    uint8_t source;
    uint8_t pad_[2];
} gamdp_l1_tail_call;
int gamdp_ctx_l1_tail_calls(const gamdp_ctx* ctx, gamdp_l1_tail_call* out, size_t cap, size_t* n);

#define GAMDP_L1_CHAIN_WALK  0
#define GAMDP_L1_CHAIN_CARRY 1
int gamdp_ctx_set_l1_chain(gamdp_ctx* ctx, int mode);
#define GAMDP_L1_WALK_BAND_150 0
#define GAMDP_L1_WALK_ANY_BAND 1
int gamdp_ctx_set_l1_walk_bands(gamdp_ctx* ctx, int which);
typedef struct gamdp_l1_chain_stats {
    uint64_t chains;
    uint64_t chain_calls;
    uint64_t round_loop_mbs;
    uint64_t scratch_bytes;
    uint32_t mode;
    uint32_t launches;
    uint32_t twins;
    uint32_t cols;
    char kernel[24];
    double chain_ms;
} gamdp_l1_chain_stats;
int gamdp_ctx_l1_chain_stats(const gamdp_ctx* ctx, gamdp_l1_chain_stats* out);

typedef struct gamdp_multi gamdp_multi;
typedef struct gamdp_multi_seqset gamdp_multi_seqset;
int gamdp_multi_create(const int* devices, int n, gamdp_multi** out);
void gamdp_multi_destroy(gamdp_multi* m);
int gamdp_multi_size(const gamdp_multi* m);
gamdp_ctx* gamdp_multi_ctx(gamdp_multi* m, int i);
const char* gamdp_multi_last_error(const gamdp_multi* m);
int gamdp_multi_seqset_create(gamdp_multi* m, const uint8_t* const* seqs, const uint64_t* lens, uint32_t n, int is_ascii,
                              gamdp_multi_seqset** out);
int gamdp_multi_seqset_create_from_fasta(gamdp_multi* m, const gamdp_fasta* f, gamdp_multi_seqset** out);
void gamdp_multi_seqset_destroy(gamdp_multi_seqset* s);
gamdp_seqset* gamdp_multi_seqset_on(gamdp_multi_seqset* s, int i);
int gamdp_multi_align_batch(gamdp_multi* m, const gamdp_multi_seqset* set_a, const gamdp_multi_seqset* set_b,
                            const gamdp_task* tasks, size_t n, gamdp_result* out);
int gamdp_multi_align_merge_blocks(gamdp_multi* m, const gamdp_multi_seqset* master, const gamdp_multi_seqset* slave,
                                   const gamdp_mb_in* in, size_t n, uint32_t band, gamdp_mb_out* out, gamdp_result* audit,
                                   uint32_t audit_stride);
int gamdp_partition_lpt(const uint64_t* weights, size_t n, int parts, uint32_t* part_of);

int64_t gamdp_find_hits(const uint8_t* a, uint64_t alen, uint64_t a_start, uint64_t a_end,
                        const uint8_t* b, uint64_t blen, uint64_t b_start, uint64_t b_end,
                        uint64_t word, uint32_t* hits, uint64_t cap);

typedef struct gamdp_hits_task {
    uint32_t a_id, b_id;
    uint64_t a_off, b_off;
    uint8_t a_rc, b_rc, pad_[2];
    uint32_t word;
// ... 86 lines not shown
```

integration/gamdp_stub.c:

```c
#include "gamdp.h"

int gamdp_multi_create(const int* devices, int n, gamdp_multi** out) { (void)devices; (void)n; if (out) *out = 0; return GAMDP_ENODEV; }
void gamdp_multi_destroy(gamdp_multi* m) { (void)m; }
const char* gamdp_multi_last_error(const gamdp_multi* m) { (void)m; return "gamdp stub library: no GPU implementation on this host"; }
int gamdp_multi_seqset_create(gamdp_multi* m, const uint8_t* const* seqs, const uint64_t* lens, uint32_t n, int is_ascii, gamdp_multi_seqset** out)
{ (void)m; (void)seqs; (void)lens; (void)n; (void)is_ascii; if (out) *out = 0; return GAMDP_ENODEV; }
void gamdp_multi_seqset_destroy(gamdp_multi_seqset* s) { (void)s; }
int gamdp_multi_align_merge_blocks(gamdp_multi* m, const gamdp_multi_seqset* master, const gamdp_multi_seqset* slave, const gamdp_mb_in* in,
                                   size_t n, uint32_t band, gamdp_mb_out* out, gamdp_result* audit, uint32_t audit_stride)
{ (void)m; (void)master; (void)slave; (void)in; (void)n; (void)band; (void)out; (void)audit; (void)audit_stride; return GAMDP_ENODEV; }
int gamdp_ctx_set_walk_skip(gamdp_ctx* ctx, int mode) { (void)ctx; (void)mode; return GAMDP_ENODEV; }
int gamdp_ctx_walk_skip_stats(const gamdp_ctx* ctx, gamdp_walk_skip_stats* out) { (void)ctx; (void)out; return GAMDP_ENODEV; }
```

Before: 15510.

## Derive traceback match count from score algebra instead of per-run base comparisons

During the traceback walk of non-N kernels without ops output, diagonal runs after the first match are deferred instead of compared base-by-base. The match count is then solved from the final score, the bottom-row H value, the alignment length and the gap count. Only the first and last match runs still run the wavefront compare, and the walk falls back to full base counting when the algebraic closing has no match to anchor. An env flag restores the old counting path, and new stats count how often each path is taken. This cuts per-run memory loads, bpermutes and reductions in the traceback, at the cost of extra control logic and reliance on exact score arithmetic.

```diff
diff --git a/gam_ngs_amd/api.py b/gam_ngs_amd/api.py
--- a/gam_ngs_amd/api.py
+++ b/gam_ngs_amd/api.py
@@ -58,6 +58,11 @@
     def walk_skip_stats(self):
         st = L.WalkSkipStats()
         _check(self, self.lib.gamdp_ctx_walk_skip_stats(self.handle, C.byref(st)), "gamdp_ctx_walk_skip_stats")
+        return st.as_dict()
+
+    def walk_count_stats(self):
+        st = L.WalkCountStats()
+        _check(self, self.lib.gamdp_ctx_walk_count_stats(self.handle, C.byref(st)), "gamdp_ctx_walk_count_stats")
         return st.as_dict()
 
     def l1_tail_calls(self):
diff --git a/gam_ngs_amd/csrc/gamdp_dev.h b/gam_ngs_amd/csrc/gamdp_dev.h
--- a/gam_ngs_amd/csrc/gamdp_dev.h
+++ b/gam_ngs_amd/csrc/gamdp_dev.h
@@ -67,7 +67,9 @@
     u32 prio_R, prio_from;
     u32* stats;
 };
-enum : int { LS_UNITS = 0, LS_DIRFREE, LS_PACKED_TOP, LS_PACKED_TOP_MIXED, LS_STRIPS, LS_TOP_WANTED, LS_SKIP_TESTS, LS_SKIP_TESTED, LS_SKIP_GROUPS, LS_SKIP_SHORT, LS_COUNT = 12 };
+enum : int { LS_UNITS = 0, LS_DIRFREE, LS_PACKED_TOP, LS_PACKED_TOP_MIXED, LS_STRIPS, LS_TOP_WANTED, LS_SKIP_TESTS, LS_SKIP_TESTED, LS_SKIP_GROUPS, LS_SKIP_SHORT,
+              LS_WALK_SCORE, LS_WALK_FALLBACK, LS_COUNT = 12 };
+constexpr u32 LP_WALK_COUNT_BASES = 64;
 constexpr u32 LP_WALK_SKIP_DIAG = 32;
 constexpr u32 LP_WALK_SIDE_BY_SIDE = 1;
 constexpr u32 LP_NO_PACKED_TOP = 2;
@@ -213,6 +215,7 @@
     u32 skew_call;
     int32_t n_margin;
     u32 n_by_contig;
+    u32 walk_flags;
 };
 int chain_slots_per_workgroup();
 
diff --git a/gam_ngs_amd/csrc/gamdp_host.cpp b/gam_ngs_amd/csrc/gamdp_host.cpp
--- a/gam_ngs_amd/csrc/gamdp_host.cpp
+++ b/gam_ngs_amd/csrc/gamdp_host.cpp
@@ -76,6 +76,7 @@
         if ((e = std::getenv("GAMDP_L1_CHAIN_CARRY"))) x.l1_chain_carry = std::atoi(e) == 1;
         if ((e = std::getenv("GAMDP_L1_WALK_ANY_BAND"))) x.l1_walk_any_band = std::atoi(e) == 1;
         if ((e = std::getenv("GAMDP_WALK_SKIP"))) x.walk_skip = std::atoi(e) == 1;
+        if ((e = std::getenv("GAMDP_WALK_COUNT_BASES"))) x.walk_count_bases = std::atoi(e) == 1;
         return x;
     }();
     return t;
@@ -743,6 +744,7 @@
     p.flags = (L.kid == K_P17_CE4 && (u64)L.count / 2 <= tu.side_walk_rounds * L.n_slots) ? LP_WALK_SIDE_BY_SIDE : 0u;
     if (tu.no_packed_top) p.flags |= LP_NO_PACKED_TOP;
     if (tu.no_packed_top_mixed) p.flags |= LP_NO_PACKED_TOP_MIXED;
+    if (tu.walk_count_bases) p.flags |= LP_WALK_COUNT_BASES;
     if (L.kid == K_O19_CE15 && walk_skip == GAMDP_WALK_SKIP_DIAG) p.flags |= LP_WALK_SKIP_DIAG;
     p.flags |= (tu.walk_prio >= 0 ? (u32)tu.walk_prio : (units > 2ull * L.n_slots ? 1u : 0u)) << LP_WALK_PRIO_SHIFT;
     p.prio_R = tu.no_prio ? 0u : (u32)std::max<u64>(1, L.dir_words / (u64)kernel_info[L.kid].dir_block_words);
@@ -857,6 +859,7 @@
                 W.rows_skipped += 64ull * st[LS_SKIP_GROUPS] - st[LS_SKIP_SHORT];
                 W.strips += st[LS_STRIPS];
             }
+            last_walk_count.by_score += st[LS_WALK_SCORE]; last_walk_count.fallback += st[LS_WALK_FALLBACK];
             r.piece = log_piece;
             r.rounds = L.n_slots ? (double)r.units / (double)L.n_slots : 0.0;
             r.kernel_ms = (double)ms;
@@ -1182,6 +1185,16 @@
     return 0;
 }
 
+static_assert(sizeof(gamdp_walk_count_stats) == 24 && offsetof(gamdp_walk_count_stats, count_bases) == 16,
+              "gamdp_walk_count_stats: the layout include/gamdp.h documents (gam_ngs_amd/lib.py WalkCountStats mirrors it)");
+
+int gamdp_ctx_walk_count_stats(const gamdp_ctx* ctx, gamdp_walk_count_stats* out)
+{
+    if (!ctx || !out) return GAMDP_EINVAL;
+    *out = reinterpret_cast<const Ctx*>(ctx)->last_walk_count;
+    return 0;
+}
+
 int gamdp_seqset_create(gamdp_ctx* ctx, const uint8_t* const* seqs, const uint64_t* lens, uint32_t n, int is_ascii,
                         gamdp_seqset** out)
 {
@@ -1222,6 +1235,8 @@
     c->launch_log.clear();
     c->last_walk_skip = gamdp_walk_skip_stats{};
     c->last_walk_skip.mode = (uint32_t)c->walk_skip;
+    c->last_walk_count = gamdp_walk_count_stats{};
+    c->last_walk_count.count_bases = tuning().walk_count_bases ? 1u : 0u;
     struct LogGuard { Ctx* c; ~LogGuard() { c->log_launches = false; for (Ctx* h : c->helpers) h->log_launches = false; } } log_guard{c};
     c->log_launches = true; c->log_piece = 0;
     return guarded(c, [&]() -> int {
@@ -1256,6 +1271,7 @@
     cc[1]->kernel_ms = 0; cc[1]->kernel_launches = 0;
     cc[1]->launch_log.clear(); cc[1]->log_launches = true;
     cc[1]->walk_skip = c->walk_skip; cc[1]->last_walk_skip = gamdp_walk_skip_stats{};
+    cc[1]->last_walk_count = gamdp_walk_count_stats{};
     int rc[2] = {0, 0};
     auto worker = [&](int t) noexcept {
         for (size_t k = (size_t)t; k < 4 && rc[t] == 0; k += 2) {
@@ -1275,6 +1291,7 @@
         gamdp_walk_skip_stats& W = c->last_walk_skip;
         const gamdp_walk_skip_stats& H = cc[1]->last_walk_skip;
         W.tests += H.tests; W.groups_tested += H.groups_tested; W.groups_skipped += H.groups_skipped; W.rows_skipped += H.rows_skipped; W.strips += H.strips;
+        c->last_walk_count.by_score += cc[1]->last_walk_count.by_score; c->last_walk_count.fallback += cc[1]->last_walk_count.fallback;
     }
     std::stable_sort(c->launch_log.begin(), c->launch_log.end(), [](const gamdp_launch_info& x, const gamdp_launch_info& y) { return x.piece < y.piece; });
     if (rc[1]) c->set_error(cc[1]->err);
diff --git a/gam_ngs_amd/csrc/gamdp_internal.h b/gam_ngs_amd/csrc/gamdp_internal.h
--- a/gam_ngs_amd/csrc/gamdp_internal.h
+++ b/gam_ngs_amd/csrc/gamdp_internal.h
@@ -53,6 +53,7 @@
     bool l1_chain_carry = false;
     bool l1_walk_any_band = false;
     bool walk_skip = false;
+    bool walk_count_bases = false;
 };
 const Tuning& tuning();
 
@@ -182,6 +183,7 @@
     gamdp_l1_chain_stats last_l1_chain{};
     int walk_skip = GAMDP_WALK_STRIPS;
     gamdp_walk_skip_stats last_walk_skip{};
+    gamdp_walk_count_stats last_walk_count{};
     HitsBuffers* hits = nullptr;
 
     void set_error(const std::string& s) { err = s; }
diff --git a/gam_ngs_amd/csrc/gamdp_kernel.hip b/gam_ngs_amd/csrc/gamdp_kernel.hip
--- a/gam_ngs_amd/csrc/gamdp_kernel.hip
+++ b/gam_ngs_amd/csrc/gamdp_kernel.hip
@@ -776,7 +776,7 @@
     LaunchParams p;
     p.tasks = nullptr; p.n_tasks = 0; p.cursor = nullptr; p.results = cp.audit; p.ops_buf = nullptr;
     p.scratch = cp.scratch; p.slot_words = (u64)uni64((int64_t)mbp->slot_words); p.dir_words = (u64)uni64((int64_t)mbp->dir_words); p.ypad = cp.ypad;
-    p.ckpt_off = (u64)uni64((int64_t)mbp->ckpt_off); p.bnd_off = (u64)uni64((int64_t)mbp->bnd_off); p.flags = 0; p.prio_R = 0; p.prio_from = 0; p.stats = nullptr;
+    p.ckpt_off = (u64)uni64((int64_t)mbp->ckpt_off); p.bnd_off = (u64)uni64((int64_t)mbp->bnd_off); p.flags = cp.walk_flags; p.prio_R = 0; p.prio_from = 0; p.stats = nullptr;
     if (threadIdx.x == 0) {
         s_mail.filled = 0; s_mail.quit = 0; s_mail.total = 0; s_mail.claim = 0; s_mail.n_done = 0;
         for (int k = 0; k < CH_NS; ++k) { s_mail.early_of[k] = 0; s_mail.done_of[k] = 0; }
diff --git a/gam_ngs_amd/csrc/gamdp_l1.cpp b/gam_ngs_amd/csrc/gamdp_l1.cpp
--- a/gam_ngs_amd/csrc/gamdp_l1.cpp
+++ b/gam_ngs_amd/csrc/gamdp_l1.cpp
@@ -600,6 +600,7 @@
     cp.epoch = c->chain_epoch;
     cp.skew_call = diag().chain_skew;
     cp.n_margin = (int32_t)(64 - diag().n_window_shrink); cp.n_by_contig = diag().force_n ? 1u : 0u;
+    cp.walk_flags = tuning().walk_count_bases ? LP_WALK_COUNT_BASES : 0u;
     run.n_by_contig = cp.n_by_contig != 0;
     run.kernel = ck;
     run.scratch_bytes = S.need_scratch * sizeof(u32); run.n_launches = (u32)S.pieces.size(); run.n_twins = (u32)S.n_tw;
diff --git a/gam_ngs_amd/csrc/kernel_finish.inc b/gam_ngs_amd/csrc/kernel_finish.inc
--- a/gam_ngs_amd/csrc/kernel_finish.inc
+++ b/gam_ngs_amd/csrc/kernel_finish.inc
@@ -114,7 +114,7 @@
     uint8_t* const p_ops_buf = unip(pp->ops_buf);
     DevResult* const p_results = unip(pp->results);
     const int Y = t.Y;
-    const int wc_status = uni(wcp->status), best = uni(wcp->best);
+    const int wc_status = uni(wcp->status);
 
     DevResult res;
     res.begin_a = res.begin_b = res.score = 0;
@@ -138,7 +138,6 @@
             res.flags = ST_OUT_OF_RANGE << 8;
         } else {
             int x = uni(wcp->x), y = uni(wcp->y), pos = uni(wcp->pos);
-            const int end_pos = uni(wcp->end_pos), end_x = uni(wcp->end_x);
             const bool want_ops = dt_flags & TF_WANT_OPS;
             uint8_t* ops = p_ops_buf + dt_ops_off;
             u32 len = (u32)uni((int)wcp->len), nm = (u32)uni((int)wcp->nm);
@@ -200,8 +199,15 @@
                 }
                 x = -1;
             }
+            constexpr bool SCORE_COUNT = !HASN;
+            enum : int { CM_BASES = 0, CM_OPEN = 1, CM_CLOSED = 2 };
+            auto starts_open = [&]() -> bool { return SCORE_COUNT && !want_ops && uni((int)wcp->len) == 0 && !(uni((int)pp->flags) & (int)LP_WALK_COUNT_BASES); };
+            int count_mode = starts_open() ? CM_OPEN : CM_BASES, pend_n = 0;
+#ifdef GAMDP_DIAG
+            bool count_bad = false;
+#endif
             int walk_it = 0;
-            while (x >= 0 && y >= 0 && pos >= 0) {
+            while (x >= 0 && pos >= 0 && (y >= 0 || (SCORE_COUNT && count_mode == CM_OPEN))) {
                 if constexpr (EARLY) {
                     walk_it = uni(walk_it) + 1;
                     if ((walk_it & 31) == 0 && cancelled(t.cancel)) break;
@@ -215,7 +221,20 @@
                 old_q = uni(old_q); old_lo = uni(old_lo); old_hi = uni(old_hi);
                 sa_w0 = uni64(sa_w0); sb_w0 = uni64(sb_w0);
                 if (HASN) { san_w0 = uni64(san_w0); sbn_w0 = uni64(sbn_w0); }
-                if (x == 0 || pos == 0 || want_ops) {
+                int cmp_n = 0, cmp_pos = 0, cmp_x = 0;
+                bool closing = false;
+                int h_bot = 0;
+                if constexpr (SCORE_COUNT) {
+                    count_mode = uni(count_mode); pend_n = uni(pend_n);
+                    closing = count_mode == CM_OPEN && (x == 0 || pos == 0 || y < 0);
+                }
+                if (closing) {
+                    if (y >= 0) {
+                        count_mode = CM_CLOSED;
+                        h_bot = uni((x == 0) ? t.h0row[y] : t.pos0[x]);
+                        if (pend_n > 0) { cmp_n = pend_n; cmp_pos = fa; cmp_x = fb - t.begin_b; }
+                    } else count_mode = CM_BASES;
+                } else if (x == 0 || pos == 0 || want_ops) {
                     const int pa = HASN ? code_at(t.a2, t.an, t.a_base + pos) : (int)((t.a2[(t.a_base + pos) >> 4] >> (((t.a_base + pos) & 15) * 2)) & 3);
                     const int64_t bi = t.b_base + t.begin_b + x;
                     const int pb = HASN ? code_at(t.b2, t.bn, bi) : (int)((t.b2[bi >> 4] >> ((bi & 15) * 2)) & 3);
@@ -283,57 +302,8 @@
                     const int n_run = n;
                     n = min(n, min(x, pos));
                     if (n > 0) {
-                        const int64_t ia_hi = t.a_base + pos, ib_hi = t.b_base + t.begin_b + x;
-                        const int64_t wa = (ia_hi - 15) >> 4, wb = (ib_hi - 15) >> 4;
-                        const int64_t wa_bot = (ia_hi - n - 15) >> 4, wb_bot = (ib_hi - n - 15) >> 4;
-                        if (wa + 1 > sa_w0 || wa_bot < sa_w0 - 63) { sa_w0 = wa + 1; sa_v = t.a2[sa_w0 - lane]; }
-                        if (wb + 1 > sb_w0 || wb_bot < sb_w0 - 63) { sb_w0 = wb + 1; sb_v = t.b2[sb_w0 - lane]; }
-                        const int da = (int)(sa_w0 - wa), db = (int)(sb_w0 - wb);
-                        const u32 a16 = __builtin_amdgcn_alignbit((u32)wave_shr1(0, (int)sa_v), sa_v, (u32)((ia_hi - 15) & 15) * 2u);
-                        const u32 b16s = __builtin_amdgcn_alignbit((u32)wave_shr1(0, (int)sb_v), sb_v, (u32)((ib_hi - 15) & 15) * 2u);
-                        const u32 b16 = (u32)__builtin_amdgcn_ds_bpermute(4 * (lane + db - da), (int)b16s);
-                        const int j = lane - da;
-                        const u32 xr = a16 ^ b16;
-                        u32 ne = (xr | (xr >> 1)) & 0x55555555u;
-                        if constexpr (HASN) {
-                            const int64_t na_lo = ia_hi - 15 - 16 * (int64_t)j, nb_lo = ib_hi - 15 - 16 * (int64_t)j;
-                            const int64_t wna = (ia_hi >> 5) + 1, wnb = (ib_hi >> 5) + 1;
-                            const int64_t wna_bot = (ia_hi - n - 31) >> 5, wnb_bot = (ib_hi - n - 31) >> 5;
-                            if (wna > san_w0 || wna_bot < san_w0 - 63) { san_w0 = wna; san_v = t.an[san_w0 - lane]; }
-                            if (wnb > sbn_w0 || wnb_bot < sbn_w0 - 63) { sbn_w0 = wnb; sbn_v = t.bn[sbn_w0 - lane]; }
-                            auto nbits = [&](const u32 win, const int64_t w0, const int64_t lo) -> u32 {
-                                const int src = (int)(w0 - (lo >> 5));
-                                const u32 wl = (u32)__builtin_amdgcn_ds_bpermute(4 * src, (int)win);
-                                const u32 wh = (u32)__builtin_amdgcn_ds_bpermute(4 * (src - 1), (int)win);
-                                return __builtin_amdgcn_alignbit(wh, wl, (u32)(lo & 31)) & 0xFFFFu;
-                            };
-                            u32 nn = nbits(san_v, san_w0, na_lo) | nbits(sbn_v, sbn_w0, nb_lo);
-                            nn = (nn | (nn << 8)) & 0x00FF00FFu;
-                            nn = (nn | (nn << 4)) & 0x0F0F0F0Fu;
-                            nn = (nn | (nn << 2)) & 0x33333333u;
-                            nn = (nn | (nn << 1)) & 0x55555555u;
-                            ne &= ~nn;
-                        }
-                        const int p0 = 16 * j + 16 - n;
-                        u32 msk = (p0 <= 0) ? 0x55555555u : ((p0 >= 16) ? 0u : (0x55555555u << (2 * p0)));
-                        if (j < 0) msk = 0u;
-                        u32 eq = ~ne & msk;
-                        const u64 m_eq = __ballot(eq != 0u);
-                        if (m_eq) {
-                            int cnt = __builtin_popcount(eq);
-                            cnt += __builtin_amdgcn_update_dpp(0, cnt, 0xB1, 0xf, 0xf, true);
-                            cnt += __builtin_amdgcn_update_dpp(0, cnt, 0x4E, 0xf, 0xf, true);
-                            cnt += __builtin_amdgcn_update_dpp(0, cnt, 0x141, 0xf, 0xf, true);
-                            cnt += __builtin_amdgcn_update_dpp(0, cnt, 0x140, 0xf, 0xf, true);
-                            nm += (u32)(__builtin_amdgcn_readlane(cnt, 0) + __builtin_amdgcn_readlane(cnt, 16) +
-                                        __builtin_amdgcn_readlane(cnt, 32) + __builtin_amdgcn_readlane(cnt, 48));
-                            const int Ltop = __builtin_ctzll(m_eq), Lbot = 63 - __builtin_clzll(m_eq);
-                            const u32 eq_top = (u32)__builtin_amdgcn_readlane((int)eq, Ltop), eq_bot = (u32)__builtin_amdgcn_readlane((int)eq, Lbot);
-                            const int off_hi = 16 * (Ltop - da) + 15 - ((31 - __builtin_clz(eq_top)) >> 1);
-                            const int off_lo = 16 * (Lbot - da) + 15 - (__builtin_ctz(eq_bot) >> 1);
-                            if (!have_last) { have_last = true; la = pos - off_hi; lb = t.begin_b + x - off_hi; post_early((ST_OK << 8) | 2u, la, lb); }
-                            have_first = true; fa = pos - off_lo; fb = t.begin_b + x - off_lo;
-                        }
+                        if (count_mode == CM_BASES || !have_last) { cmp_n = n; cmp_pos = pos; cmp_x = x; pend_n = 0; }
+                        else { fa = pos; fb = t.begin_b + x; pend_n = n; }
                         x -= n; pos -= n; len += (u32)n;
                         if (Ls >= 0 && n == n_run && x >= 1 && pos >= 1) {
                             const u32 w2 = (u32)__builtin_amdgcn_readlane((int)cw, Ls);
@@ -359,18 +329,94 @@
                         len++;
                     }
                 }
+                if (cmp_n > 0) {
+                    const int64_t ia_hi = t.a_base + cmp_pos, ib_hi = t.b_base + t.begin_b + cmp_x;
+                    const int64_t wa = (ia_hi - 15) >> 4, wb = (ib_hi - 15) >> 4;
+                    const int64_t wa_bot = (ia_hi - cmp_n - 15) >> 4, wb_bot = (ib_hi - cmp_n - 15) >> 4;
+                    if (wa + 1 > sa_w0 || wa_bot < sa_w0 - 63) { sa_w0 = wa + 1; sa_v = t.a2[sa_w0 - lane]; }
+                    if (wb + 1 > sb_w0 || wb_bot < sb_w0 - 63) { sb_w0 = wb + 1; sb_v = t.b2[sb_w0 - lane]; }
+                    const int da = (int)(sa_w0 - wa), db = (int)(sb_w0 - wb);
+                    const u32 a16 = __builtin_amdgcn_alignbit((u32)wave_shr1(0, (int)sa_v), sa_v, (u32)((ia_hi - 15) & 15) * 2u);
+                    const u32 b16s = __builtin_amdgcn_alignbit((u32)wave_shr1(0, (int)sb_v), sb_v, (u32)((ib_hi - 15) & 15) * 2u);
+                    const u32 b16 = (u32)__builtin_amdgcn_ds_bpermute(4 * (lane + db - da), (int)b16s);
+                    const int j = lane - da;
+                    const u32 xr = a16 ^ b16;
+                    u32 ne = (xr | (xr >> 1)) & 0x55555555u;
+                    if constexpr (HASN) {
+                        const int64_t na_lo = ia_hi - 15 - 16 * (int64_t)j, nb_lo = ib_hi - 15 - 16 * (int64_t)j;
+                        const int64_t wna = (ia_hi >> 5) + 1, wnb = (ib_hi >> 5) + 1;
+                        const int64_t wna_bot = (ia_hi - cmp_n - 31) >> 5, wnb_bot = (ib_hi - cmp_n - 31) >> 5;
+                        if (wna > san_w0 || wna_bot < san_w0 - 63) { san_w0 = wna; san_v = t.an[san_w0 - lane]; }
+                        if (wnb > sbn_w0 || wnb_bot < sbn_w0 - 63) { sbn_w0 = wnb; sbn_v = t.bn[sbn_w0 - lane]; }
+                        auto nbits = [&](const u32 win, const int64_t w0, const int64_t lo) -> u32 {
+                            const int src = (int)(w0 - (lo >> 5));
+                            const u32 wl = (u32)__builtin_amdgcn_ds_bpermute(4 * src, (int)win);
+                            const u32 wh = (u32)__builtin_amdgcn_ds_bpermute(4 * (src - 1), (int)win);
+                            return __builtin_amdgcn_alignbit(wh, wl, (u32)(lo & 31)) & 0xFFFFu;
+                        };
+                        u32 nn = nbits(san_v, san_w0, na_lo) | nbits(sbn_v, sbn_w0, nb_lo);
+                        nn = (nn | (nn << 8)) & 0x00FF00FFu;
+                        nn = (nn | (nn << 4)) & 0x0F0F0F0Fu;
+                        nn = (nn | (nn << 2)) & 0x33333333u;
+                        nn = (nn | (nn << 1)) & 0x55555555u;
+                        ne &= ~nn;
+                    }
+                    const int p0 = 16 * j + 16 - cmp_n;
+                    u32 msk = (p0 <= 0) ? 0x55555555u : ((p0 >= 16) ? 0u : (0x55555555u << (2 * p0)));
+                    if (j < 0) msk = 0u;
+                    u32 eq = ~ne & msk;
+                    const u64 m_eq = __ballot(eq != 0u);
+                    if (m_eq) {
+                        int cnt = __builtin_popcount(eq);
+                        cnt += __builtin_amdgcn_update_dpp(0, cnt, 0xB1, 0xf, 0xf, true);
+                        cnt += __builtin_amdgcn_update_dpp(0, cnt, 0x4E, 0xf, 0xf, true);
+                        cnt += __builtin_amdgcn_update_dpp(0, cnt, 0x141, 0xf, 0xf, true);
+                        cnt += __builtin_amdgcn_update_dpp(0, cnt, 0x140, 0xf, 0xf, true);
+                        nm += (u32)(__builtin_amdgcn_readlane(cnt, 0) + __builtin_amdgcn_readlane(cnt, 16) +
+                                    __builtin_amdgcn_readlane(cnt, 32) + __builtin_amdgcn_readlane(cnt, 48));
+                        const int Ltop = __builtin_ctzll(m_eq), Lbot = 63 - __builtin_clzll(m_eq);
+                        const u32 eq_top = (u32)__builtin_amdgcn_readlane((int)eq, Ltop), eq_bot = (u32)__builtin_amdgcn_readlane((int)eq, Lbot);
+                        const int off_hi = 16 * (Ltop - da) + 15 - ((31 - __builtin_clz(eq_top)) >> 1);
+                        const int off_lo = 16 * (Lbot - da) + 15 - (__builtin_ctz(eq_bot) >> 1);
+                        if (!have_last) { have_last = true; la = cmp_pos - off_hi; lb = t.begin_b + cmp_x - off_hi; post_early((ST_OK << 8) | 2u, la, lb); }
+                        have_first = true; fa = cmp_pos - off_lo; fb = t.begin_b + cmp_x - off_lo;
+                    } else if (closing) count_mode = CM_BASES;
+                }
+                if (closing) {
+                    if (count_mode == CM_CLOSED) {
+                        const int n_gap = 2 * (int)len - (uni(wcp->x) - x) - (uni(wcp->pos) - pos);
+                        const int num = uni(wcp->best) - h_bot + 4 * (int)len + 4 * n_gap;
+#ifdef GAMDP_DIAG
+                        if (num % 9 != 0 || num < 0 || num / 9 > (int)len - n_gap) count_bad = true;
+#endif
+                        nm = (u32)(num / 9);
+                    } else {
+                        x = uni(wcp->x); y = uni(wcp->y); pos = uni(wcp->pos);
+                        len = (u32)uni((int)wcp->len); nm = (u32)uni((int)wcp->nm);
+                        have_last = uni(wcp->have) & 2; have_first = uni(wcp->have) & 1;
+                        la = uni(wcp->la); lb = uni(wcp->lb); fa = uni(wcp->fa); fb = uni(wcp->fb);
+                        l = y / C; c = y - l * C;
+                    }
+                }
             }
             res.begin_a = pos + 1;
             res.begin_b = t.begin_b + x + 1;
-            res.score = best;
+            res.score = uni(wcp->best);
             res.n_match = nm;
             res.length = len;
-            res.first_a = have_first ? fa : end_pos + 1;
-            res.first_b = have_first ? fb : t.begin_b + end_x + 1;
+            res.first_a = have_first ? fa : uni(wcp->end_pos) + 1;
+            res.first_b = have_first ? fb : t.begin_b + uni(wcp->end_x) + 1;
             res.last_a = have_last ? la : res.begin_a;
             res.last_b = have_last ? lb : res.begin_b;
             res.flags = (have_first ? 1u : 0u) | (have_last ? 2u : 0u) | (ST_OK << 8);
+#ifdef GAMDP_DIAG
+            if (count_bad) res.flags = ST_DIAG_RANGE << 8;
+#endif
             if (pp->stats != nullptr && lane == 0 && mat_calls > 0) atomicAdd(unip(pp->stats) + LS_STRIPS, (u32)mat_calls);
+            if (pp->stats != nullptr && lane == 0 && starts_open()) {
+                if (count_mode == CM_CLOSED) atomicAdd(unip(pp->stats) + LS_WALK_SCORE, 1u);
+                if (count_mode == CM_BASES) atomicAdd(unip(pp->stats) + LS_WALK_FALLBACK, 1u);
+            }
             if (dt_flags & TF_DIAG_COUNT_MAT) {
                 res.n_match = (u32)mat_calls;
                 res.first_a = (int)mat_ticks + uni(wcp->mat_ticks);
diff --git a/gam_ngs_amd/lib.py b/gam_ngs_amd/lib.py
--- a/gam_ngs_amd/lib.py
+++ b/gam_ngs_amd/lib.py
@@ -23,7 +23,7 @@
     "gamdp_find_hits_batch", "gamdp_ctx_set_l1_hits", "gamdp_ctx_l1_hits_stats",
     "gamdp_ctx_l1_tail_calls", "gamdp_score_batch", "gamdp_ctx_score_info", "gamdp_carry_batch", "gamdp_ctx_carry_info",
     "gamdp_ctx_set_l1_chain", "gamdp_ctx_l1_chain_stats", "gamdp_ctx_set_l1_walk_bands",
-    "gamdp_ctx_set_walk_skip", "gamdp_ctx_walk_skip_stats",
+    "gamdp_ctx_set_walk_skip", "gamdp_ctx_walk_skip_stats", "gamdp_ctx_walk_count_stats",
 ]
 
 EINVAL, ENODEV, ENOMEM, ENOTSUP, EHIP = -1, -2, -3, -4, -5
@@ -134,6 +134,13 @@
 class WalkSkipStats(C.Structure):
     _fields_ = [("tests", C.c_uint64), ("groups_tested", C.c_uint64), ("groups_skipped", C.c_uint64), ("rows_skipped", C.c_uint64),
                 ("strips", C.c_uint64), ("mode", C.c_uint32), ("pad_", C.c_uint32)]
+
+    def as_dict(self):
+        return {k: getattr(self, k) for k, _ in self._fields_ if k != "pad_"}
+
+
+class WalkCountStats(C.Structure):
+    _fields_ = [("by_score", C.c_uint64), ("fallback", C.c_uint64), ("count_bases", C.c_uint32), ("pad_", C.c_uint32)]
 
     def as_dict(self):
         return {k: getattr(self, k) for k, _ in self._fields_ if k != "pad_"}
@@ -247,6 +254,9 @@
         lib.gamdp_ctx_set_walk_skip.restype = C.c_int
         lib.gamdp_ctx_walk_skip_stats.argtypes = [vp, C.POINTER(WalkSkipStats)]
         lib.gamdp_ctx_walk_skip_stats.restype = C.c_int
+    if hasattr(lib, "gamdp_ctx_walk_count_stats"):
+        lib.gamdp_ctx_walk_count_stats.argtypes = [vp, C.POINTER(WalkCountStats)]
+        lib.gamdp_ctx_walk_count_stats.restype = C.c_int
     lib.gamdp_ctx_l1_hits_stats.argtypes = [vp, C.POINTER(L1HitsStats)]
     lib.gamdp_ctx_l1_hits_stats.restype = C.c_int
     lib.gamdp_ctx_l1_tail_calls.argtypes = [vp, C.POINTER(L1TailCall), C.c_size_t, C.POINTER(C.c_size_t)]
diff --git a/include/gamdp.h b/include/gamdp.h
--- a/include/gamdp.h
+++ b/include/gamdp.h
@@ -122,6 +122,14 @@
     uint32_t pad_;
 } gamdp_walk_skip_stats;
 int gamdp_ctx_walk_skip_stats(const gamdp_ctx* ctx, gamdp_walk_skip_stats* out);
+
+typedef struct gamdp_walk_count_stats {
+    uint64_t by_score;
+    uint64_t fallback;
+    uint32_t count_bases;
+    uint32_t pad_;
+} gamdp_walk_count_stats;
+int gamdp_ctx_walk_count_stats(const gamdp_ctx* ctx, gamdp_walk_count_stats* out);
 
 int gamdp_seqset_create(gamdp_ctx* ctx, const uint8_t* const* seqs, const uint64_t* lens, uint32_t n,
                         int is_ascii, gamdp_seqset** out);
diff --git a/integration/gamdp_stub.c b/integration/gamdp_stub.c
--- a/integration/gamdp_stub.c
+++ b/integration/gamdp_stub.c
@@ -11,3 +11,4 @@
 { (void)m; (void)master; (void)slave; (void)in; (void)n; (void)band; (void)out; (void)audit; (void)audit_stride; return GAMDP_ENODEV; }
 int gamdp_ctx_set_walk_skip(gamdp_ctx* ctx, int mode) { (void)ctx; (void)mode; return GAMDP_ENODEV; }
 int gamdp_ctx_walk_skip_stats(const gamdp_ctx* ctx, gamdp_walk_skip_stats* out) { (void)ctx; (void)out; return GAMDP_ENODEV; }
+int gamdp_ctx_walk_count_stats(const gamdp_ctx* ctx, gamdp_walk_count_stats* out) { (void)ctx; (void)out; return GAMDP_ENODEV; }
```

After: 15620, median of 6. No clear change (+0.7%).
